# EnricoMiccoli/nodal

Measured on AMD Instinct MI355X. Metric: circuits_per_sec, higher is better.
Workload: dtype f64; 1 GPU; cfg3: grid(1000) 1e6 nodes, sparse CSR path; n=999999, nnz=4995995, parallelism=one GPU

## Files before the change

nodal_amd/csrc/sagg.hip:

```cpp
#include <hip/hip_ext.h>

#include <atomic>
#include <type_traits>

#include "group.h"

int grounded_flags(nodal_ctx *h, uint8_t *flags_dev);

namespace {

using grp::TB;
constexpr int PW = 4;
constexpr int ACAP = 64;
constexpr int RCAP = 96;
constexpr int RCAP_SMALL = 512;
constexpr int RCAP_SMALL_ROWS = 16384;
inline int rcap_for(int64_t nc) { return nc <= RCAP_SMALL_ROWS ? RCAP_SMALL : RCAP; }
constexpr int W0_MAX = 32;
constexpr int COARSEST = 64;
constexpr int MAX_LEVELS = 12;
constexpr int MIS_ROUNDS = 6;
constexpr int TAIL_MAX_N = 1024;
constexpr int TAIL_LEVELS = 6;
constexpr int TAIL_LDS_BUDGET = 150 * 1024;
constexpr int APAD = 32;
constexpr int DOT_BLOCKS = 1024;
#ifndef NODAL_SA_OMEGA
#define NODAL_SA_OMEGA 0.85
#endif
constexpr double OMEGA = NODAL_SA_OMEGA;
constexpr double OMEGA_P = 0.70;
constexpr double OMEGA_P_COARSE = 0.85;
using cyc_t = nodal_cyc_t;

inline unsigned grid_for(int64_t n, unsigned cap = 8192) {
    int64_t g = (n + TB - 1) / TB;
    if (g < 1) g = 1;
    if (g >= 64) g = (g + 7) & ~(int64_t)7;
    return (unsigned)(g > cap ? cap : g);
}
inline int64_t pad64(int64_t n) { return (n + 63) & ~(int64_t)63; }
inline size_t align256(size_t x) { return (x + 255) & ~(size_t)255; }

__device__ __forceinline__ unsigned xcd_block() {
    const unsigned g = gridDim.x, b = blockIdx.x;
    return (g & 7u) ? b : (b & 7u) * (g >> 3) + (b >> 3);
}


struct Ell {
    int64_t n = 0, ld = 0;
    int32_t width = 0;
    const int32_t *col = nullptr;
    const int16_t *dcol = nullptr;
    const double *val = nullptr;
    const float *valf = nullptr;
    const int32_t *len = nullptr;
};

enum { ST_MAXLEN = 0, ST_GRADED = 1, ST_BADDIAG = 2, ST_OVERFLOW = 3, ST_NNZ = 4, ST_UNASSIGNED = 5,
       ST_MAXR = 6, ST_NC = 7 ,
       ST_FARCOL = 8 ,
       ST_FOLDMISS = 9 ,
       ST_COUNT = 10 };

struct SLevel {
    int64_t n = 0, ld = 0, nc = 0;
    int32_t width = 0;
    int32_t maxlen = 0;
    int32_t wfix = 0;
    int64_t nnz = 0;
    DevBuf acol, aval, alen, dinv;
    DevBuf adcol;
    bool d16 = false;
    DevBuf agg, pcol, pval;
    DevBuf rcol, rval, rlen;
    int64_t rld = 0;
    DevBuf vec, part, gflag;
    DevBuf avalf, pvalf, rvalf;
    DevBuf wcol, wval, wlen;
    int32_t wslots = 0;
    bool fold_want = false, fold = false;
    Ell A() const {
        Ell e;
        e.n = n; e.ld = ld; e.width = width;
        e.col = acol.as<int32_t>(); e.val = aval.as<double>(); e.len = alen.as<int32_t>();
        e.valf = avalf.as<float>();
        e.dcol = d16 ? adcol.as<int16_t>() : nullptr;
        return e;
    }
    template <typename T = double> T *v(int which) const { return reinterpret_cast<T *>(vec.as<double>() + (int64_t)which * ld); }
};
enum { V_X = 0, V_R = 1, V_XP = 2, V_RC = 3, V_C1 = 4, V_C2 = 5, V_V1 = 6, V_V2 = 7, V_R2 = 8, V_X1 = 9, V_T = 10,
       V_COUNT = 11 };

struct TailLevelDesc {
    int n, nc, ld, rld, width, nq, lpr;
    const int32_t *acol, *pcol, *rcol, *rlen, *alen;
    const double *aval, *dinv, *pval, *rval;
    int o_aval, o_acol, o_dinv, o_pval, o_pcol, o_rval, o_rcol, o_B, o_X, o_Y, o_R;
};
struct TailDesc {
    int nlev;
    TailLevelDesc lv[TAIL_LEVELS];
    const double *inv;
    int nu;
    int image_bytes;
    int lds_bytes;
    int skip;
    int slots;
    long long *stamps;
};

struct SHierarchy {
    std::vector<SLevel *> pool;
    int nlev = 0;
    int tail = -1;
    bool ready = false;
    bool kcycle = true;
    bool kfrozen = false;
    int kslot = -1, kcount = 0, ksamples = 0;
    int klevels = 1;
    int nu[3] = {2, 1, 2};
    bool dense_coarsest = true;
    DevBuf tail_stamps, tail_image, apcol, apval, aplen, bstat;
    DevBuf tail_op;
    bool tail_dense = false;
    DevBuf mvec;
    hipEvent_t ev_copy = nullptr;
    hipStream_t aux = nullptr;
    hipEvent_t ev_fork = nullptr, ev_join = nullptr, ev_flags = nullptr;
    bool aux_pending = false;
    bool aux_tried = false;
    bool want_flags = false;
    int flags_levels = 0;
    DevBuf stats, coarse_inv, mis_t, mis_m, mis_flag, mis_id, agg1, keys, rstart, cursor, lists;
    TailDesc td;
    uint64_t *host_stats = nullptr;
    bool sym_valid = false;
    uint64_t sym_epoch = 0;
    int64_t sym_n = 0, sym_nnz = 0;
    bool sym_general = false, sym_check = false;
    int32_t sym_floating = 0;
    hipGraph_t it_graph = nullptr;
    hipGraphExec_t it_exec = nullptr;
    uint64_t it_key = 0;
    bool refreshed = false;
    int last_iters = 0;
    int hint_iters = 0;
    int64_t hint_n = 0, hint_nnz = 0;
    int mblock_iters = 0;
    int64_t mblock_n = 0;
    unsigned long long sym_stats[MAX_LEVELS * ST_COUNT] = {0};
    SLevel *level(int l) {
        while ((int)pool.size() <= l) pool.push_back(new SLevel());
        return pool[l];
    }
    void drop_graph() {
        if (it_exec) (void)hipGraphExecDestroy(it_exec);
        if (it_graph) (void)hipGraphDestroy(it_graph);
        it_exec = nullptr;
        it_graph = nullptr;
        it_key = 0;
    }
    ~SHierarchy() {
        drop_graph();
        if (ev_copy) (void)hipEventDestroy(ev_copy);
        if (ev_fork) (void)hipEventDestroy(ev_fork);
        if (ev_join) (void)hipEventDestroy(ev_join);
        if (ev_flags) (void)hipEventDestroy(ev_flags);
        if (aux) (void)hipStreamDestroy(aux);
        for (SLevel *l : pool) {
            DevBuf *b[] = {&l->acol, &l->aval, &l->alen, &l->dinv, &l->agg, &l->pcol, &l->pval, &l->rcol,
                           &l->rval, &l->rlen, &l->vec, &l->part, &l->gflag, &l->avalf, &l->pvalf, &l->rvalf, &l->adcol,
                           &l->wcol, &l->wval, &l->wlen};
            for (DevBuf *x : b) x->release();
            delete l;
        }
        tail_image.release();
        tail_op.release();
        mvec.release();
        tail_stamps.release();
        bstat.release();
        apcol.release();
        apval.release();
        aplen.release();
        DevBuf *b[] = {&stats, &coarse_inv, &mis_t, &mis_m, &mis_flag, &mis_id, &agg1, &keys, &rstart, &cursor, &lists};
        for (DevBuf *x : b) x->release();
        if (host_stats) (void)hipHostFree(host_stats);
    }
};


constexpr int BSTAT_MAX = 65536;
__global__ __launch_bounds__(1024) void reduce_bstat(int nblocks, const uint32_t *__restrict__ bstat,
                                                     unsigned long long *__restrict__ stats, int slot_max,
                                                     int slot_sum) {
    __shared__ unsigned int s_max;
    __shared__ unsigned long long s_sum;
    if (threadIdx.x == 0) { s_max = 0; s_sum = 0; }
    __syncthreads();
    unsigned int m = 0;
    unsigned long long t = 0;
    for (int i = threadIdx.x; i < nblocks; i += 1024) {
        m = max(m, bstat[i]);
        t += bstat[BSTAT_MAX + i];
    }
    atomicMax(&s_max, m);
    atomicAdd(&s_sum, t);
    __syncthreads();
    if (threadIdx.x == 0) {
        if (slot_max >= 0) stats[slot_max] = s_max;
        if (slot_sum >= 0) stats[slot_sum] = s_sum;
    }
}

__global__ __launch_bounds__(TB) void row_stats(int64_t n, const int32_t *__restrict__ indptr,
                                                const int32_t *__restrict__ indices,
                                                const double *__restrict__ data, double share, double spread,
                                                bool general, unsigned long long *__restrict__ stats,
                                                uint32_t *__restrict__ bstat) {
    int32_t mlen = 0;
    uint32_t graded = 0, bad = 0, far = 0;
    for (int64_t i = (int64_t)xcd_block() * TB + threadIdx.x; i < n; i += (int64_t)gridDim.x * TB) {
        const int32_t e0 = indptr[i], e1 = indptr[i + 1];
        mlen = max(mlen, e1 - e0);
        double d = 0.0, mx = 0.0, mn = 1e300;
        for (int32_t e = e0; e < e1; ++e) {
            const double v = data[e];
            const int64_t dc = (int64_t)indices[e] - i;
            if (dc > 32767 || dc < -32767) far = 1;
            if (indices[e] == (int32_t)i) d = v;
            else if (v != 0.0) {
                mx = fmax(mx, fabs(v));
                mn = fmin(mn, fabs(v));
                if (v > 0.0 && !general) bad = 1;
            }
        }
        if (!(d > 0.0)) bad = 1;
        graded += (d > 0.0 && (mx > share * d || mx > spread * mn)) ? 1u : 0u;
    }
    __shared__ unsigned int s_len, s_graded, s_bad;
    if (threadIdx.x == 0) s_len = s_graded = s_bad = 0;
    __syncthreads();
    atomicMax(&s_len, (unsigned)mlen);
    if (graded) atomicAdd(&s_graded, graded);
    if (bad) atomicOr(&s_bad, 1u);
    if (far) atomicOr(&s_bad, 2u);
    __syncthreads();
    if (threadIdx.x == 0) {
        bstat[blockIdx.x] = s_len;
        bstat[BSTAT_MAX + blockIdx.x] = s_graded;
        if (s_bad & 1u) atomicOr(&stats[ST_BADDIAG], 1ull);
        if (s_bad & 2u) stats[ST_FARCOL] = 1ull;
    }
}

__global__ __launch_bounds__(TB) void csr_to_ell(int64_t n, int64_t ld, const int32_t *__restrict__ indptr,
                                                 const int32_t *__restrict__ indices,
                                                 const double *__restrict__ data, int32_t *__restrict__ col,
                                                 double *__restrict__ val, float *__restrict__ valf,
                                                 int32_t *__restrict__ len, double *__restrict__ dinv, int32_t wpad,
                                                 int16_t *__restrict__ dcol) {
    for (int64_t i = (int64_t)xcd_block() * TB + threadIdx.x; i < n; i += (int64_t)gridDim.x * TB) {
        const int32_t e0 = indptr[i], e1 = indptr[i + 1];
        double d = 1.0;
        for (int32_t e = e0; e < e1; ++e) {
            const int32_t c = indices[e];
            const double v = data[e];
            col[(int64_t)(e - e0) * ld + i] = c;
            if (dcol) dcol[(int64_t)(e - e0) * ld + i] = (int16_t)(c - (int32_t)i);
            val[(int64_t)(e - e0) * ld + i] = v;
            valf[(int64_t)(e - e0) * ld + i] = (float)v;
            if (c == (int32_t)i) d = v;
        }
        for (int32_t s = e1 - e0; s < wpad; ++s) {
            col[(int64_t)s * ld + i] = (int32_t)i;
            if (dcol) dcol[(int64_t)s * ld + i] = 0;
            val[(int64_t)s * ld + i] = 0.0;
            valf[(int64_t)s * ld + i] = 0.0f;
        }
        len[i] = e1 - e0;
        dinv[i] = 1.0 / d;
    }
}


__device__ __forceinline__ uint32_t hash30(uint32_t x) {
    x ^= x >> 16;
    x *= 0x7feb352du;
    x ^= x >> 15;
    x *= 0x846ca68bu;
    x ^= x >> 16;
    return x & 0x3fffffffu;
}

__global__ __launch_bounds__(TB) void mis_init(int64_t n, uint32_t *__restrict__ T) {
    for (int64_t i = (int64_t)xcd_block() * TB + threadIdx.x; i < n; i += (int64_t)gridDim.x * TB)
        T[i] = (1u << 30) | hash30((uint32_t)i);
}

template <int NB>
__device__ __forceinline__ uint32_t nbr_max_batch(const Ell &A, const uint32_t *__restrict__ v, int64_t i, int32_t l, int32_t s0,
                                                  uint32_t best) {
    int32_t c[NB];
#pragma unroll
    for (int u = 0; u < NB; ++u) c[u] = A.col[(int64_t)(s0 + u < l ? s0 + u : 0) * A.ld + i];
    uint32_t t[NB];
#pragma unroll
    for (int u = 0; u < NB; ++u) t[u] = v[c[u]];
#pragma unroll
    for (int u = 0; u < NB; ++u) best = t[u] > best ? t[u] : best;
    return best;
}
__device__ __forceinline__ uint32_t nbr_max(const Ell &A, const uint32_t *__restrict__ v, int64_t i, int32_t l, uint32_t best) {
    if (l <= 5) return nbr_max_batch<5>(A, v, i, l, 0, best);
    for (int32_t s0 = 0; s0 < l; s0 += 8) best = nbr_max_batch<8>(A, v, i, l, s0, best);
    return best;
}

__global__ __launch_bounds__(TB) void mis_max(Ell A, const uint32_t *__restrict__ v, uint32_t *__restrict__ m) {
    for (int64_t i = (int64_t)xcd_block() * TB + threadIdx.x; i < A.n; i += (int64_t)gridDim.x * TB)
        m[i] = nbr_max(A, v, i, A.len[i], v[i]);
}

__global__ __launch_bounds__(TB) void mis_update(Ell A, uint32_t *__restrict__ T, const uint32_t *__restrict__ m1) {
    for (int64_t i = (int64_t)xcd_block() * TB + threadIdx.x; i < A.n; i += (int64_t)gridDim.x * TB) {
        const uint32_t own = T[i];
        if ((own >> 30) != 1) continue;
        const uint32_t best = nbr_max(A, m1, i, A.len[i], m1[i]);
        if (best == own) T[i] = own | (2u << 30);
        else if ((best >> 30) == 3) T[i] = 0;
    }
}

__global__ __launch_bounds__(TB) void mis_count(int64_t n, const uint32_t *__restrict__ T,
                                                unsigned long long *__restrict__ out) {
    uint32_t left = 0;
    for (int64_t i = (int64_t)xcd_block() * TB + threadIdx.x; i < n; i += (int64_t)gridDim.x * TB)
        left += (T[i] >> 30) == 1 ? 1u : 0u;
#pragma unroll
    for (int off = 32; off > 0; off >>= 1) left += __shfl_down(left, off, 64);
    if ((threadIdx.x & 63) == 0 && left) atomicAdd(out, (unsigned long long)left);
}

__global__ __launch_bounds__(TB) void mis_flag_roots(Ell A, const uint32_t *__restrict__ T,
                                                     uint32_t *__restrict__ flag) {
    for (int64_t i = (int64_t)xcd_block() * TB + threadIdx.x; i <= A.n; i += (int64_t)gridDim.x * TB) {
        uint32_t f = 0;
        if (i < A.n) {
            const uint32_t own = T[i];
            if ((own >> 30) == 3) f = 1;
            else if ((own >> 30) == 1) {
                bool near = false;
                const int32_t l = A.len[i];
                for (int32_t s = 0; s < l; ++s) near = near || (T[A.col[(int64_t)s * A.ld + i]] >> 30) == 3;
                f = near ? 0u : 1u;
            }
        }
        flag[i] = f;
    }
}

constexpr int64_t MIS_SMALL_MAX = 1024;
__global__ __launch_bounds__(1024) void mis_small(Ell A, uint32_t *__restrict__ T, uint32_t *__restrict__ M,
                                                  uint32_t *__restrict__ flag, int rounds) {
    const int64_t n = A.n;
    for (int64_t i = threadIdx.x; i < n; i += 1024) T[i] = (1u << 30) | hash30((uint32_t)i);
    __syncthreads();
    for (int r = 0; r < rounds; ++r) {
        for (int64_t i = threadIdx.x; i < n; i += 1024) {
            uint32_t best = T[i];
            const int32_t l = A.len[i];
            for (int32_t s = 0; s < l; ++s) {
                const uint32_t t = T[A.col[(int64_t)s * A.ld + i]];
                best = t > best ? t : best;
            }
            M[i] = best;
        }
        __syncthreads();
        for (int64_t i = threadIdx.x; i < n; i += 1024) {
            const uint32_t own = T[i];
            if ((own >> 30) != 1) continue;
            uint32_t best = M[i];
            const int32_t l = A.len[i];
            for (int32_t s = 0; s < l; ++s) {
                const uint32_t t = M[A.col[(int64_t)s * A.ld + i]];
                best = t > best ? t : best;
            }
            if (best == own) T[i] = own | (2u << 30);
            else if ((best >> 30) == 3) T[i] = 0;
        }
        __syncthreads();
    }
    for (int64_t i = threadIdx.x; i <= n; i += 1024) {
        uint32_t f = 0;
        if (i < n) {
            const uint32_t own = T[i];
            if ((own >> 30) == 3) f = 1;
            else if ((own >> 30) == 1) {
                bool near = false;
                const int32_t l = A.len[i];
                for (int32_t s = 0; s < l; ++s) near = near || (T[A.col[(int64_t)s * A.ld + i]] >> 30) == 3;
                f = near ? 0u : 1u;
            }
        }
        flag[i] = f;
    }
}

__global__ __launch_bounds__(TB) void assign_near(Ell A, const uint32_t *__restrict__ T,
                                                  const uint32_t *__restrict__ flag,
                                                  const uint32_t *__restrict__ id, int32_t *__restrict__ agg1) {
    for (int64_t i = (int64_t)xcd_block() * TB + threadIdx.x; i < A.n; i += (int64_t)gridDim.x * TB) {
        int32_t a = -1;
        if (flag[i]) a = (int32_t)id[i];
        else {
            uint32_t best = 0;
            const int32_t l = A.len[i];
            auto batch = [&](auto NBc, int32_t s0) {
                constexpr int NB = decltype(NBc)::value;
                int32_t c[NB];
#pragma unroll
                for (int u = 0; u < NB; ++u) c[u] = A.col[(int64_t)(s0 + u < l ? s0 + u : 0) * A.ld + i];
                uint32_t fl[NB], tt[NB], idd[NB];
#pragma unroll
                for (int u = 0; u < NB; ++u) {
                    fl[u] = flag[c[u]];
                    tt[u] = T[c[u]];
                    idd[u] = id[c[u]];
                }
#pragma unroll
                for (int u = 0; u < NB; ++u) {
                    if (s0 + u >= l || c[u] == (int32_t)i || !fl[u]) continue;
                    const uint32_t t = tt[u] | (3u << 30);
                    if (t > best) { best = t; a = (int32_t)idd[u]; }
                }
            };
            if (l <= 5) batch(std::integral_constant<int, 5>{}, 0);
            else for (int32_t s0 = 0; s0 < l; s0 += 8) batch(std::integral_constant<int, 8>{}, s0);
        }
        agg1[i] = a;
    }
}

__global__ __launch_bounds__(TB) void assign_far(Ell A, const int32_t *__restrict__ agg1, int32_t *__restrict__ agg,
                                                 unsigned long long *__restrict__ stats) {
    for (int64_t i = (int64_t)xcd_block() * TB + threadIdx.x; i < A.n; i += (int64_t)gridDim.x * TB) {
        int32_t a = agg1[i];
        if (a < 0) {
            double bw = -1.0;
            const int32_t l = A.len[i];
            auto batch = [&](auto NBc, int32_t s0) {
                constexpr int NB = decltype(NBc)::value;
                int32_t c[NB];
                double w[NB];
#pragma unroll
                for (int u = 0; u < NB; ++u) {
                    const int64_t at = (int64_t)(s0 + u < l ? s0 + u : 0) * A.ld + i;
                    c[u] = A.col[at];
                    w[u] = fabs(A.val[at]);
                }
                int32_t aj[NB];
#pragma unroll
                for (int u = 0; u < NB; ++u) aj[u] = agg1[c[u]];
#pragma unroll
                for (int u = 0; u < NB; ++u) {
                    if (s0 + u >= l || c[u] == (int32_t)i || aj[u] < 0) continue;
                    if (w[u] > bw) { bw = w[u]; a = aj[u]; }
                }
            };
            if (l <= 5) batch(std::integral_constant<int, 5>{}, 0);
            else for (int32_t s0 = 0; s0 < l; s0 += 8) batch(std::integral_constant<int, 8>{}, s0);
            if (a < 0) stats[ST_UNASSIGNED] = 1;
        }
        agg[i] = a;
    }
}
// ... 59 lines not shown
                                               const uint64_t *__restrict__ keys, int64_t ld,
                                               const double *__restrict__ pval, int32_t *__restrict__ rcol,
                                               double *__restrict__ rval, float *__restrict__ rvalf,
                                               int32_t *__restrict__ rlen,
                                               unsigned long long *__restrict__ stats, uint32_t *__restrict__ bstat,
                                               uint32_t rcap) {
    uint32_t mlen = 0;
    const int sub = threadIdx.x & 7;
    const int64_t rows_per_pass = (int64_t)gridDim.x * (TB / 8);
    for (int64_t I = (int64_t)xcd_block() * (TB / 8) + threadIdx.x / 8; I < nc; I += rows_per_pass) {
        const uint32_t s0 = rstart[I];
        uint32_t l = rstart[I + 1] - s0;
        mlen = l > mlen ? l : mlen;
        if (l > rcap) l = rcap;
        const uint32_t upto = nc <= 4096 ? rcap : ((l + 7u) & ~7u);
        for (uint32_t t = sub; t < upto; t += 8) {
            const int64_t at = ((int64_t)(t >> 3) * rld + I) * 8 + (t & 7);
            if (t < l) {
                const uint64_t key = keys[s0 + t];
                const int64_t i = (int64_t)(key >> 2);
                const double v = pval[(int64_t)(key & 3) * ld + i];
                rcol[at] = (int32_t)i;
                rval[at] = v;
                rvalf[at] = (float)v;
            } else {
                rcol[at] = 0;
                rval[at] = 0.0;
                rvalf[at] = 0.0f;
            }
        }
        if (sub == 0) rlen[I] = (int32_t)l;
    }
    if (mlen > rcap) atomicOr(&stats[ST_OVERFLOW], 2ull);
    __shared__ unsigned int s_max;
    if (threadIdx.x == 0) s_max = 0;
    __syncthreads();
#pragma unroll
    for (int off = 32; off > 0; off >>= 1) {
        const uint32_t o = __shfl_down(mlen, off, 64);
        mlen = o > mlen ? o : mlen;
    }
    if ((threadIdx.x & 63) == 0) atomicMax(&s_max, mlen);
    __syncthreads();
    if (threadIdx.x == 0) {
        bstat[blockIdx.x] = s_max;
        bstat[BSTAT_MAX + blockIdx.x] = 0;
    }
}

__global__ __launch_bounds__(TB) void r_refresh(int64_t nc, int64_t rld, const int32_t *__restrict__ rlen,
                                                const int32_t *__restrict__ rcol, int64_t ld,
                                                const int32_t *__restrict__ pcol, const double *__restrict__ pval,
                                                double *__restrict__ rval, float *__restrict__ rvalf) {
    const int sub = threadIdx.x & 7;
    const int64_t rows_per_pass = (int64_t)gridDim.x * (TB / 8);
    for (int64_t I = (int64_t)xcd_block() * (TB / 8) + threadIdx.x / 8; I < nc; I += rows_per_pass) {
        const int32_t l = rlen[I];
        for (int32_t t = sub; t < l; t += 8) {
            const int64_t at = ((int64_t)(t >> 3) * rld + I) * 8 + (t & 7);
            const int64_t i = rcol[at];
            double v = 0.0;
#pragma unroll
            for (int k = 0; k < PW; ++k) {
                const double pv = pval[(int64_t)k * ld + i];
                v = pcol[(int64_t)k * ld + i] == (int32_t)I ? pv : v;
            }
            rval[at] = v;
            rvalf[at] = (float)v;
        }
    }
}

__global__ __launch_bounds__(TB) void r_sort_short(const uint32_t *__restrict__ rstart, uint64_t *__restrict__ keys,
                                                   int64_t nc) {
    for (int64_t I = (int64_t)xcd_block() * TB + threadIdx.x; I < nc; I += (int64_t)gridDim.x * TB) {
        const uint32_t s0 = rstart[I];
        const int len = (int)(rstart[I + 1] - s0);
        if (len < 2) continue;
        if (len <= 4) grp::sort_short_row<4>(keys + s0, len);
        else if (len <= 8) grp::sort_short_row<8>(keys + s0, len);
        else if (len <= 16) grp::sort_short_row<16>(keys + s0, len);
        else if (len <= 32) grp::sort_short_row<32>(keys + s0, len);
    }
}
__global__ __launch_bounds__(64) void r_sort_medium(const uint32_t *__restrict__ rstart, uint64_t *__restrict__ keys,
                                                    int64_t nc) {
    __shared__ uint64_t buf[RCAP_SMALL];
    const int lane = threadIdx.x;
    for (int64_t I = blockIdx.x; I < nc; I += gridDim.x) {
        const uint32_t s0 = rstart[I];
        const int len = (int)(rstart[I + 1] - s0);
        if (len <= 32 || len > RCAP_SMALL) continue;
        const int P = len <= 64 ? 64 : (len <= 128 ? 128 : (len <= 256 ? 256 : 512));
        for (int e = lane; e < P; e += 64) buf[e] = e < len ? keys[s0 + e] : ~0ull;
        __syncthreads();
        for (int size = 2; size <= P; size <<= 1)
            for (int stride = size >> 1; stride > 0; stride >>= 1) {
                for (int p = lane; p < P / 2; p += 64) {
                    const int i = ((p & ~(stride - 1)) << 1) | (p & (stride - 1));
                    const int j = i | stride;
                    const bool up = (i & size) == 0;
                    const uint64_t a = buf[i], b = buf[j];
                    if ((a > b) == up) { buf[i] = b; buf[j] = a; }
                }
                __syncthreads();
            }
        for (int e = lane; e < len; e += 64) keys[s0 + e] = buf[e];
        __syncthreads();
    }
}

__device__ __forceinline__ int wave_excl_scan(int v, int *total) {
    const int lane = threadIdx.x & 63;
    int incl = v;
#pragma unroll
    for (int off = 1; off < 64; off <<= 1) {
        const int t = __shfl_up(incl, off, 64);
        if (lane >= off) incl += t;
    }
    *total = __shfl(incl, 63, 64);
    return incl - v;
}

template <int APW, bool EMIT>
__global__ __launch_bounds__(TB) void ap_rows(Ell A, const int32_t *__restrict__ pcol, const double *__restrict__ pval,
                                              int32_t *__restrict__ apcol, double *__restrict__ apval,
                                              int32_t *__restrict__ aplen, unsigned long long *__restrict__ stats,
                                              const double *__restrict__ dinv, int32_t *__restrict__ wcol,
                                              float *__restrict__ wval, int32_t *__restrict__ wlen) {
    bool overflow = false, miss = false;
    for (int64_t i = (int64_t)xcd_block() * TB + threadIdx.x; i < A.n; i += (int64_t)gridDim.x * TB) {
        int32_t c[APW];
        double v[APW];
        [[maybe_unused]] int32_t Jo[PW];
        [[maybe_unused]] double po[PW], wd = 0.0;
        if constexpr (EMIT) {
#pragma unroll
            for (int sp = 0; sp < PW; ++sp) {
                Jo[sp] = pcol[(int64_t)sp * A.ld + i];
                po[sp] = pval[(int64_t)sp * A.ld + i];
            }
            wd = OMEGA * dinv[i];
        }
#pragma unroll
        for (int q = 0; q < APW; ++q) { c[q] = -1; v[q] = 0.0; }
        int cnt = 0;
        const int32_t l = A.len[i];
        for (int32_t s = 0; s < l; ++s) {
            const int32_t k = A.col[(int64_t)s * A.ld + i];
            const double a = A.val[(int64_t)s * A.ld + i];
            int32_t J[PW];
            double pp[PW];
#pragma unroll
            for (int sp = 0; sp < PW; ++sp) {
                J[sp] = pcol[(int64_t)sp * A.ld + k];
                pp[sp] = pval[(int64_t)sp * A.ld + k];
            }
#pragma unroll
            for (int sp = 0; sp < PW; ++sp) {
                if (J[sp] < 0) continue;
                const double t = a * pp[sp];
                bool placed = false;
#pragma unroll
                for (int q = 0; q < APW; ++q)
                    if (!placed && c[q] == J[sp]) { v[q] += t; placed = true; }
#pragma unroll
                for (int q = 0; q < APW; ++q)
                    if (!placed && c[q] < 0) { c[q] = J[sp]; v[q] = t; placed = true; cnt = q + 1; }
                if (!placed) overflow = true;
            }
        }
#pragma unroll
        for (int q = 0; q < APW; ++q)
            if (q < cnt) {
                apcol[(int64_t)q * A.ld + i] = c[q];
                apval[(int64_t)q * A.ld + i] = v[q];
            }
        aplen[i] = cnt;
        if constexpr (EMIT) {
            int have = 0, found = 0;
#pragma unroll
            for (int sp = 0; sp < PW; ++sp) have += Jo[sp] >= 0 ? 1 : 0;
#pragma unroll
            for (int q = 0; q < APW; ++q)
                if (q < cnt) {
                    double pv = 0.0;
#pragma unroll
                    for (int sp = 0; sp < PW; ++sp)
                        if (Jo[sp] == c[q]) { pv += po[sp]; ++found; }
                    wcol[(int64_t)q * A.ld + i] = c[q];
                    wval[(int64_t)q * A.ld + i] = (float)(pv - wd * v[q]);
                }
            wlen[i] = cnt;
            if (found != have) miss = true;
        }
    }
    if (overflow) atomicOr(&stats[ST_OVERFLOW], 4ull);
    if (miss) stats[ST_FOLDMISS] = 1ull;
}

template <int APW, bool EMIT>
__global__ __launch_bounds__(64) void ap_rows_lds(Ell A, const int32_t *__restrict__ pcol,
                                                  const double *__restrict__ pval, int32_t *__restrict__ apcol,
                                                  double *__restrict__ apval, int32_t *__restrict__ aplen,
                                                  unsigned long long *__restrict__ stats,
                                                  const double *__restrict__ dinv, int32_t *__restrict__ wcol,
                                                  float *__restrict__ wval, int32_t *__restrict__ wlen) {
    __shared__ int32_t tc[APW * 64];
    __shared__ double tv[APW * 64];
    const int lane = threadIdx.x;
    bool overflow = false, miss = false;
    for (int64_t i0 = (int64_t)xcd_block() * 64; i0 < A.n; i0 += (int64_t)gridDim.x * 64) {
        const int64_t i = i0 + lane;
#pragma unroll 8
        for (int q = 0; q < APW; ++q) tc[q * 64 + lane] = -1;
        int cnt = 0;
        if (i < A.n) {
            const int32_t l = A.len[i];
            [[maybe_unused]] int32_t Jo[PW];
            [[maybe_unused]] double po[PW], wd = 0.0;
            if constexpr (EMIT) {
#pragma unroll
                for (int sp = 0; sp < PW; ++sp) {
                    Jo[sp] = pcol[(int64_t)sp * A.ld + i];
                    po[sp] = pval[(int64_t)sp * A.ld + i];
                }
                wd = OMEGA * dinv[i];
            }
            constexpr int AB = 4;
            for (int32_t s0 = 0; s0 < l; s0 += AB) {
                int32_t kk[AB];
                double aa[AB];
#pragma unroll
                for (int u = 0; u < AB; ++u) {
                    const int32_t su = s0 + u < l ? s0 + u : 0;
                    kk[u] = A.col[(int64_t)su * A.ld + i];
                    aa[u] = A.val[(int64_t)su * A.ld + i];
                }
                int32_t J[AB][PW];
                double pp[AB][PW];
#pragma unroll
                for (int u = 0; u < AB; ++u)
#pragma unroll
                    for (int sp = 0; sp < PW; ++sp) {
                        J[u][sp] = pcol[(int64_t)sp * A.ld + kk[u]];
                        pp[u][sp] = pval[(int64_t)sp * A.ld + kk[u]];
                    }
#pragma unroll
                for (int u = 0; u < AB; ++u) {
                    if (s0 + u >= l) continue;
#pragma unroll
                    for (int sp = 0; sp < PW; ++sp) {
                        if (J[u][sp] < 0) continue;
                        const double t = aa[u] * pp[u][sp];
                        uint32_t slot = ((uint32_t)J[u][sp] * 2654435761u) >> 16 & (APW - 1);
                        bool placed = false;
                        for (int probe = 0; probe < APW && !placed; ++probe) {
                            const int32_t c = tc[slot * 64 + lane];
                            if (c == J[u][sp]) {
                                tv[slot * 64 + lane] += t;
                                placed = true;
                            } else if (c < 0) {
                                tc[slot * 64 + lane] = J[u][sp];
                                tv[slot * 64 + lane] = t;
                                ++cnt;
                                placed = true;
                            }
                            slot = (slot + 1) & (APW - 1);
                        }
                        if (!placed) overflow = true;
                    }
                }
            }
            int o = 0, found = 0;
            for (int q = 0; q < APW; ++q) {
                const int32_t c = tc[q * 64 + lane];
                if (c >= 0) {
                    const double t = tv[q * 64 + lane];
                    apcol[(int64_t)o * A.ld + i] = c;
                    apval[(int64_t)o * A.ld + i] = t;
                    if constexpr (EMIT) {
                        double pv = 0.0;
#pragma unroll
                        for (int sp = 0; sp < PW; ++sp)
                            if (Jo[sp] == c) { pv += po[sp]; ++found; }
                        wcol[(int64_t)o * A.ld + i] = c;
                        wval[(int64_t)o * A.ld + i] = (float)(pv - wd * t);
                    }
                    ++o;
                }
            }
            aplen[i] = cnt;
            if constexpr (EMIT) {
                int have = 0;
#pragma unroll
                for (int sp = 0; sp < PW; ++sp) have += Jo[sp] >= 0 ? 1 : 0;
                wlen[i] = cnt;
                if (found != have) miss = true;
            }
        }
    }
    if (overflow) atomicOr(&stats[ST_OVERFLOW], 4ull);
    if (miss) stats[ST_FOLDMISS] = 1ull;
}

__device__ __forceinline__ int galerkin_products(int64_t ld, const int32_t *__restrict__ apcol,
                                                 const double *__restrict__ apval, const int32_t *__restrict__ aplen,
                                                 int64_t rld, const int32_t *__restrict__ rcol,
                                                 const double *__restrict__ rval, int64_t I, int t0, int tn,
                                                 int32_t *lJ, double *lV) {
    const int lane = threadIdx.x;
    int32_t i = 0, len = 0;
    double w = 0.0;
    if (lane < tn) {
        const int t = t0 + lane;
        const int64_t rat = ((int64_t)(t >> 3) * rld + I) * 8 + (t & 7);
        i = rcol[rat];
        w = rval[rat];
        len = aplen[i];
    }
    int np = 0;
    int o = wave_excl_scan(len, &np);
    constexpr int INFL = 8;
    for (int32_t s0 = 0; s0 < len; s0 += INFL) {
        int32_t cj[INFL];
        double cv[INFL];
#pragma unroll
        for (int q = 0; q < INFL; ++q) {
            const int32_t s = s0 + q < len ? s0 + q : s0;
            cj[q] = apcol[(int64_t)s * ld + i];
            cv[q] = apval[(int64_t)s * ld + i];
        }
#pragma unroll
        for (int q = 0; q < INFL; ++q)
            if (s0 + q < len) {
                lJ[o] = cj[q];
                lV[o] = w * cv[q];
                ++o;
            }
    }
    for (int p = lane + np; p < np + 72; p += 64) lJ[p] = -1;
    __syncthreads();
    return np;
}

template <bool NUMERIC>
__global__ __launch_bounds__(64) void galerkin(int64_t ld, const int32_t *__restrict__ apcol,
                                               const double *__restrict__ apval, const int32_t *__restrict__ aplen,
                                               int64_t nc, int64_t rld, const int32_t *__restrict__ rcol,
                                               const double *__restrict__ rval, const int32_t *__restrict__ rlen,
                                               int64_t cld, int32_t *__restrict__ ccol, double *__restrict__ cval,
                                               float *__restrict__ cvalf,
                                               int32_t *__restrict__ clen, double *__restrict__ cdinv,
                                               unsigned long long *__restrict__ stats, uint32_t *__restrict__ bstat,
                                               int G, int pcap, int maxseg) {
    extern __shared__ __attribute__((aligned(16))) char gsm[];
    int32_t *set = reinterpret_cast<int32_t *>(gsm);
    double *lV = reinterpret_cast<double *>(gsm + 1024);
    int32_t *lJ = reinterpret_cast<int32_t *>(lV + pcap);
    const int lane = threadIdx.x;
    uint32_t my_max = 0, my_nnz = 0, my_flags = 0;
    for (int64_t I = blockIdx.x; I < nc; I += gridDim.x) {
        const int rl = rlen[I];
        const int ngroups = (rl + G - 1) / G;
        int np = 0;
        int total = 0;
        int32_t myJ = 0x7fffffff;
        if constexpr (NUMERIC) {
            total = clen[I];
            if (lane < total) myJ = ccol[(int64_t)lane * cld + I];
        } else {
        for (int k = lane; k < 256; k += 64) set[k] = -1;
        __syncthreads();
        for (int g = 0; g < ngroups; ++g) {
            np = galerkin_products(ld, apcol, apval, aplen, rld, rcol, rval, I, g * G, min(G, rl - g * G), lJ, lV);
            for (int p = lane; p < np; p += 64) {
                const int32_t J = lJ[p];
                uint32_t hsh = ((uint32_t)J * 2654435761u) >> 24;
                for (int probe = 0; probe < 256; ++probe) {
                    const int32_t old = atomicCAS(&set[hsh], -1, J);
                    if (old == -1 || old == J) break;
                    hsh = (hsh + 1) & 255u;
                    if (probe == 255) my_flags |= 1u;
                }
            }
            __syncthreads();
        }
        int32_t mine[4];
        int cnt = 0;
#pragma unroll
        for (int q = 0; q < 4; ++q) {
            mine[q] = set[lane * 4 + q];
            cnt += mine[q] >= 0 ? 1 : 0;
        }
        int off = wave_excl_scan(cnt, &total);
        __syncthreads();
#pragma unroll
        for (int q = 0; q < 4; ++q)
            if (mine[q] >= 0) set[off++] = mine[q];
        __syncthreads();
        if (total > ACAP) {
            my_flags |= 1u;
            total = ACAP;
        }
        myJ = lane < total ? set[lane] : 0x7fffffff;
        __syncthreads();
#pragma unroll
        for (int k = 2; k <= 64; k <<= 1) {
#pragma unroll
            for (int j = k >> 1; j > 0; j >>= 1) {
                const int32_t other = __shfl_xor(myJ, j, 64);
                const bool up = (lane & k) == 0, lower = (lane & j) == 0;
                const int32_t lo = myJ < other ? myJ : other, hi = myJ < other ? other : myJ;
                myJ = (lower == up) ? lo : hi;
            }
        }
        }
        const int nseg = min(maxseg, total <= 16 ? 4 : (total <= 32 ? 2 : 1)), segw = 64 / nseg;
        const int seg = lane / segw;
        const int32_t segJ = __shfl(myJ, lane % segw, 64);
        double acc = 0.0;
        for (int g = 0; g < ngroups; ++g) {
            if (ngroups > 1 || NUMERIC)
                np = galerkin_products(ld, apcol, apval, aplen, rld, rcol, rval, I, g * G, min(G, rl - g * G), lJ, lV);
            int chunk = (((np + nseg - 1) / nseg) + 7) & ~7;
            if (nseg > 1 && ((chunk >> 3) & 1) == 0) chunk += 8;
            for (int p = seg * chunk; p < (seg + 1) * chunk; p += 8) {
                int32_t j8[8];
                double v8[8];
#pragma unroll
                for (int u = 0; u < 8; ++u) {
                    j8[u] = lJ[p + u];
                    v8[u] = lV[p + u];
                }
#pragma unroll
                for (int u = 0; u < 8; ++u) acc += j8[u] == segJ ? v8[u] : 0.0;
            }
            __syncthreads();
        }
        if (nseg == 4) {
            const double a1 = __shfl(acc, lane + 16, 64), a2 = __shfl(acc, lane + 32, 64), a3 = __shfl(acc, lane + 48, 64);
            acc = (acc + a1) + (a2 + a3);
        } else if (nseg == 2) {
            acc += __shfl(acc, lane + 32, 64);
        }
        if (lane >= total && lane < APAD) {
            ccol[(int64_t)lane * cld + I] = (int32_t)I;
            cval[(int64_t)lane * cld + I] = 0.0;
            cvalf[(int64_t)lane * cld + I] = 0.0f;
        }
        if (lane < total) {
            ccol[(int64_t)lane * cld + I] = myJ;
            cval[(int64_t)lane * cld + I] = acc;
            cvalf[(int64_t)lane * cld + I] = (float)acc;
            if (myJ == (int32_t)I) {
                if (!(acc > 0.0)) my_flags |= 4u;
                cdinv[I] = acc > 0.0 ? 1.0 / acc : 1.0;
            }
        }
        if (lane == 0) {
            clen[I] = total;
            my_max = (uint32_t)total > my_max ? (uint32_t)total : my_max;
            my_nnz += (uint32_t)total;
        }
        __syncthreads();
    }
    if (lane == 0) {
        bstat[blockIdx.x] = my_max;
        bstat[BSTAT_MAX + blockIdx.x] = my_nnz;
    }
    if (my_flags & 1u) atomicOr(&stats[ST_OVERFLOW], 1ull);
    if (my_flags & 4u) atomicOr(&stats[ST_BADDIAG], 1ull);
}

__global__ __launch_bounds__(256) void coarsest_inverse(Ell A, double *__restrict__ inv,
                                                        unsigned long long *__restrict__ stats) {
    __shared__ double M[COARSEST][2 * COARSEST + 1];
    const int n = (int)A.n;
    for (int t = threadIdx.x; t < n * 2 * n; t += 256) {
        const int r = t / (2 * n), c = t % (2 * n);
        M[r][c] = (c >= n && c - n == r) ? 1.0 : 0.0;
    }
    __syncthreads();
    for (int r = threadIdx.x; r < n; r += 256)
        for (int s = 0; s < A.len[r]; ++s) M[r][A.col[(int64_t)s * A.ld + r]] = A.val[(int64_t)s * A.ld + r];
    __syncthreads();
    for (int k = 0; k < n; ++k) {
        const double pv = M[k][k];
        if (!(pv > 0.0)) {
            if (threadIdx.x == 0) atomicOr(&stats[ST_BADDIAG], 2ull);
            return;
        }
        const double rp = 1.0 / pv;
        __syncthreads();
        for (int c = threadIdx.x; c < 2 * n; c += 256) M[k][c] *= rp;
        __syncthreads();
        for (int t = threadIdx.x; t < n * 2 * n; t += 256) {
            const int r = t / (2 * n), c = t % (2 * n);
            if (r != k && c != k) M[r][c] = fma(-M[r][k], M[k][c], M[r][c]);
        }
        __syncthreads();
        for (int r = threadIdx.x; r < n; r += 256)
            if (r != k) M[r][k] = 0.0;
        __syncthreads();
    }
    for (int t = threadIdx.x; t < n * n; t += 256) inv[t] = M[t / n][n + t % n];
}

__global__ __launch_bounds__(TB) void flags_up(int64_t n, const int32_t *__restrict__ agg,
                                               const uint8_t *__restrict__ fine, uint8_t *__restrict__ coarse) {
    for (int64_t i = (int64_t)xcd_block() * TB + threadIdx.x; i < n; i += (int64_t)gridDim.x * TB)
        if (fine[i]) coarse[agg[i]] = 1;
}
__global__ __launch_bounds__(64) void last_level_floating(Ell A, const uint8_t *__restrict__ grounded,
                                                          uint32_t *__restrict__ floating) {
    __shared__ int label[COARSEST];
    __shared__ int changed;
    const int n = (int)A.n, i = threadIdx.x;
    if (i < n) label[i] = i;
    __syncthreads();
    for (int it = 0; it < COARSEST; ++it) {
        if (i == 0) changed = 0;
        __syncthreads();
        int best = i < n ? label[i] : 0;
        if (i < n)
            for (int s = 0; s < A.len[i]; ++s) {
                const int l = label[A.col[(int64_t)s * A.ld + i]];
                best = l < best ? l : best;
            }
        __syncthreads();
        if (i < n && best < label[i]) {
            label[i] = best;
            changed = 1;
        }
        __syncthreads();
        if (!changed) break;
        __syncthreads();
    }
    __shared__ int ok[COARSEST];
    if (i < n) ok[i] = 0;
    __syncthreads();
    if (i < n && grounded[i]) ok[label[i]] = 1;
    __syncthreads();
    if (i < n && label[i] == i && !ok[i]) *floating = 1;
}

__global__ __launch_bounds__(TB) void any_unflagged(int64_t n, const uint8_t *__restrict__ grounded,
                                                    uint32_t *__restrict__ floating) {
    for (int64_t i = (int64_t)xcd_block() * TB + threadIdx.x; i < n; i += (int64_t)gridDim.x * TB)
        if (!grounded[i]) *floating = 1;
}

}

#include "sagg_cycle.h"

namespace {

constexpr int SAGG_DECLINED = -3;

int width_class(int maxlen) {
    static const int classes[] = {4, 5, 6, 8, 12, 16, 20, 24, 32};
    for (int c : classes)
        if (maxlen <= c) return c;
    return 0;
}
int choose_wfix(int maxlen, int64_t n, int64_t nnz, int pad_limit) {
    const int c = width_class(maxlen);
    if (c == 0 || c > pad_limit) return 0;
    static const double slack = getenv("NODAL_SA_PADSLACK") ? atof(getenv("NODAL_SA_PADSLACK")) : 1.3;
    if ((double)c * (double)n <= slack * (double)nnz || n <= 32768) return c;
    return 0;
}

SHierarchy *hierarchy_of(nodal_ctx *h) {
    if (!h->sagg) h->sagg = new SHierarchy();
    return static_cast<SHierarchy *>(h->sagg);
}

struct SolveBufs {
    double *r, *p, *p2, *Ap, *part_rz, *part_zap, *part_rr, *part_pap, *sc;
    cyc_t *z, *x0;
    int g0;
};

template <bool NUMERIC>
int galerkin_product(nodal_ctx *h, SHierarchy *H, int l, hipEvent_t r_ready = nullptr, int phase = 0) {
    hipStream_t st = h->stream;
    SLevel *L = H->level(l), *C = H->level(l + 1);
    const int64_t n = L->n, ld = L->ld, nc = C->n;
    Ell A = L->A();
    A.width = L->maxlen;
    unsigned long long *dstats = H->stats.as<unsigned long long>();
    const int apw = A.width <= 6 ? 16 : 64;
    NODAL_HIP_TRY(h, H->apcol.reserve((size_t)apw * ld * 4 + 64));
    NODAL_HIP_TRY(h, H->apval.reserve((size_t)apw * ld * 8 + 64));
    NODAL_HIP_TRY(h, H->aplen.reserve((size_t)ld * 4 + 64));
    int32_t *apcol = H->apcol.as<int32_t>(), *aplen = H->aplen.as<int32_t>();
    double *apval = H->apval.as<double>();
    unsigned long long *lst = dstats + (size_t)l * ST_COUNT;
    const unsigned g = grid_for(n);
    if (phase != 2) {
        const bool w = L->fold_want && L->wslots == apw;
        int32_t *wcol = w ? L->wcol.as<int32_t>() : nullptr, *wlen = w ? L->wlen.as<int32_t>() : nullptr;
        float *wval = w ? L->wval.as<float>() : nullptr;
        const double *dinv = L->dinv.as<double>();
        const int32_t *pc = L->pcol.as<int32_t>();
        const double *pv = L->pval.as<double>();
        const unsigned gl = (unsigned)((n + 63) / 64 < 4096 ? (n + 63) / 64 : 4096);
        if (apw == 16 && w) ap_rows<16, true><<<g, TB, 0, st>>>(A, pc, pv, apcol, apval, aplen, lst, dinv, wcol, wval, wlen);
        else if (apw == 16) ap_rows<16, false><<<g, TB, 0, st>>>(A, pc, pv, apcol, apval, aplen, lst, dinv, wcol, wval, wlen);
        else if (w) ap_rows_lds<64, true><<<gl, 64, 0, st>>>(A, pc, pv, apcol, apval, aplen, lst, dinv, wcol, wval, wlen);
        else ap_rows_lds<64, false><<<gl, 64, 0, st>>>(A, pc, pv, apcol, apval, aplen, lst, dinv, wcol, wval, wlen);
        NODAL_HIP_TRY(h, hipGetLastError());
    }
    if (phase == 1) return NODAL_OK;
    int G = 1024 / apw;
    G = (G < 8 ? 8 : (G > 64 ? 64 : G));
    static const int g_env = getenv("NODAL_SA_GG") ? atoi(getenv("NODAL_SA_GG")) : 40;
    if (g_env >= 8 && g_env <= 64 && apw == 16) G = g_env & ~7;
    const int pcap = G * apw + 72;
    const size_t lds = 1024 + (size_t)pcap * 12;
    static const int64_t gcap = getenv("NODAL_SA_GCAP") ? atoll(getenv("NODAL_SA_GCAP")) : 16384;
    static const int maxseg = getenv("NODAL_SA_GSEG") ? atoi(getenv("NODAL_SA_GSEG")) : 4;
    const unsigned gg = (unsigned)(nc < gcap ? nc : (gcap < BSTAT_MAX ? gcap : BSTAT_MAX));
    if (r_ready) NODAL_HIP_TRY(h, hipStreamWaitEvent(st, r_ready, 0));
    galerkin<NUMERIC><<<gg, 64, lds, st>>>(
        ld, apcol, apval, aplen, nc, L->rld, L->rcol.as<int32_t>(), L->rval.as<double>(), L->rlen.as<int32_t>(),
        C->ld, C->acol.as<int32_t>(), C->aval.as<double>(), C->avalf.as<float>(), C->alen.as<int32_t>(),
        C->dinv.as<double>(), dstats + (size_t)(l + 1) * ST_COUNT, H->bstat.as<uint32_t>(), G, pcap, maxseg);
    if (!NUMERIC)
        reduce_bstat<<<1, 1024, 0, st>>>((int)gg, H->bstat.as<uint32_t>(), dstats + (size_t)(l + 1) * ST_COUNT,
                                         ST_MAXLEN, ST_NNZ);
    NODAL_HIP_TRY(h, hipGetLastError());
    return NODAL_OK;
}

double omega_p(int level) {
    static double w[2] = {-1.0, -1.0};
    if (w[0] < 0.0) {
        double a = OMEGA_P, b = OMEGA_P_COARSE;
        if (const char *e = getenv("NODAL_SA_OMEGA_P")) {
            a = atof(e);
            const char *c = strchr(e, ',');
            b = c ? atof(c + 1) : a;
        }
        w[1] = b > 0.0 && b < 1.2 ? b : OMEGA_P_COARSE;
        w[0] = a > 0.0 && a < 1.0 ? a : OMEGA_P;
    }
    return w[level > 0 ? 1 : 0];
}

constexpr int64_t FOLD_MAX_ROWS = 1 << 19;
struct FoldSetting { int mode = 0; unsigned mask = 0; };
const FoldSetting &fold_setting() {
    static const FoldSetting s = [] {
        FoldSetting f;
        const char *e = getenv("NODAL_SA_FOLD_POST");
        if (!e || !*e) return f;
        if (strchr(e, 'l')) {
            f.mode = 3;
            for (const char *q = e; (q = strchr(q, 'l')) != nullptr; ++q) {
                const int k = atoi(q + 1);
                if (q[1] >= '0' && q[1] <= '9' && k < MAX_LEVELS) f.mask |= 1u << k;
            }
        } else {
            f.mode = atoi(e) == 0 ? 1 : 2;
        }
        return f;
    }();
    return s;
}
bool fold_wanted(int level, int64_t n) {
    if (level > 0 && n <= TAIL_MAX_N) return false;
    const FoldSetting &f = fold_setting();
    switch (f.mode) {
    case 1: return false;
    case 2: return true;
    case 3: return (f.mask >> level & 1u) != 0;
    default: return n <= FOLD_MAX_ROWS;
    }
}
void decide_folds(SHierarchy *H, const unsigned long long *hs, bool trace) {
    for (int k = 0; k < H->nlev; ++k) {
        SLevel *L = H->pool[k];
        const bool runs_cycle = k + 1 < H->nlev && (H->tail < 0 || k < H->tail);
        const bool miss = hs[(size_t)k * ST_COUNT + ST_FOLDMISS] != 0;
        L->fold = L->fold_want && runs_cycle && !miss;
        if (trace && L->fold_want && runs_cycle)
            fprintf(stderr, "[sagg] level %d (%lld rows): first post-smoothing sweep %s\n", k, (long long)L->n,
                    miss ? "NOT folded: a row of A P lacks a column of its P row (no stored diagonal)"
                         : "folded into the prolongation");
    }
}

int build_level(nodal_ctx *h, SHierarchy *H, int l, unsigned long long *hs, bool *declined, bool *stop) {
    hipStream_t st = h->stream;
    SLevel *L = H->level(l);
    const int64_t n = L->n, ld = L->ld;
    Ell A = L->A();
    A.width = L->maxlen;
    unsigned long long *dstats = H->stats.as<unsigned long long>();

    NODAL_HIP_TRY(h, H->mis_t.reserve((size_t)n * 8 + 64));
    NODAL_HIP_TRY(h, H->mis_m.reserve((size_t)n * 8 + 64));
    NODAL_HIP_TRY(h, H->mis_flag.reserve((size_t)(n + 1) * 4 + 64));
    NODAL_HIP_TRY(h, H->mis_id.reserve((size_t)(n + 1) * 4 + 64 + scan_tmp_bytes(n + 1)));
    NODAL_HIP_TRY(h, H->agg1.reserve((size_t)n * 4 + 64));
    NODAL_HIP_TRY(h, L->agg.reserve((size_t)n * 4 + 64));
    NODAL_HIP_TRY(h, H->cursor.reserve((MIS_ROUNDS + 2) * 8 + 64));
    uint32_t *T = H->mis_t.as<uint32_t>(), *M = H->mis_m.as<uint32_t>();
    uint32_t *flag = H->mis_flag.as<uint32_t>(), *id = H->mis_id.as<uint32_t>();
    unsigned long long *cnt = H->cursor.as<unsigned long long>();
    void *scan_tmp = H->mis_id.as<char>() + (((size_t)(n + 1) * 4 + 63) & ~(size_t)63);

    const unsigned g = grid_for(n);
    static const bool trace_mis = getenv("NODAL_TRACE") != nullptr;
    if (trace_mis) NODAL_HIP_TRY(h, hipMemsetAsync(cnt, 0, (MIS_ROUNDS + 2) * 8, st));
    static const int mis_rounds = getenv("NODAL_SA_MIS") ? std::min(MIS_ROUNDS, std::max(1, atoi(getenv("NODAL_SA_MIS")))) : MIS_ROUNDS;
    if (n <= MIS_SMALL_MAX && !trace_mis) {
        mis_small<<<1, 1024, 0, st>>>(A, T, M, flag, mis_rounds);
    } else {
        mis_init<<<g, TB, 0, st>>>(n, T);
        for (int r = 0; r < mis_rounds; ++r) {
            mis_max<<<g, TB, 0, st>>>(A, T, M);
            mis_update<<<g, TB, 0, st>>>(A, T, M);
            if (trace_mis) mis_count<<<g, TB, 0, st>>>(n, T, cnt + r + 1);
        }
        mis_flag_roots<<<grid_for(n + 1), TB, 0, st>>>(A, T, flag);
    }
    NODAL_HIP_TRY(h, hipGetLastError());
    NODAL_TRY(scan_exclusive_u32(h, flag, id, n + 1, reinterpret_cast<uint32_t *>(dstats + (size_t)l * ST_COUNT + ST_NC),
                                 scan_tmp));
    NODAL_HIP_TRY(h, hipMemcpyAsync(hs, dstats, (size_t)MAX_LEVELS * ST_COUNT * 8, hipMemcpyDeviceToHost, st));
    unsigned long long hcnt[MIS_ROUNDS + 1] = {0};
    if (trace_mis) NODAL_HIP_TRY(h, hipMemcpyAsync(hcnt, cnt, sizeof hcnt, hipMemcpyDeviceToHost, st));
    if (!H->ev_copy) NODAL_HIP_TRY(h, hipEventCreateWithFlags(&H->ev_copy, hipEventDisableTiming));
    NODAL_HIP_TRY(h, hipEventRecord(H->ev_copy, st));
    NODAL_HIP_TRY(h, L->pcol.reserve((size_t)PW * ld * 4 + 64));
    NODAL_HIP_TRY(h, L->pval.reserve((size_t)PW * ld * 8 + 64));
    NODAL_HIP_TRY(h, L->pvalf.reserve((size_t)PW * ld * 4 + 64));
    assign_near<<<g, TB, 0, st>>>(A, T, flag, id, H->agg1.as<int32_t>());
    assign_far<<<g, TB, 0, st>>>(A, H->agg1.as<int32_t>(), L->agg.as<int32_t>(), dstats + (size_t)l * ST_COUNT);
    build_P<<<g, TB, 0, st>>>(A, L->dinv.as<double>(), L->agg.as<int32_t>(), L->pcol.as<int32_t>(),
                             L->pval.as<double>(), L->pvalf.as<float>(), omega_p(l));
    NODAL_HIP_TRY(h, hipGetLastError());
    NODAL_WAIT_EVENT(h, H->ev_copy, st);
    if (trace_mis) {
        fprintf(stderr, "[sagg] level %d: undecided after each MIS round:", l);
        for (int r = 1; r <= MIS_ROUNDS; ++r) fprintf(stderr, " %llu", hcnt[r]);
        fprintf(stderr, "\n");
    }
    const int64_t nc = (int64_t)(hs[(size_t)l * ST_COUNT + ST_NC] & 0xffffffffull);
    if (l > 0) {
        const unsigned long long *s = hs + (size_t)l * ST_COUNT;
        L->maxlen = (int32_t)s[ST_MAXLEN];
        L->nnz = (int64_t)s[ST_NNZ];
        A.width = L->maxlen;
        if (s[ST_OVERFLOW] || s[ST_BADDIAG] || hs[(size_t)(l - 1) * ST_COUNT + ST_OVERFLOW] ||
            hs[(size_t)(l - 1) * ST_COUNT + ST_UNASSIGNED]) {
            *declined = true;
            return NODAL_OK;
        }
    }
    if (nc >= n || L->maxlen <= 1) {
        *stop = true;
        return NODAL_OK;
    }
    if ((nc * 2 > n && n > 4096) || nc < 1) {
        *declined = true;
        return NODAL_OK;
    }
    L->nc = nc;

    static const bool fork_allowed = !(getenv("NODAL_SA_FORK") && atoi(getenv("NODAL_SA_FORK")) == 0);
    if (H->aux && !nodal_extra_streams_ok(h) && nodal_calls_in_flight() <= 1) {
        NODAL_WAIT_STREAM(h, H->aux);
        (void)hipStreamDestroy(H->aux);
        H->aux = nullptr;
        H->aux_tried = false;
    }
    if (fork_allowed && !H->aux_tried && nodal_extra_streams_ok(h)) {
        H->aux_tried = true;
        if (hipStreamCreateWithFlags(&H->aux, hipStreamNonBlocking) != hipSuccess) H->aux = nullptr;
        if (H->aux && ((!H->ev_fork && hipEventCreateWithFlags(&H->ev_fork, hipEventDisableTiming) != hipSuccess) ||
                       (!H->ev_join && hipEventCreateWithFlags(&H->ev_join, hipEventDisableTiming) != hipSuccess) ||
                       (!H->ev_flags && hipEventCreateWithFlags(&H->ev_flags, hipEventDisableTiming) != hipSuccess))) {
            (void)hipStreamDestroy(H->aux);
            H->aux = nullptr;
        }
        (void)hipGetLastError();
    }
    const bool forked = fork_allowed && H->aux != nullptr && nodal_extra_streams_ok(h);
    const size_t a4 = (((size_t)(nc + 1) * 4) + 255) & ~(size_t)255;
    const size_t scan2 = (scan_tmp_bytes(nc + 1) + 255) & ~(size_t)255;
    NODAL_HIP_TRY(h, H->rstart.reserve(a4 + 256 + scan2 + (size_t)PW * ld * 4 + 64));
    NODAL_HIP_TRY(h, H->keys.reserve((size_t)PW * n * 8 + 64));
    SLevel *C = H->level(l + 1);
    C->n = nc;
    C->ld = pad64(nc);
    C->width = ACAP;
    C->nc = 0;
    L->rld = C->ld;
    const int rcap = rcap_for(nc);
    NODAL_HIP_TRY(h, L->rcol.reserve((size_t)rcap * C->ld * 4 + 64));
    NODAL_HIP_TRY(h, L->rval.reserve((size_t)rcap * C->ld * 8 + 64));
    NODAL_HIP_TRY(h, L->rvalf.reserve((size_t)rcap * C->ld * 4 + 64));
    NODAL_HIP_TRY(h, L->rlen.reserve((size_t)C->ld * 4 + 64));
    NODAL_HIP_TRY(h, C->acol.reserve((size_t)ACAP * C->ld * 4 + 64));
    NODAL_HIP_TRY(h, C->aval.reserve((size_t)ACAP * C->ld * 8 + 64));
    NODAL_HIP_TRY(h, C->avalf.reserve((size_t)ACAP * C->ld * 4 + 64));
    NODAL_HIP_TRY(h, C->alen.reserve((size_t)C->ld * 4 + 64));
    NODAL_HIP_TRY(h, C->dinv.reserve((size_t)C->ld * 8 + 64));
    if (forked && H->want_flags) {
        if (l == 0) NODAL_HIP_TRY(h, L->gflag.reserve((size_t)n + 64));
        NODAL_HIP_TRY(h, C->gflag.reserve((size_t)C->n + 64));
    }
    {
        const int apw = L->maxlen <= 6 ? 16 : 64;
        NODAL_HIP_TRY(h, H->apcol.reserve((size_t)apw * ld * 4 + 64));
        NODAL_HIP_TRY(h, H->apval.reserve((size_t)apw * ld * 8 + 64));
        NODAL_HIP_TRY(h, H->aplen.reserve((size_t)ld * 4 + 64));
        L->fold = false;
        L->fold_want = fold_wanted(l, n);
        L->wslots = apw;
        if (L->fold_want) {
            NODAL_HIP_TRY(h, L->wcol.reserve((size_t)apw * ld * 4 + 64));
            NODAL_HIP_TRY(h, L->wval.reserve((size_t)apw * ld * 4 + 64));
            NODAL_HIP_TRY(h, L->wlen.reserve((size_t)ld * 4 + 64));
        }
    }
    hipStream_t main_st = h->stream;
    struct StreamGuard {
        nodal_ctx *h;
        hipStream_t keep;
        ~StreamGuard() { h->stream = keep; }
    } guard{h, main_st};
    if (forked) {
        NODAL_HIP_TRY(h, hipEventRecord(H->ev_fork, main_st));
        NODAL_HIP_TRY(h, hipStreamWaitEvent(H->aux, H->ev_fork, 0));
        H->aux_pending = true;
        NODAL_TRY(galerkin_product<false>(h, H, l, nullptr, 1));
        h->stream = H->aux;
        st = H->aux;
    }
    char *rs = H->rstart.as<char>();
    uint32_t *rstart = reinterpret_cast<uint32_t *>(rs);
    void *scan_tmp2 = rs + a4 + 256;
    uint32_t *place = reinterpret_cast<uint32_t *>(rs + a4 + 256 + scan2);
    NODAL_HIP_TRY(h, hipMemsetAsync(rs, 0, a4 + 256, st));
    r_count<<<g, TB, 0, st>>>(n, ld, L->pcol.as<int32_t>(), rstart, place);
    NODAL_HIP_TRY(h, hipGetLastError());
    NODAL_TRY(scan_exclusive_u32(h, rstart, rstart, nc + 1, nullptr, scan_tmp2));
    uint64_t *keys = H->keys.as<uint64_t>();
    r_fill<<<g, TB, 0, st>>>(n, ld, L->pcol.as<int32_t>(), rstart, place, keys);
    r_sort_short<<<grid_for(nc), TB, 0, st>>>(rstart, keys, nc);
    r_sort_medium<<<(unsigned)(nc < 8192 ? nc : 8192), 64, 0, st>>>(rstart, keys, nc);
    NODAL_HIP_TRY(h, hipGetLastError());

    {
        const unsigned gr = grid_for(nc * 8);
        r_to_ell<<<gr, TB, 0, st>>>(nc, L->rld, rstart, keys, ld, L->pval.as<double>(), L->rcol.as<int32_t>(),
                                   L->rval.as<double>(), L->rvalf.as<float>(), L->rlen.as<int32_t>(),
                                   dstats + (size_t)l * ST_COUNT, H->bstat.as<uint32_t>(), (uint32_t)rcap);
        reduce_bstat<<<1, 1024, 0, st>>>((int)gr, H->bstat.as<uint32_t>(), dstats + (size_t)l * ST_COUNT, ST_MAXR, -1);
    }
    if (forked) {
        NODAL_HIP_TRY(h, hipGetLastError());
        NODAL_HIP_TRY(h, hipEventRecord(H->ev_join, H->aux));
        if (H->want_flags && H->flags_levels == l) {
            if (l == 0) NODAL_TRY(grounded_flags(h, L->gflag.as<uint8_t>()));
            NODAL_HIP_TRY(h, hipMemsetAsync(C->gflag.p, 0, ((size_t)C->n + 63) & ~(size_t)63, st));
            flags_up<<<grid_for(n), TB, 0, st>>>(n, L->agg.as<int32_t>(), L->gflag.as<uint8_t>(), C->gflag.as<uint8_t>());
            NODAL_HIP_TRY(h, hipGetLastError());
            NODAL_HIP_TRY(h, hipEventRecord(H->ev_flags, H->aux));
            H->flags_levels = l + 1;
        }
        h->stream = main_st;
        st = main_st;
    }
    NODAL_TRY(galerkin_product<false>(h, H, l, forked ? H->ev_join : nullptr, forked ? 2 : 0));
    if (forked && H->flags_levels != l + 1) H->aux_pending = false;
    return NODAL_OK;
}

const void *tail_kernel(int slots) {
    return slots <= 8 ? reinterpret_cast<const void *>(k_tail<8>)
                      : slots <= 16 ? reinterpret_cast<const void *>(k_tail<16>)
                                    : reinterpret_cast<const void *>(k_tail<32>);
}

const void *tail_op_kernel(int slots) {
    return slots <= 8 ? reinterpret_cast<const void *>(k_tail_pack_op<8>)
                      : slots <= 16 ? reinterpret_cast<const void *>(k_tail_pack_op<16>)
                                    : reinterpret_cast<const void *>(k_tail_pack_op<32>);
}

int tail_walk(nodal_ctx *h, SHierarchy *H, const double *b, double *out, int nv) {
    const TailDesc &d = H->td;
    const char *img = H->tail_image.as<char>();
    if (d.slots <= 8) k_tail<8><<<nv, 1024, (size_t)d.lds_bytes, h->stream>>>(d, img, b, out, nv);
    else if (d.slots <= 16) k_tail<16><<<nv, 1024, (size_t)d.lds_bytes, h->stream>>>(d, img, b, out, nv);
    else k_tail<32><<<nv, 1024, (size_t)d.lds_bytes, h->stream>>>(d, img, b, out, nv);
    NODAL_HIP_TRY(h, hipGetLastError());
    return NODAL_OK;
}

template <int NV>
int tail_apply(nodal_ctx *h, SHierarchy *H, const double *b, double *out) {
    const int n = H->td.lv[0].n;
    const double *T = H->tail_op.as<double>();
    const unsigned gr = (unsigned)((n + 3) / 4);
    if (n <= 256) k_tail_apply<4, NV><<<gr, 256, 0, h->stream>>>(n, T, b, out);
    else if (n <= 512) k_tail_apply<8, NV><<<gr, 256, 0, h->stream>>>(n, T, b, out);
    else k_tail_apply<16, NV><<<gr, 256, 0, h->stream>>>(n, T, b, out);
    NODAL_HIP_TRY(h, hipGetLastError());
    return NODAL_OK;
}

int tail_self_check(nodal_ctx *h, SHierarchy *H) {
    const int n = H->td.lv[0].n;
    std::vector<double> b((size_t)n), yc((size_t)n), yd((size_t)n), T((size_t)n * n);
    uint64_t seed = 0x9e3779b97f4a7c15ull;
    for (int i = 0; i < n; ++i) {
        uint64_t z = (seed += 0x9e3779b97f4a7c15ull);
        z = (z ^ (z >> 30)) * 0xbf58476d1ce4e5b9ull;
        z = (z ^ (z >> 27)) * 0x94d049bb133111ebull;
        z ^= z >> 31;
        b[i] = (double)(z >> 11) * (1.0 / 4503599627370496.0) - 1.0;
    }
    DevBuf v;
    hipError_t e = v.reserve((size_t)3 * n * 8);
    double *db = v.as<double>(), *dc = db + n, *dd = dc + n;
    int rc = NODAL_OK;
    if (e == hipSuccess) e = hipMemcpyAsync(db, b.data(), (size_t)n * 8, hipMemcpyHostToDevice, h->stream);
    if (e == hipSuccess) rc = tail_walk(h, H, db, dc, 1);
    if (e == hipSuccess && rc == NODAL_OK) rc = tail_apply<1>(h, H, db, dd);
    if (e == hipSuccess && rc == NODAL_OK) e = hipStreamSynchronize(h->stream);
    if (e == hipSuccess) e = hipMemcpy(yc.data(), dc, (size_t)n * 8, hipMemcpyDeviceToHost);
    if (e == hipSuccess) e = hipMemcpy(yd.data(), dd, (size_t)n * 8, hipMemcpyDeviceToHost);
    if (e == hipSuccess) e = hipMemcpy(T.data(), H->tail_op.p, (size_t)n * n * 8, hipMemcpyDeviceToHost);
    v.release();
    if (rc != NODAL_OK) return rc;
    NODAL_HIP_TRY(h, e);
    double d = 0.0, dp = 0.0;
    for (int i = 0; i < n; ++i) {
        long double y = 0.0L, a = 0.0L;
        for (int j = 0; j < n; ++j) {
            y += (long double)T[(size_t)i * n + j] * b[j];
            a += fabsl((long double)T[(size_t)i * n + j] * b[j]);
        }
        const double den = (double)a;
        const double q = fabs(yd[i] - yc[i]) / den, qp = (double)(fabsl((long double)yd[i] - y) / a);
        d = !(q <= d) ? q : d;
        dp = !(qp <= dp) ? qp : dp;
    }
    fprintf(stderr, "[sagg] tail check: n_t %d, dense operator against the cycle d = %.3e (product alone %.3e)\n", n, d, dp);
    return NODAL_OK;
}

int form_tail_op(nodal_ctx *h, SHierarchy *H) {
    static const bool on = !(getenv("NODAL_SA_TAIL_DENSE") && atoi(getenv("NODAL_SA_TAIL_DENSE")) == 0);
    H->tail_dense = false;
    if (!on || H->tail < 0) return NODAL_OK;
    const TailDesc &d = H->td;
    const int n = d.lv[0].n;
    static std::atomic<int> cus[64];
    const int dev = h->device >= 0 && h->device < 64 ? h->device : 0;
    int ncu = cus[dev].load(std::memory_order_acquire);
    if (ncu == 0) {
        NODAL_HIP_TRY(h, hipDeviceGetAttribute(&ncu, hipDeviceAttributeMultiprocessorCount, h->device >= 0 ? h->device : 0));
        if (ncu < 1) ncu = 1;
        cus[dev].store(ncu, std::memory_order_release);
    }
    NODAL_HIP_TRY(h, H->tail_op.reserve((size_t)n * n * 8 + 64));
    const unsigned gr = (unsigned)(n < ncu ? n : ncu);
    double *T = H->tail_op.as<double>();
    const char *img = H->tail_image.as<char>();
    if (d.slots <= 8) k_tail_pack_op<8><<<gr, 1024, (size_t)d.lds_bytes, h->stream>>>(d, img, T);
    else if (d.slots <= 16) k_tail_pack_op<16><<<gr, 1024, (size_t)d.lds_bytes, h->stream>>>(d, img, T);
    else k_tail_pack_op<32><<<gr, 1024, (size_t)d.lds_bytes, h->stream>>>(d, img, T);
    NODAL_HIP_TRY(h, hipGetLastError());
    H->tail_dense = true;
    static const bool check = getenv("NODAL_TRACE") && getenv("NODAL_SA_TAIL_CHECK") && atoi(getenv("NODAL_SA_TAIL_CHECK")) != 0;
    if (check) NODAL_TRY(tail_self_check(h, H));
    return NODAL_OK;
}

template <typename TC>
int fold_check_level(nodal_ctx *h, SHierarchy *H, int l, bool two) {
    hipStream_t st = h->stream;
    const SLevel *L = H->pool[l];
    const int64_t n = L->n, nc = H->pool[l + 1]->n;
    const Ell A = L->A();
    uint64_t seed = 0x9e3779b97f4a7c15ull + (uint64_t)l;
    auto unit = [&]() {
        uint64_t z = (seed += 0x9e3779b97f4a7c15ull);
        z = (z ^ (z >> 30)) * 0xbf58476d1ce4e5b9ull;
        z = (z ^ (z >> 27)) * 0x94d049bb133111ebull;
        z ^= z >> 31;
        return (double)(z >> 11) * (1.0 / 4503599627370496.0) - 1.0;
    };
    std::vector<cyc_t> hx((size_t)n), hb((size_t)n);
    std::vector<TC> he((size_t)2 * nc);
    for (auto &v : hx) v = (cyc_t)unit();
    for (auto &v : hb) v = (cyc_t)unit();
    for (auto &v : he) v = (TC)unit();
    const double hcoef[2] = {0.9, 0.4};
    const size_t vb = align256((size_t)n * sizeof(cyc_t)), eb = align256((size_t)nc * sizeof(TC)), db = align256((size_t)n * 8);
    DevBuf buf;
    hipError_t e = buf.reserve(6 * vb + 2 * eb + 2 * db + 256);
    char *p = buf.as<char>();
    cyc_t *x = reinterpret_cast<cyc_t *>(p), *b = reinterpret_cast<cyc_t *>(p + vb), *r = reinterpret_cast<cyc_t *>(p + 2 * vb),
          *xp = reinterpret_cast<cyc_t *>(p + 3 * vb), *mt = reinterpret_cast<cyc_t *>(p + 4 * vb),
          *mf = reinterpret_cast<cyc_t *>(p + 5 * vb);
    TC *c1 = reinterpret_cast<TC *>(p + 6 * vb), *c2 = reinterpret_cast<TC *>(p + 6 * vb + eb);
    double *d = reinterpret_cast<double *>(p + 6 * vb + 2 * eb), *q = reinterpret_cast<double *>(p + 6 * vb + 2 * eb + db);
    double *coef = reinterpret_cast<double *>(p + 6 * vb + 2 * eb + 2 * db);
    std::vector<double> hd((size_t)n), hq((size_t)n);
    if (e == hipSuccess) e = hipMemcpyAsync(x, hx.data(), (size_t)n * sizeof(cyc_t), hipMemcpyHostToDevice, st);
    if (e == hipSuccess) e = hipMemcpyAsync(b, hb.data(), (size_t)n * sizeof(cyc_t), hipMemcpyHostToDevice, st);
    if (e == hipSuccess) e = hipMemcpyAsync(c1, he.data(), (size_t)nc * sizeof(TC), hipMemcpyHostToDevice, st);
    if (e == hipSuccess) e = hipMemcpyAsync(c2, he.data() + nc, (size_t)nc * sizeof(TC), hipMemcpyHostToDevice, st);
    if (e == hipSuccess) e = hipMemcpyAsync(coef, hcoef, sizeof hcoef, hipMemcpyHostToDevice, st);
    if (e == hipSuccess) {
        const unsigned g = grid_for(n), tb = L->wfix ? TB : TB * LPR_RAGGED;
        const double *dinv = L->dinv.as<double>(), *cf = two ? coef : nullptr;
        const int32_t *wcol = L->wcol.as<int32_t>(), *wlen = L->wlen.as<int32_t>();
        const float *wval = L->wval.as<float>();
        SAGG_DISPATCH_W(L->wfix, (k_smooth_residual<W, cyc_t><<<g, tb, 0, st>>>(A, b, x, r)));
        k_prolong<TC><<<g, TB, 0, st>>>(n, L->ld, L->pcol.as<int32_t>(), L->pvalf.as<float>(), x, c1, two ? c2 : nullptr, cf, xp);
        SAGG_DISPATCH_W(L->wfix, (k_post<W, false, cyc_t, cyc_t><<<g, tb, 0, st>>>(A, dinv, b, xp, mt, nullptr, nullptr, nullptr)));
        k_prolong_post<TC, cyc_t><<<g, TB, 0, st>>>(n, L->ld, wcol, wval, wlen, x, r, dinv, c1, two ? c2 : nullptr, cf, mf);
        k_fold_check<TC><<<g, TB, 0, st>>>(A, dinv, b, x, xp, wcol, wval, wlen, c1, two ? c2 : nullptr, cf, mt, mf, d, q);
        e = hipGetLastError();
    }
    if (e == hipSuccess) e = hipStreamSynchronize(st);
    if (e == hipSuccess) e = hipMemcpy(hd.data(), d, (size_t)n * 8, hipMemcpyDeviceToHost);
    if (e == hipSuccess) e = hipMemcpy(hq.data(), q, (size_t)n * 8, hipMemcpyDeviceToHost);
    buf.release();
    NODAL_HIP_TRY(h, e);
    double dm = 0.0, qm = 0.0;
    for (int64_t i = 0; i < n; ++i) {
        dm = !(hd[i] <= dm) ? hd[i] : dm;
        qm = !(hq[i] <= qm) ? hq[i] : qm;
    }
    fprintf(stderr, "[sagg] fold check: level %d, rows %lld, slots %d, width %d, fused launch against the two d = %.3e "
                    "(worst row against its own bound: %.3e)\n", l, (long long)n, (int)L->wslots, (int)L->maxlen, dm, qm);
    return NODAL_OK;
}
int fold_self_check(nodal_ctx *h, SHierarchy *H) {
    static const bool check = getenv("NODAL_TRACE") && getenv("NODAL_SA_FOLD_CHECK") && atoi(getenv("NODAL_SA_FOLD_CHECK")) != 0;
    if (!check) return NODAL_OK;
    for (int l = 0; l + 1 < H->nlev; ++l) {
        if (!H->pool[l]->fold) continue;
        const bool last = l + 1 == H->tail || l + 1 == H->nlev - 1;
        if (last) NODAL_TRY(fold_check_level<double>(h, H, l, false));
        else NODAL_TRY(fold_check_level<cyc_t>(h, H, l, true));
    }
    return NODAL_OK;
}

int build_tail(nodal_ctx *h, SHierarchy *H, const unsigned long long *hs) {
    H->tail = -1;
    H->tail_dense = false;
    const int last = H->nlev - 1;
    auto up16 = [](int x) { return (x + 15) & ~15; };
    for (int t = 1; t <= last; ++t) {
        if (H->pool[t]->n > TAIL_MAX_N || last - t + 1 > TAIL_LEVELS) continue;
        TailDesc d;
        memset(&d, 0, sizeof d);
        d.nlev = last - t + 1;
        d.nu = getenv("NODAL_SA_TAIL_NU") ? atoi(getenv("NODAL_SA_TAIL_NU")) : 3;
        if (d.nu < 1) d.nu = 1;
        int off = 0;
        for (int k = 0; k < d.nlev; ++k) {
            const SLevel *L = H->pool[t + k];
            TailLevelDesc &q = d.lv[k];
            q.n = (int)L->n; q.nc = (int)L->nc; q.ld = (int)L->ld; q.rld = (int)L->rld; q.width = L->maxlen;
            q.acol = L->acol.as<int32_t>(); q.aval = L->aval.as<double>();
            q.dinv = L->dinv.as<double>(); q.alen = L->alen.as<int32_t>();
            q.pcol = L->pcol.as<int32_t>(); q.pval = L->pval.as<double>();
            q.rcol = L->rcol.as<int32_t>(); q.rval = L->rval.as<double>(); q.rlen = L->rlen.as<int32_t>();
            if (k == d.nlev - 1) {
                q.o_aval = off; off = up16(off + (H->dense_coarsest ? q.n * q.n : q.n) * 8);
                continue;
            }
            const int maxr = (int)hs[(size_t)(t + k) * ST_COUNT + ST_MAXR];
            q.nq = (maxr + 7) / 8;
            q.lpr = 1;
            while (q.lpr < 8 && q.n * q.lpr * 2 <= 1024) q.lpr *= 2;
            q.o_aval = off; off = up16(off + q.n * q.width * 8);
            q.o_acol = off; off = up16(off + q.n * q.width * 2);
            q.o_dinv = off; off = up16(off + q.n * 8);
            q.o_pval = off; off = up16(off + q.n * PW * 8);
            q.o_pcol = off; off = up16(off + q.n * PW * 2);
            q.o_rval = off; off = up16(off + q.nq * q.nc * 8 * 8);
            q.o_rcol = off; off = up16(off + q.nq * q.nc * 8 * 2);
        }
        d.image_bytes = off;
        for (int k = 0; k < d.nlev; ++k) {
            TailLevelDesc &q = d.lv[k];
            q.o_B = off; off = up16(off + q.n * 8);
            q.o_X = off; off = up16(off + q.n * 8);
            if (k == d.nlev - 1) continue;
            q.o_Y = off; off = up16(off + q.n * 8);
            q.o_R = off; off = up16(off + q.n * 8);
        }
        d.inv = H->dense_coarsest ? H->coarse_inv.as<double>() : nullptr;
        d.skip = d.nlev > 1 ? d.lv[0].o_dinv : 0;
        d.lds_bytes = off - d.skip;
        if (getenv("NODAL_TAIL_PROBE")) {
            NODAL_HIP_TRY(h, H->tail_stamps.reserve(64 * sizeof(long long)));
            d.stamps = H->tail_stamps.as<long long>();
        }
        if (d.lds_bytes > TAIL_LDS_BUDGET) continue;
        d.slots = d.nlev > 1 ? (d.lv[0].width + d.lv[0].lpr - 1) / d.lv[0].lpr : 1;
        if (d.slots > 32) continue;
        {
            static std::atomic<bool> lds_allowed[64][3];
            const int dev = h->device >= 0 && h->device < 64 ? h->device : 0;
            const int which = d.slots <= 8 ? 0 : (d.slots <= 16 ? 1 : 2);
            if (!lds_allowed[dev][which].load(std::memory_order_acquire)) {
                NODAL_HIP_TRY(h, hipFuncSetAttribute(tail_kernel(d.slots), hipFuncAttributeMaxDynamicSharedMemorySize,
                                                     TAIL_LDS_BUDGET));
                NODAL_HIP_TRY(h, hipFuncSetAttribute(tail_op_kernel(d.slots), hipFuncAttributeMaxDynamicSharedMemorySize,
                                                     TAIL_LDS_BUDGET));
                lds_allowed[dev][which].store(true, std::memory_order_release);
            }
        }
        NODAL_HIP_TRY(h, H->tail_image.reserve((size_t)d.image_bytes + 256));
        k_tail_pack<<<1, 1024, 0, h->stream>>>(d, H->tail_image.as<char>());
        NODAL_HIP_TRY(h, hipGetLastError());
        H->td = d;
        H->tail = t;
        NODAL_TRY(form_tail_op(h, H));
        break;
    }
    return NODAL_OK;
}

int sagg_refresh(nodal_ctx *h, SHierarchy *H, const int32_t *indptr0, const int32_t *indices0, const double *data0,
                 bool general, bool *ok) {
    *ok = false;
    hipStream_t st = h->stream;
    unsigned long long *dstats = H->stats.as<unsigned long long>();
    unsigned long long *hs = reinterpret_cast<unsigned long long *>(H->host_stats);
    NODAL_HIP_TRY(h, hipMemsetAsync(dstats, 0, (size_t)MAX_LEVELS * ST_COUNT * 8, st));
    SLevel *L0 = H->pool[0];
    const int64_t n0 = L0->n;
    {
        const unsigned gr = grid_for(n0);
        static const double spread = getenv("NODAL_SA_SPREAD") ? atof(getenv("NODAL_SA_SPREAD")) : 16.0;
        static const double share = getenv("NODAL_SA_SHARE") ? atof(getenv("NODAL_SA_SHARE")) : 0.9;
        row_stats<<<gr, TB, 0, st>>>(n0, indptr0, indices0, data0, share, spread, general, dstats, H->bstat.as<uint32_t>());
        reduce_bstat<<<1, 1024, 0, st>>>((int)gr, H->bstat.as<uint32_t>(), dstats, ST_MAXLEN, ST_GRADED);
    }
    csr_to_ell<<<grid_for(n0), TB, 0, st>>>(n0, L0->ld, indptr0, indices0, data0, L0->acol.as<int32_t>(),
                                           L0->aval.as<double>(), L0->avalf.as<float>(),
                                           L0->alen.as<int32_t>(), L0->dinv.as<double>(), L0->wfix,
                                           L0->d16 ? L0->adcol.as<int16_t>() : nullptr);
    NODAL_HIP_TRY(h, hipGetLastError());
    for (int l = 0; l + 1 < H->nlev; ++l) {
        SLevel *L = H->pool[l], *C = H->pool[l + 1];
        Ell A = L->A();
        A.width = L->maxlen;
        build_P<<<grid_for(L->n), TB, 0, st>>>(A, L->dinv.as<double>(), L->agg.as<int32_t>(), L->pcol.as<int32_t>(),
                                              L->pval.as<double>(), L->pvalf.as<float>(), omega_p(l));
        const bool forked = H->aux != nullptr && nodal_extra_streams_ok(h) &&
                            !(getenv("NODAL_SA_FORK") && atoi(getenv("NODAL_SA_FORK")) == 0);
        hipStream_t rst = st;
        if (forked) {
            NODAL_HIP_TRY(h, hipEventRecord(H->ev_fork, st));
            NODAL_HIP_TRY(h, hipStreamWaitEvent(H->aux, H->ev_fork, 0));
            H->aux_pending = true;
            NODAL_TRY(galerkin_product<true>(h, H, l, nullptr, 1));
            rst = H->aux;
        }
        r_refresh<<<grid_for(C->n * 8), TB, 0, rst>>>(C->n, L->rld, L->rlen.as<int32_t>(), L->rcol.as<int32_t>(), L->ld,
                                                     L->pcol.as<int32_t>(), L->pval.as<double>(), L->rval.as<double>(),
                                                     L->rvalf.as<float>());
        NODAL_HIP_TRY(h, hipGetLastError());
        if (forked) NODAL_HIP_TRY(h, hipEventRecord(H->ev_join, H->aux));
        NODAL_TRY(galerkin_product<true>(h, H, l, forked ? H->ev_join : nullptr, forked ? 2 : 0));
        if (forked) H->aux_pending = false;
    }
    const int last = H->nlev - 1;
    if (H->dense_coarsest)
        coarsest_inverse<<<1, 256, 0, st>>>(H->pool[last]->A(), H->coarse_inv.as<double>(), dstats + (size_t)last * ST_COUNT);
    if (H->tail >= 0) k_tail_pack<<<1, 1024, 0, st>>>(H->td, H->tail_image.as<char>());
    NODAL_HIP_TRY(h, hipGetLastError());
    NODAL_TRY(form_tail_op(h, H));
    NODAL_HIP_TRY(h, hipMemcpyAsync(hs, dstats, (size_t)MAX_LEVELS * ST_COUNT * 8, hipMemcpyDeviceToHost, st));
    NODAL_WAIT_STREAM(h, st);
    const int64_t bar = n0 / 100 < 32 ? (n0 / 100 > 0 ? n0 / 100 : 1) : 32;
    if (hs[ST_BADDIAG] || (int64_t)hs[ST_GRADED] >= bar) return NODAL_OK;
    for (int k = 1; k < H->nlev; ++k)
        if (hs[(size_t)k * ST_COUNT + ST_BADDIAG] || hs[(size_t)k * ST_COUNT + ST_OVERFLOW]) return NODAL_OK;
    decide_folds(H, hs, false);
    NODAL_TRY(fold_self_check(h, H));
    *ok = true;
    return NODAL_OK;
}

}

void sagg_destroy(nodal_ctx *h) {
    delete static_cast<SHierarchy *>(h->sagg);
    h->sagg = nullptr;
}

static int sagg_setup_csr_body(nodal_ctx *h, int64_t n0, int64_t nnz0, const int32_t *indptr0, const int32_t *indices0,
                               const double *data0, bool general, bool check_floating, bool *accepted, int32_t *floating);

int sagg_setup_csr(nodal_ctx *h, int64_t n0, int64_t nnz0, const int32_t *indptr0, const int32_t *indices0,
                   const double *data0, bool general, bool check_floating, bool *accepted, int32_t *floating) {
    const int s = sagg_setup_csr_body(h, n0, nnz0, indptr0, indices0, data0, general, check_floating, accepted, floating);
    SHierarchy *H = static_cast<SHierarchy *>(h->sagg);
    if (H && H->aux && H->aux_pending && H->ev_flags) {
        if (hipEventRecord(H->ev_flags, H->aux) == hipSuccess) (void)hipStreamWaitEvent(h->stream, H->ev_flags, 0);
        H->aux_pending = false;
        (void)hipGetLastError();
    }
    return s;
}

static int sagg_setup_csr_body(nodal_ctx *h, int64_t n0, int64_t nnz0, const int32_t *indptr0, const int32_t *indices0,
                               const double *data0, bool general, bool check_floating, bool *accepted, int32_t *floating) {
    *accepted = false;
    *floating = 0;
    static const bool enabled = !(getenv("NODAL_SAGG") && atoi(getenv("NODAL_SAGG")) == 0);
    static const bool trace = getenv("NODAL_TRACE") != nullptr;
    if (!enabled) return NODAL_OK;
    SHierarchy *H = hierarchy_of(h);
    H->ready = false;
    hipStream_t st = h->stream;
    if (n0 >= (1ll << 30)) return NODAL_OK;
    static const bool reuse = !(getenv("NODAL_SA_REUSE") && atoi(getenv("NODAL_SA_REUSE")) == 0);
    if (reuse && H->sym_valid && H->sym_epoch == h->struct_epoch && H->sym_n == n0 && H->sym_nnz == nnz0 &&
        H->sym_general == general && H->sym_check == check_floating) {
        bool ok = false;
        NODAL_TRY(sagg_refresh(h, H, indptr0, indices0, data0, general, &ok));
        if (ok) {
            *floating = H->sym_floating;
            H->refreshed = true;
            H->ready = true;
            *accepted = true;
            if (trace) fprintf(stderr, "[sagg] symbolic setup kept (struct epoch %llu): values refreshed\n",
                               (unsigned long long)h->struct_epoch);
            return NODAL_OK;
        }
        if (trace) fprintf(stderr, "[sagg] the kept hierarchy does not take the new values: full setup\n");
    }
    H->sym_valid = false;
    H->refreshed = false;
    H->want_flags = check_floating;
    H->flags_levels = 0;
    H->last_iters = 0;
    H->drop_graph();
    NODAL_HIP_TRY(h, H->stats.reserve((size_t)MAX_LEVELS * ST_COUNT * 8 + 64));
    if (!H->host_stats)
        NODAL_HIP_TRY(h, hipHostMalloc(reinterpret_cast<void **>(&H->host_stats), (size_t)MAX_LEVELS * ST_COUNT * 8 + 64));
    unsigned long long *dstats = H->stats.as<unsigned long long>();
    unsigned long long *hs = reinterpret_cast<unsigned long long *>(H->host_stats);
    NODAL_HIP_TRY(h, hipMemsetAsync(dstats, 0, (size_t)MAX_LEVELS * ST_COUNT * 8, st));
    NODAL_HIP_TRY(h, H->bstat.reserve((size_t)2 * BSTAT_MAX * 4 + 64));
    {
        const unsigned gr = grid_for(n0);
        static const double spread = getenv("NODAL_SA_SPREAD") ? atof(getenv("NODAL_SA_SPREAD")) : 16.0;
        static const double share = getenv("NODAL_SA_SHARE") ? atof(getenv("NODAL_SA_SHARE")) : 0.9;
        row_stats<<<gr, TB, 0, st>>>(n0, indptr0, indices0, data0, share, spread, general, dstats, H->bstat.as<uint32_t>());
        reduce_bstat<<<1, 1024, 0, st>>>((int)gr, H->bstat.as<uint32_t>(), dstats, ST_MAXLEN, ST_GRADED);
    }
    NODAL_HIP_TRY(h, hipGetLastError());
    NODAL_HIP_TRY(h, hipMemcpyAsync(hs, dstats, ST_COUNT * 8, hipMemcpyDeviceToHost, st));
    NODAL_WAIT_STREAM(h, st);
    const int64_t bar = n0 / 100 < 32 ? (n0 / 100 > 0 ? n0 / 100 : 1) : 32;
    if (hs[ST_MAXLEN] > (unsigned long long)W0_MAX || hs[ST_MAXLEN] == 0 || hs[ST_BADDIAG] ||
        (int64_t)hs[ST_GRADED] >= bar) {
        if (trace)
            fprintf(stderr, "[sagg] declined: longest row %llu, graded nodes %llu (bar %lld), M-matrix %s\n",
                    hs[ST_MAXLEN], hs[ST_GRADED], (long long)bar, hs[ST_BADDIAG] ? "no" : "yes");
        return NODAL_OK;
    }
    SLevel *L0 = H->level(0);
    L0->n = n0;
    L0->ld = pad64(n0);
    L0->maxlen = (int32_t)hs[ST_MAXLEN];
    L0->nnz = nnz0;
    L0->wfix = choose_wfix(L0->maxlen, n0, nnz0, 8);
    L0->width = L0->wfix ? L0->wfix : L0->maxlen;
    NODAL_HIP_TRY(h, L0->acol.reserve((size_t)L0->width * L0->ld * 4 + 64));
    NODAL_HIP_TRY(h, L0->aval.reserve((size_t)L0->width * L0->ld * 8 + 64));
    NODAL_HIP_TRY(h, L0->avalf.reserve((size_t)L0->width * L0->ld * 4 + 64));
    NODAL_HIP_TRY(h, L0->alen.reserve((size_t)L0->ld * 4 + 64));
    NODAL_HIP_TRY(h, L0->dinv.reserve((size_t)L0->ld * 8 + 64));
    static const bool d16_env = !(getenv("NODAL_SA_D16") && atoi(getenv("NODAL_SA_D16")) == 0);
    L0->d16 = d16_env && hs[ST_FARCOL] == 0;
    if (L0->d16) NODAL_HIP_TRY(h, L0->adcol.reserve((size_t)L0->width * L0->ld * 2 + 64));
    csr_to_ell<<<grid_for(n0), TB, 0, st>>>(n0, L0->ld, indptr0, indices0, data0, L0->acol.as<int32_t>(),
                                           L0->aval.as<double>(), L0->avalf.as<float>(),
                                           L0->alen.as<int32_t>(), L0->dinv.as<double>(), L0->wfix,
                                           L0->d16 ? L0->adcol.as<int16_t>() : nullptr);
    NODAL_HIP_TRY(h, hipGetLastError());

    int l = 0;
    bool diag_last = false;
    for (;; ++l) {
        SLevel *L = H->level(l);
        if (L->n <= COARSEST && l > 0) break;
        if (l + 1 >= MAX_LEVELS) {
            if (trace) fprintf(stderr, "[sagg] declined: more than %d levels\n", MAX_LEVELS);
            return NODAL_OK;
        }
        bool declined = false, stop = false;
        NODAL_TRY(build_level(h, H, l, hs, &declined, &stop));
        if (declined) {
            if (trace)
                fprintf(stderr, "[sagg] declined at level %d (%lld rows): does not coarsen / over a cap / not positive "
                                "(this level: overflow %llx baddiag %llx; level above: overflow %llx unassigned %llu maxr %llu)\n",
                        l, (long long)L->n, hs[(size_t)l * ST_COUNT + ST_OVERFLOW], hs[(size_t)l * ST_COUNT + ST_BADDIAG],
                        l > 0 ? hs[(size_t)(l - 1) * ST_COUNT + ST_OVERFLOW] : 0ull,
                        l > 0 ? hs[(size_t)(l - 1) * ST_COUNT + ST_UNASSIGNED] : 0ull,
                        l > 0 ? hs[(size_t)(l - 1) * ST_COUNT + ST_MAXR] : 0ull);
            return NODAL_OK;
        }
        if (stop) {
            diag_last = true;
            break;
        }
    }
    H->nlev = l + 1;
    SLevel *last = H->level(l);
    last->fold_want = last->fold = false;
    if (H->nlev < 2) return NODAL_OK;
    NODAL_HIP_TRY(h, hipMemcpyAsync(hs, dstats, (size_t)MAX_LEVELS * ST_COUNT * 8, hipMemcpyDeviceToHost, st));
    if (!H->ev_copy) NODAL_HIP_TRY(h, hipEventCreateWithFlags(&H->ev_copy, hipEventDisableTiming));
    NODAL_HIP_TRY(h, hipEventRecord(H->ev_copy, st));
    if (check_floating) {
        if (H->flags_levels == 0) {
            NODAL_HIP_TRY(h, H->level(0)->gflag.reserve((size_t)n0 + 64));
            NODAL_TRY(grounded_flags(h, H->level(0)->gflag.as<uint8_t>()));
        } else {
            NODAL_HIP_TRY(h, hipStreamWaitEvent(st, H->ev_flags, 0));
            H->aux_pending = false;
        }
        for (int k = H->flags_levels; k + 1 < H->nlev; ++k) {
            SLevel *L = H->pool[k], *C = H->pool[k + 1];
            NODAL_HIP_TRY(h, C->gflag.reserve((size_t)C->n + 64));
            NODAL_HIP_TRY(h, hipMemsetAsync(C->gflag.p, 0, ((size_t)C->n + 63) & ~(size_t)63, st));
            flags_up<<<grid_for(L->n), TB, 0, st>>>(L->n, L->agg.as<int32_t>(), L->gflag.as<uint8_t>(),
                                                   C->gflag.as<uint8_t>());
        }
        NODAL_HIP_TRY(h, hipGetLastError());
    }
    NODAL_WAIT_EVENT(h, H->ev_copy, st);
    for (int k = 0; k < H->nlev; ++k) {
        const unsigned long long *s = hs + (size_t)k * ST_COUNT;
        if (k > 0) {
            H->pool[k]->maxlen = (int32_t)s[ST_MAXLEN];
            H->pool[k]->nnz = (int64_t)s[ST_NNZ];
            H->pool[k]->wfix = choose_wfix(H->pool[k]->maxlen, H->pool[k]->n, H->pool[k]->nnz, APAD);
        }
        if (s[ST_OVERFLOW] || (k > 0 && s[ST_BADDIAG]) || s[ST_UNASSIGNED]) {
            if (trace) fprintf(stderr, "[sagg] declined: level %d over a cap / not positive\n", k);
            return NODAL_OK;
        }
    }
    diag_last = last->maxlen <= 1;
    H->dense_coarsest = !diag_last;
    if (H->dense_coarsest) {
        if (last->n > COARSEST) return NODAL_OK;
        NODAL_HIP_TRY(h, H->coarse_inv.reserve((size_t)last->n * last->n * 8 + 64));
        coarsest_inverse<<<1, 256, 0, st>>>(last->A(), H->coarse_inv.as<double>(),
                                            dstats + (size_t)l * ST_COUNT);
        NODAL_HIP_TRY(h, hipGetLastError());
    }
    for (int k = 0; k < H->nlev; ++k) {
        SLevel *L = H->pool[k];
        NODAL_HIP_TRY(h, L->vec.reserve((size_t)V_COUNT * L->ld * 8 + 256));
        NODAL_HIP_TRY(h, L->part.reserve(5 * DOT_BLOCKS * 8 + 512));
    }
    NODAL_TRY(build_tail(h, H, hs));

    if (!check_floating) {
        NODAL_HIP_TRY(h, hipMemcpyAsync(hs, dstats, (size_t)MAX_LEVELS * ST_COUNT * 8, hipMemcpyDeviceToHost, st));
        NODAL_WAIT_STREAM(h, st);
        if (hs[(size_t)l * ST_COUNT + ST_BADDIAG] & 2ull) return NODAL_OK;
    } else {
        uint32_t *fl = reinterpret_cast<uint32_t *>(dstats + (size_t)(MAX_LEVELS - 1) * ST_COUNT + ST_COUNT - 1);
        if (H->dense_coarsest) last_level_floating<<<1, 64, 0, st>>>(last->A(), last->gflag.as<uint8_t>(), fl);
        else any_unflagged<<<grid_for(last->n), TB, 0, st>>>(last->n, last->gflag.as<uint8_t>(), fl);
        NODAL_HIP_TRY(h, hipGetLastError());
        NODAL_HIP_TRY(h, hipMemcpyAsync(hs, dstats, (size_t)MAX_LEVELS * ST_COUNT * 8, hipMemcpyDeviceToHost, st));
        NODAL_WAIT_STREAM(h, st);
        if (hs[(size_t)l * ST_COUNT + ST_BADDIAG] & 2ull) {
            if (trace) fprintf(stderr, "[sagg] declined: coarsest matrix not positive definite\n");
            return NODAL_OK;
        }
        *floating = hs[(size_t)(MAX_LEVELS - 1) * ST_COUNT + ST_COUNT - 1] != 0 ? 1 : 0;
    }
    if (trace) {
        fprintf(stderr, "[sagg] levels (rows/entries/longest row/padded width):");
        for (int k = 0; k < H->nlev; ++k)
            fprintf(stderr, " %lld/%lld/%d/%d", (long long)H->pool[k]->n, (long long)H->pool[k]->nnz,
                    H->pool[k]->maxlen, H->pool[k]->wfix);
        fprintf(stderr, "  tail %d (%d register slots)  coarsest %s\n", H->tail, H->tail >= 0 ? H->td.slots : 0,
                H->dense_coarsest ? "dense" : "diagonal");
    }
    decide_folds(H, hs, trace);
    NODAL_TRY(fold_self_check(h, H));
    H->ready = true;
    *accepted = true;
    H->sym_valid = true;
    H->sym_epoch = h->struct_epoch;
    H->sym_n = n0;
    H->sym_nnz = nnz0;
    H->sym_general = general;
    H->sym_check = check_floating;
    H->sym_floating = *floating;
    memcpy(H->sym_stats, hs, sizeof H->sym_stats);
    return NODAL_OK;
}

int sagg_setup(nodal_ctx *h, bool *accepted, int32_t *floating) {
    return sagg_setup_csr(h, h->n, h->nnz, h->indptr.as<int32_t>(), h->indices.as<int32_t>(), h->data.as<double>(),
                          false, true, accepted, floating);
}

namespace {

int last_level(nodal_ctx *h, SHierarchy *H, int l, const double *b, double *out) {
    hipStream_t st = h->stream;
    SLevel *L = H->pool[l];
    const int64_t n = L->n;
    if (l == H->tail) return H->tail_dense ? tail_apply<1>(h, H, b, out) : tail_walk(h, H, b, out, 1);
    k_coarsest<<<grid_for(n), TB, 0, st>>>(n, H->dense_coarsest ? H->coarse_inv.as<double>() : nullptr,
                                           L->dinv.as<double>(), b, out);
    NODAL_HIP_TRY(h, hipGetLastError());
    return NODAL_OK;
}

void kcycle_schedule(SHierarchy *H, int it) {
    static const bool on = !(getenv("NODAL_SA_KFREEZE") && atoi(getenv("NODAL_SA_KFREEZE")) == 0);
    H->kfrozen = false;
    H->kslot = -1;
    if (!on || it < 0) return;
    if (it == 0) H->ksamples = 0;
    const bool adaptive = it < 4 || (it & 3) == 0;
    if (!adaptive && H->ksamples > 0) {
        H->kfrozen = true;
    } else if (it >= 2) {
        H->kslot = H->ksamples % 3;
        ++H->ksamples;
        H->kcount = H->ksamples < 3 ? H->ksamples : 3;
    }
}

template <typename TBV, typename TOUT>
int cycle(nodal_ctx *h, SHierarchy *H, int l, const TBV *b, const cyc_t *x0, TOUT *out, const SolveBufs *sb) {
    hipStream_t st = h->stream;
    SLevel *L = H->pool[l];
    const int64_t n = L->n;
    SLevel *C = H->pool[l + 1];
    const int64_t nc = C->n;
    const Ell A = L->A();
    const double *dinv = L->dinv.as<double>();
    const cyc_t *x = x0;
    cyc_t *r = L->v<cyc_t>(V_R), *xp = L->v<cyc_t>(V_XP);
    const unsigned g = sb ? (unsigned)sb->g0 : grid_for(n);
    const unsigned tb = L->wfix ? TB : TB * LPR_RAGGED;
    const int nu = H->nu[l < 2 ? l : 2];
    const bool fold = L->fold && !(sb && nu == 1);
    auto hand_up = [&](const auto *c1, const auto *c2, const double *cf) {
        using TC = std::remove_cv_t<std::remove_pointer_t<decltype(c1)>>;
        if (!fold)
            k_prolong<TC><<<grid_for(n), TB, 0, st>>>(n, L->ld, L->pcol.as<int32_t>(), L->pvalf.as<float>(), x, c1, c2, cf, xp);
        else if (nu == 1)
            k_prolong_post<TC, TOUT><<<grid_for(n), TB, 0, st>>>(n, L->ld, L->wcol.as<int32_t>(), L->wval.as<float>(),
                                                               L->wlen.as<int32_t>(), x, r, dinv, c1, c2, cf, out);
        else
            k_prolong_post<TC, cyc_t><<<grid_for(n), TB, 0, st>>>(n, L->ld, L->wcol.as<int32_t>(), L->wval.as<float>(),
                                                                L->wlen.as<int32_t>(), x, r, dinv, c1, c2, cf, xp);
    };
    if (nu >= 2) {
        cyc_t *x1 = L->v<cyc_t>(V_X1);
        SAGG_DISPATCH_W(L->wfix, (k_post<W, false, TBV, cyc_t><<<g, tb, 0, st>>>(A, dinv, b, x0, x1, nullptr, nullptr, nullptr)));
        x = x1;
    }
    if (nu >= 3) {
        cyc_t *x2 = L->v<cyc_t>(V_T);
        SAGG_DISPATCH_W(L->wfix, (k_post<W, false, TBV, cyc_t><<<g, tb, 0, st>>>(A, dinv, b, x, x2, nullptr, nullptr, nullptr)));
        x = x2;
    }
    SAGG_DISPATCH_W(L->wfix, (k_smooth_residual<W, TBV><<<g, tb, 0, st>>>(A, b, x, r)));
    const bool last = l + 1 == H->tail || l + 1 == H->nlev - 1;
    const double *coef = nullptr;
    if (last) {
        double *rc = C->v<double>(V_RC), *c1 = C->v<double>(V_C1);
        k_restrict<double><<<grid_for(nc * RL), TB, 0, st>>>(nc, L->rld, L->rcol.as<int32_t>(), L->rvalf.as<float>(),
                                                            L->rlen.as<int32_t>(), r, rc, C->dinv.as<double>(), nullptr);
        NODAL_HIP_TRY(h, hipGetLastError());
        NODAL_TRY(last_level(h, H, l + 1, rc, c1));
        hand_up((const double *)c1, (const double *)nullptr, nullptr);
    } else {
        cyc_t *rc = C->v<cyc_t>(V_RC), *c1 = C->v<cyc_t>(V_C1), *c2 = C->v<cyc_t>(V_C2), *x0c = C->v<cyc_t>(V_X);
        k_restrict<cyc_t><<<grid_for(nc * RL), TB, 0, st>>>(nc, L->rld, L->rcol.as<int32_t>(), L->rvalf.as<float>(),
                                                           L->rlen.as<int32_t>(), r, rc, C->dinv.as<double>(), x0c);
        NODAL_HIP_TRY(h, hipGetLastError());
        int nparts = 0;
        const bool kcycle = l < H->klevels && H->kcycle;
        if (kcycle) {
            cyc_t *v1 = C->v<cyc_t>(V_V1), *v2 = C->v<cyc_t>(V_V2), *r2 = C->v<cyc_t>(V_R2);
            double *part = C->part.as<double>();
            const Ell Ac = C->A();
            const unsigned gd = grid_for(nc, DOT_BLOCKS);
            const unsigned tbc = C->wfix ? TB : TB * LPR_RAGGED;
            nparts = (int)gd;
            double *cf = part + 5 * DOT_BLOCKS;
            if (H->kfrozen && l == 0) {
                NODAL_TRY((cycle<cyc_t, cyc_t>(h, H, l + 1, rc, x0c, c1, nullptr)));
                SAGG_DISPATCH_W(C->wfix, (k_spmv_resid<W><<<gd, tbc, 0, st>>>(Ac, c1, rc, cf + 3, r2, C->dinv.as<double>(), x0c)));
                NODAL_HIP_TRY(h, hipGetLastError());
                NODAL_TRY((cycle<cyc_t, cyc_t>(h, H, l + 1, r2, x0c, c2, nullptr)));
                coef = cf + 3;
                nparts = 0;
            } else {
                NODAL_TRY((cycle<cyc_t, cyc_t>(h, H, l + 1, rc, x0c, c1, nullptr)));
                SAGG_DISPATCH_W(C->wfix, (k_spmv_dots<W><<<gd, tbc, 0, st>>>(Ac, c1, v1, rc, nullptr, part + 0 * DOT_BLOCKS,
                                                                            part + 1 * DOT_BLOCKS, nullptr)));
                k_second_residual<<<grid_for(nc), TB, 0, st>>>(nc, rc, v1, part, nparts, r2, C->dinv.as<double>(), x0c);
                NODAL_HIP_TRY(h, hipGetLastError());
                NODAL_TRY((cycle<cyc_t, cyc_t>(h, H, l + 1, r2, x0c, c2, nullptr)));
                SAGG_DISPATCH_W(C->wfix, (k_spmv_dots<W><<<gd, tbc, 0, st>>>(Ac, c2, v2, v1, r2, part + 3 * DOT_BLOCKS,
                                                                            part + 2 * DOT_BLOCKS, part + 4 * DOT_BLOCKS)));
                NODAL_HIP_TRY(h, hipGetLastError());
            }
        } else {
            NODAL_TRY((cycle<cyc_t, cyc_t>(h, H, l + 1, rc, x0c, c1, nullptr)));
        }
        if (nparts) {
            double *cf = C->part.as<double>() + 5 * DOT_BLOCKS;
            const bool sample = l == 0 && H->kslot >= 0;
            k_kcoef<<<1, 320, 0, st>>>(C->part.as<double>(), nparts, cf, sample ? H->kslot : -1, sample ? H->kcount : 0);
            coef = cf;
        }
        hand_up((const cyc_t *)c1, (const cyc_t *)c2, coef);
    }
    const cyc_t *cur = xp;
    const int left = fold ? nu - 1 : nu;
    if (left == 0) {
        NODAL_HIP_TRY(h, hipGetLastError());
        return NODAL_OK;
    }
    if (left >= 2) {
        cyc_t *mid = L->v<cyc_t>(V_T);
        SAGG_DISPATCH_W(L->wfix, (k_post<W, false, TBV, cyc_t><<<g, tb, 0, st>>>(A, dinv, b, cur, mid, nullptr, nullptr, nullptr)));
        cur = mid;
    }
    if (left >= 3) {
        cyc_t *mid2 = L->v<cyc_t>(V_X1);
        SAGG_DISPATCH_W(L->wfix, (k_post<W, false, TBV, cyc_t><<<g, tb, 0, st>>>(A, dinv, b, cur, mid2, nullptr, nullptr, nullptr)));
        cur = mid2;
    }
    if (sb) {
        SAGG_DISPATCH_W(L->wfix, (k_post<W, true, TBV, TOUT><<<g, tb, 0, st>>>(A, dinv, b, cur, out, sb->Ap, sb->part_rz,
                                                                              sb->part_zap)));
    } else {
        SAGG_DISPATCH_W(L->wfix, (k_post<W, false, TBV, TOUT><<<g, tb, 0, st>>>(A, dinv, b, cur, out, nullptr, nullptr, nullptr)));
    }
    NODAL_HIP_TRY(h, hipGetLastError());
    return NODAL_OK;
}

__global__ void f_set_scalars(double *__restrict__ sc, double tol2) {
    for (int k = 0; k < F_COUNT; ++k) sc[k] = 0.0;
    sc[F_TOL2] = tol2;
}

size_t align_up(size_t x) { return (x + 255) & ~(size_t)255; }

}

__global__ __launch_bounds__(TB) void k_x0(int64_t n, const double *__restrict__ dinv, const double *__restrict__ r,
                                           cyc_t *__restrict__ x0) {
    for (int64_t i = (int64_t)xcd_block() * TB + threadIdx.x; i < n; i += (int64_t)gridDim.x * TB)
        x0[i] = (cyc_t)(OMEGA * dinv[i] * r[i]);
}
bool sagg_ready(nodal_ctx *h, int64_t n) {
    SHierarchy *H = static_cast<SHierarchy *>(h->sagg);
    return H && H->ready && H->pool[0]->n == n;
}
void sagg_invalidate(nodal_ctx *h) {
    if (h->sagg) static_cast<SHierarchy *>(h->sagg)->ready = false;
}
int sagg_levels(nodal_ctx *h) { return h->sagg ? static_cast<SHierarchy *>(h->sagg)->nlev : 0; }
bool sagg_x0_slot(nodal_ctx *h, const double **dinv, nodal_cyc_t **x0, int64_t *n0, double *omega) {
    SHierarchy *H = static_cast<SHierarchy *>(h->sagg);
    if (!H || !H->ready) return false;
    SLevel *L0 = H->pool[0];
    *dinv = L0->dinv.as<double>();
    *x0 = L0->v<cyc_t>(V_X);
    *n0 = L0->n;
    *omega = OMEGA;
    return true;
}
int sagg_apply(nodal_ctx *h, const double *r, double *z, bool x0_ready, int it) {
    SHierarchy *H = static_cast<SHierarchy *>(h->sagg);
    if (!H || !H->ready) return nodal_fail(h, NODAL_E_INVALID, "sagg_setup_csr not called");
    SLevel *L0 = H->pool[0];
    cyc_t *x0 = L0->v<cyc_t>(V_X);
    if (!x0_ready) k_x0<<<grid_for(L0->n), TB, 0, h->stream>>>(L0->n, L0->dinv.as<double>(), r, x0);
    NODAL_HIP_TRY(h, hipGetLastError());
    kcycle_schedule(H, it);
    const int rc = cycle<double, double>(h, H, 0, r, x0, z, nullptr);
    H->kfrozen = false;
    H->kslot = -1;
    return rc;
}

int sagg_spmv(nodal_ctx *h, const double *x, double *y, hipEvent_t start, hipEvent_t stop) {
    SHierarchy *H = static_cast<SHierarchy *>(h->sagg);
    if (!H || !H->ready) return nodal_fail(h, NODAL_E_INVALID, "sagg_setup_csr not called");
    const SLevel *L0 = H->pool[0];
    const Ell A0 = L0->A();
    const unsigned tb0 = L0->wfix ? TB : TB * LPR_RAGGED;
    if (start && stop) {
        SAGG_DISPATCH_W(L0->wfix, (hipExtLaunchKernelGGL((k_ell_spmv<W>), dim3(grid_for(L0->n)), dim3(tb0), 0, h->stream,
                                                         start, stop, 0, A0, x, y)));
    } else {
        SAGG_DISPATCH_W(L0->wfix, (k_ell_spmv<W><<<grid_for(L0->n), tb0, 0, h->stream>>>(A0, x, y)));
    }
    NODAL_HIP_TRY(h, hipGetLastError());
    return NODAL_OK;
}

int sagg_fcg_solve(nodal_ctx *h, const double *b, bool do_setup, int32_t *info, int32_t *iters, double *resid) {
    static const bool trace = getenv("NODAL_TRACE") != nullptr;
    const int64_t n = h->n;
    hipStream_t st = h->stream;
    SHierarchy *H = hierarchy_of(h);
    if (do_setup) {
        bool accepted = false;
        int32_t floating = 0;
        NODAL_TRY(sagg_setup(h, &accepted, &floating));
        if (!accepted) return SAGG_DECLINED;
        if (floating) {
            *info = 1;
            *iters = 0;
            *resid = 0.0;
            return -2;
        }
    }
    if (!H->ready || H->pool[0]->n != n) return SAGG_DECLINED;
    h->amg_levels = H->nlev;
    static const int kc = getenv("NODAL_SA_KCYCLE") ? atoi(getenv("NODAL_SA_KCYCLE")) : 1;
    H->kcycle = kc != 0;
    H->klevels = getenv("NODAL_SA_KLEVELS") ? atoi(getenv("NODAL_SA_KLEVELS")) : 1;
    if (const char *e = getenv("NODAL_SA_NU")) {
        for (int k = 0; k < 3 && e[k] >= '1' && e[k] <= '3'; ++k) H->nu[k] = e[k] - '0';
    }

    const size_t vec = align_up((size_t)n * 8);
    NODAL_HIP_TRY(h, h->solver.reserve(6 * vec + 4 * MAX_PARTIALS * 8 + F_COUNT * 8 + 256));
    char *base = h->solver.as<char>();
    SolveBufs sb;
    sb.r = reinterpret_cast<double *>(base);
    sb.z = reinterpret_cast<cyc_t *>(base + vec);
    sb.p = reinterpret_cast<double *>(base + 2 * vec);
    sb.Ap = reinterpret_cast<double *>(base + 3 * vec);
    sb.x0 = reinterpret_cast<cyc_t *>(base + 4 * vec);
    sb.p2 = reinterpret_cast<double *>(base + 5 * vec);
    sb.part_rz = reinterpret_cast<double *>(base + 6 * vec);
    sb.part_zap = sb.part_rz + MAX_PARTIALS;
    sb.part_rr = sb.part_zap + MAX_PARTIALS;
    sb.part_pap = sb.part_rr + MAX_PARTIALS;
    sb.sc = sb.part_pap + MAX_PARTIALS;
    sb.g0 = (int)grid_for(n, MAX_PARTIALS);
    double *x = h->x.as<double>();
    const Ell A0 = H->pool[0]->A();

    const double tol = 1e-13;
    f_set_scalars<<<1, 1, 0, st>>>(sb.sc, tol * tol);
    const double *dinv0 = H->pool[0]->dinv.as<double>();
    f_init<<<sb.g0, TB, 0, st>>>(b, x, sb.r, sb.Ap, dinv0, sb.x0, sb.part_rr, n);
    NODAL_HIP_TRY(h, hipGetLastError());

    const int64_t maxit = getenv("NODAL_FCG_MAXIT") ? atoll(getenv("NODAL_FCG_MAXIT")) : 2000;
    hipEvent_t e0 = h->ev[2], e1 = h->ev[3];
    h->kern_ms = 0;
    h->kern_launches = 0;
    double hs[F_COUNT];
    int64_t enqueued = 0;
    int batch = 6;
    if (H->last_iters > 6 && (H->refreshed || !do_setup)) batch = H->last_iters + 1 > 32 ? 32 : H->last_iters + 1;
    else if (H->hint_iters > 8 && H->hint_n == n && H->hint_nnz == H->pool[0]->nnz) {
        batch = (3 * H->hint_iters) / 4;
        if (batch > 32) batch = 32;
    }
    int status = 0;
    const bool poll_partials = !(getenv("NODAL_FCG_HOST_SUM") && atoi(getenv("NODAL_FCG_HOST_SUM")) == 0);
    double rr_prev = -1.0;
    int64_t it_prev = 0;
    int polls = 0;
    static const bool fuse_dir_env = !(getenv("NODAL_SA_FUSE_DIR") && atoi(getenv("NODAL_SA_FUSE_DIR")) == 0);
    const bool fuse_dir = fuse_dir_env && LPR_RAGGED == 1;
    static const bool graphs_env = getenv("NODAL_SA_GRAPH") && atoi(getenv("NODAL_SA_GRAPH")) != 0;
    auto iteration = [&](int it, bool timed) -> int {
        kcycle_schedule(H, graphs_env ? -1 : it);
        struct KReset {
            SHierarchy *H;
            ~KReset() { H->kfrozen = false; H->kslot = -1; }
        } kreset{H};
        NODAL_TRY((cycle<double, cyc_t>(h, H, 0, sb.r, sb.x0, sb.z, &sb)));
        if (fuse_dir) {
            double *p_new = (it & 1) ? sb.p2 : sb.p;
            const double *p_old = (it & 1) ? sb.p : sb.p2;
            const unsigned tbf = TB;
            if (timed) {
                SAGG_DISPATCH_W(H->pool[0]->wfix, (hipExtLaunchKernelGGL((f_dir_spmv<W>), dim3(sb.g0), dim3(tbf), 0, st, e0, e1, 0,
                                                                         A0, (const cyc_t *)sb.z, p_old, p_new, sb.Ap,
                                                                         (const double *)sb.part_rz, (const double *)sb.part_zap,
                                                                         (const double *)sb.part_rr, sb.g0, sb.part_pap, sb.sc,
                                                                         it & 1)));
            } else {
                SAGG_DISPATCH_W(H->pool[0]->wfix, (f_dir_spmv<W><<<sb.g0, tbf, 0, st>>>(A0, sb.z, p_old, p_new, sb.Ap, sb.part_rz,
                                                                                       sb.part_zap, sb.part_rr, sb.g0,
                                                                                       sb.part_pap, sb.sc, it & 1)));
            }
            f_update<<<sb.g0, TB, 0, st>>>(x, sb.r, p_new, sb.Ap, sb.part_pap, sb.g0, dinv0, sb.x0, sb.part_rr, sb.sc, it & 1, n);
            NODAL_HIP_TRY(h, hipGetLastError());
            return NODAL_OK;
        }
        f_direction<<<sb.g0, TB, 0, st>>>(sb.z, sb.p, sb.part_rz, sb.part_zap, sb.part_rr, sb.g0, sb.sc, it & 1, n);
        const unsigned tb0 = H->pool[0]->wfix ? TB : TB * LPR_RAGGED;
        if (timed) {
            SAGG_DISPATCH_W(H->pool[0]->wfix, (hipExtLaunchKernelGGL((f_spmv<W>), dim3(sb.g0), dim3(tb0), 0, st, e0, e1, 0,
                                                                     A0, (const double *)sb.p, sb.Ap, sb.part_pap,
                                                                     (const double *)sb.sc, it & 1)));
        } else {
            SAGG_DISPATCH_W(H->pool[0]->wfix, (f_spmv<W><<<sb.g0, tb0, 0, st>>>(A0, sb.p, sb.Ap, sb.part_pap, sb.sc, it & 1)));
        }
        f_update<<<sb.g0, TB, 0, st>>>(x, sb.r, sb.p, sb.Ap, sb.part_pap, sb.g0, dinv0, sb.x0, sb.part_rr, sb.sc, it & 1, n);
        NODAL_HIP_TRY(h, hipGetLastError());
        return NODAL_OK;
    };
    static const bool graphs = getenv("NODAL_SA_GRAPH") && atoi(getenv("NODAL_SA_GRAPH")) != 0;
    if (graphs && (H->refreshed || !do_setup)) {
        uint64_t key = 1469598103934665603ull;
        auto mix = [&](uint64_t v) { key = (key ^ v) * 1099511628211ull; };
        mix((uint64_t)(uintptr_t)base); mix((uint64_t)(uintptr_t)x); mix((uint64_t)n); mix((uint64_t)sb.g0);
        mix((uint64_t)H->nlev); mix((uint64_t)(H->tail + 1)); mix((uint64_t)H->kcycle); mix((uint64_t)H->klevels);
        mix((uint64_t)(H->nu[0] * 100 + H->nu[1] * 10 + H->nu[2])); mix((uint64_t)H->td.lds_bytes);
        mix((uint64_t)(uintptr_t)H->tail_image.p); mix((uint64_t)(uintptr_t)H->coarse_inv.p);
        mix((uint64_t)(uintptr_t)(H->tail_dense ? H->tail_op.p : nullptr));
        for (int k = 0; k < H->nlev; ++k) {
            const SLevel *L = H->pool[k];
            const void *ps[] = {L->acol.p, L->aval.p, L->avalf.p, L->alen.p, L->dinv.p, L->pcol.p, L->pvalf.p,
                                L->rcol.p, L->rvalf.p, L->rlen.p, L->vec.p, L->part.p};
            for (const void *q : ps) mix((uint64_t)(uintptr_t)q);
            mix((uint64_t)(L->fold ? 1 + L->wslots : 0));
            if (L->fold) { mix((uint64_t)(uintptr_t)L->wcol.p); mix((uint64_t)(uintptr_t)L->wval.p); mix((uint64_t)(uintptr_t)L->wlen.p); }
            mix((uint64_t)L->n); mix((uint64_t)L->ld); mix((uint64_t)L->wfix); mix((uint64_t)L->rld);
        }
        if (H->it_exec && H->it_key != key) H->drop_graph();
        if (!H->it_exec) {
            hipGraph_t g = nullptr;
            hipGraphExec_t ex = nullptr;
            if (hipStreamBeginCapture(st, hipStreamCaptureModeThreadLocal) == hipSuccess) {
                int cs = iteration(0, false);
                if (cs == NODAL_OK) cs = iteration(1, false);
                const hipError_t ce = hipStreamEndCapture(st, &g);
                if (cs == NODAL_OK && ce == hipSuccess && g && hipGraphInstantiate(&ex, g, nullptr, nullptr, 0) == hipSuccess) {
                    H->it_graph = g;
                    H->it_exec = ex;
                    H->it_key = key;
                } else {
                    if (g) (void)hipGraphDestroy(g);
                    (void)hipGetLastError();
                }
            } else {
                (void)hipGetLastError();
            }
        }
    } else if (H->it_exec && do_setup) {
        H->drop_graph();
    }
    while (status == 0) {
        for (int c = 0; c < batch;) {
            if (H->it_exec && c > 0 && c + 1 < batch && (enqueued & 1) == 0) {
                NODAL_HIP_TRY(h, hipGraphLaunch(H->it_exec, st));
                c += 2;
                enqueued += 2;
            } else {
                NODAL_TRY(iteration((int)enqueued, c == 0));
                ++c;
                ++enqueued;
            }
        }
        double rr_now = -1.0;
        {
            const size_t bytes = (size_t)(2 * MAX_PARTIALS + F_COUNT) * 8;
            double *stage = poll_partials ? static_cast<double *>(nodal_pinned_arena(h, bytes)) : nullptr;
            if (stage) {
                NODAL_HIP_TRY(h, hipMemcpyAsync(stage, sb.part_rr, bytes, hipMemcpyDeviceToHost, st));
                NODAL_WAIT_STREAM(h, st);
                memcpy(hs, stage + 2 * MAX_PARTIALS, F_COUNT * 8);
                double acc = 0.0;
                for (int k = 0; k < sb.g0; ++k) acc += stage[k];
                rr_now = acc;
            } else {
                NODAL_TRY(nodal_read_words(h, hs, sb.sc, F_COUNT * 8));
            }
        }
        ++polls;
        bool conv = hs[F_CONV + ((enqueued - 1) & 1)] != 0.0;
        bool host_conv = false;
        if (!conv && rr_now >= 0.0 && hs[F_FLAG] == 0.0 && hs[F_BB] > 0.0 && rr_now <= tol * tol * hs[F_BB]) {
            host_conv = true;
            hs[F_RR] = rr_now;
            hs[F_ITERS] = (double)enqueued;
        } else if (!conv && rr_now >= 0.0) {
            hs[F_RR] = rr_now;
        }
        float ms = 0;
        if (!(conv && !host_conv && hs[F_ITERS] <= (double)(enqueued - batch)) && hipEventElapsedTime(&ms, e0, e1) == hipSuccess) {
            h->kern_ms += ms;
            h->kern_launches += 1;
        }
        if (hs[F_FLAG] != 0.0 || !(hs[F_RR] == hs[F_RR])) status = 2;
        else if (conv || host_conv) status = 1;
        else if (enqueued >= maxit) status = 3;
        else {
            int next = 2;
            const double target = tol * tol * hs[F_BB];
            const double rr_ref = rr_prev > 0.0 ? rr_prev : hs[F_BB];
            const int64_t it_ref = rr_prev > 0.0 ? it_prev : 0;
            if (hs[F_RR] > 0.0 && hs[F_RR] < rr_ref && enqueued > it_ref) {
                const double rate = log(hs[F_RR] / rr_ref) / (double)(enqueued - it_ref);
                static const double look = getenv("NODAL_FCG_LOOK") ? atof(getenv("NODAL_FCG_LOOK")) : 0.75;
                next = (int)floor(look * log(target / hs[F_RR]) / rate);
            }
            if (next > enqueued) next = (int)enqueued;
            batch = next < 1 ? 1 : (next > 32 ? 32 : next);
            rr_prev = hs[F_RR];
            it_prev = enqueued;
        }
    }
    const int64_t its = status == 1 ? (int64_t)hs[F_ITERS] : enqueued;
    *iters = (int32_t)its;
    *resid = hs[F_BB] > 0 ? sqrt(hs[F_RR] / hs[F_BB]) : 0.0;
    const SLevel *L0 = H->pool[0];
    h->kern_alg = 12.0 * (double)L0->nnz + 4.0 * (double)n + 16.0 * (double)n;
    if (fuse_dir) h->kern_alg += 12.0 * (double)n;
    if (trace)
        fprintf(stderr, "[sagg] %d iterations (%lld enqueued, %d polls), relative residual %.2e, status %d\n", *iters,
                (long long)enqueued, polls, *resid, status);
    if (trace && H->tail >= 0 && H->td.stamps && !H->tail_dense) {
        long long ts[64];
        if (hipMemcpy(ts, H->td.stamps, sizeof ts, hipMemcpyDeviceToHost) == hipSuccess) {
            fprintf(stderr, "[sagg] tail phases (us):");
            for (int k = 1; k < (int)ts[63] && k < 63; ++k) fprintf(stderr, " %.2f", (double)(ts[k] - ts[k - 1]) * 0.01);
            fprintf(stderr, "  total %.2f, image %d B, lds %d B\n", (double)(ts[ts[63] - 1] - ts[0]) * 0.01,
                    H->td.image_bytes, H->td.lds_bytes);
            for (int k = 0; k < H->td.nlev; ++k)
                fprintf(stderr, "[sagg]   tail level %d: n %d width %d lpr %d nq %d\n", k, H->td.lv[k].n,
                        H->td.lv[k].width, H->td.lv[k].lpr, H->td.lv[k].nq);
        }
    }
    if (status != 1) {
        H->last_iters = 0;
        return -1;
    }
    H->last_iters = (int)its;
    H->hint_iters = (int)its;
    H->hint_n = n;
    H->hint_nnz = H->pool[0]->nnz;
    *info = 0;
    return NODAL_OK;
}

#include "sagg_multi.h"
```

nodal_amd/csrc/sagg_cycle.h:

```cpp
#pragma once

namespace {

constexpr int LPR_RAGGED = 1;
template <int W> struct RowLanes { static constexpr int value = W == 0 ? LPR_RAGGED : 1; };

template <class VT, class XF>
__device__ __forceinline__ double ell_row_lanes(const Ell &A, const VT *__restrict__ val, int64_t i, int sub, XF xf) {
    constexpr int Q = 8;
    const int32_t len = A.len[i];
    double acc = 0.0;
    for (int32_t s0 = sub; s0 < len; s0 += LPR_RAGGED * Q) {
        int32_t c[Q];
        double v[Q];
        if (A.dcol) {
#pragma unroll
            for (int q = 0; q < Q; ++q) {
                const bool ok = s0 + q * LPR_RAGGED < len;
                const int64_t at = (int64_t)(ok ? s0 + q * LPR_RAGGED : s0) * A.ld + i;
                c[q] = (int32_t)i + (int32_t)A.dcol[at];
                const VT loaded = val[at];
                v[q] = ok ? (double)loaded : 0.0;
            }
        } else {
// ... 73 lines not shown
    case 6: { constexpr int W = 6; CALL; } break;        \
    case 8: { constexpr int W = 8; CALL; } break;        \
    case 12: { constexpr int W = 12; CALL; } break;      \
    case 16: { constexpr int W = 16; CALL; } break;      \
    case 20: { constexpr int W = 20; CALL; } break;      \
    case 24: { constexpr int W = 24; CALL; } break;      \
    case 32: { constexpr int W = 32; CALL; } break;      \
    default: { constexpr int W = 0; CALL; } break;       \
    }

__device__ __forceinline__ double wave_sum(double v) {
#pragma unroll
    for (int off = 32; off > 0; off >>= 1) v += __shfl_down(v, off, 64);
    return v;
}
template <int NT = TB>
__device__ __forceinline__ double block_sum(double v) {
    __shared__ double ws[NT / 64];
    __syncthreads();
    v = wave_sum(v);
    if ((threadIdx.x & 63) == 0) ws[threadIdx.x >> 6] = v;
    __syncthreads();
    double s = 0.0;
#pragma unroll
    for (int w = 0; w < NT / 64; ++w) s += ws[w];
    return s;
}
__device__ __forceinline__ double reduce_partials(const double *__restrict__ part, int count) {
    double s = 0.0;
    for (int i = threadIdx.x; i < count; i += TB) s += part[i];
    return block_sum(s);
}
__device__ __forceinline__ void reduce_partials3(const double *__restrict__ pa, const double *__restrict__ pb,
                                                 const double *__restrict__ pc, int count, double &ra, double &rb,
                                                 double &rc) {
    __shared__ double ws[3][TB / 64];
    double a = 0.0, b = 0.0, c = 0.0;
    for (int i = threadIdx.x; i < count; i += TB) {
        a += pa[i];
        b += pb[i];
        if (pc) c += pc[i];
    }
    __syncthreads();
    a = wave_sum(a);
    b = wave_sum(b);
    c = wave_sum(c);
    if ((threadIdx.x & 63) == 0) {
        ws[0][threadIdx.x >> 6] = a;
        ws[1][threadIdx.x >> 6] = b;
        ws[2][threadIdx.x >> 6] = c;
    }
    __syncthreads();
    ra = rb = rc = 0.0;
#pragma unroll
    for (int w = 0; w < TB / 64; ++w) {
        ra += ws[0][w];
        rb += ws[1][w];
        rc += ws[2][w];
    }
}

template <int W, typename TBV>
__global__ __launch_bounds__(TB * RowLanes<W>::value) void k_smooth_residual(Ell A, const TBV *__restrict__ b,
                                                        const cyc_t *__restrict__ x0, cyc_t *__restrict__ r) {
    constexpr int LPR = RowLanes<W>::value, NT = TB * LPR;
    const int sub = threadIdx.x & (LPR - 1);
    for (int64_t t = (int64_t)xcd_block() * NT + threadIdx.x; t / LPR < A.n; t += (int64_t)gridDim.x * NT) {
        const int64_t i = t / LPR;
        const double s = ell_row_w<W>(A, A.valf, i, sub, [&](int32_t j) { return (double)x0[j]; });
        if (sub == 0) r[i] = (cyc_t)((double)b[i] - s);
    }
}

constexpr int RL = 8;
template <typename TO>
__global__ __launch_bounds__(TB) void k_restrict(int64_t nc, int64_t rld, const int32_t *__restrict__ rcol,
                                                 const float *__restrict__ rval, const int32_t *__restrict__ rlen,
                                                 const cyc_t *__restrict__ r, TO *__restrict__ rc,
                                                 const double *__restrict__ cdinv, cyc_t *__restrict__ x0c) {
    const int sub = threadIdx.x & (RL - 1);
    const int64_t rows_per_pass = (int64_t)gridDim.x * (TB / RL);
    for (int64_t I0 = (int64_t)xcd_block() * (TB / RL); I0 < nc; I0 += rows_per_pass) {
        const int64_t I = I0 + threadIdx.x / RL;
        double s = 0.0;
        if (I < nc) {
            const int32_t len = rlen[I];
            constexpr int RU = 6;
            for (int32_t q0 = 0; q0 * RL < len; q0 += RU) {
                int32_t c[RU];
                double v[RU];
#pragma unroll
                for (int u = 0; u < RU; ++u) {
                    const bool ok = (q0 + u) * RL < len;
                    const int64_t at = ((int64_t)(ok ? q0 + u : q0) * rld + I) * RL + sub;
                    c[u] = rcol[at];
                    const float loaded = rval[at];
                    v[u] = ok ? (double)loaded : 0.0;
                }
#pragma unroll
                for (int u = 0; u < RU; ++u) s = fma(v[u], (double)r[c[u]], s);
            }
        }
#pragma unroll
        for (int off = RL >> 1; off > 0; off >>= 1) s += __shfl_down(s, off, RL);
        if (I < nc && sub == 0) {
            rc[I] = (TO)s;
            if (x0c) x0c[I] = (cyc_t)(OMEGA * cdinv[I] * s);
        }
    }
}

struct KCoef { double s1, s2; };
__device__ __forceinline__ KCoef kcycle_coefficients(const double *__restrict__ part, int nparts) {
    if (nparts == 0) return KCoef{1.0, 0.0};
    const double rho1 = reduce_partials(part + 0 * DOT_BLOCKS, nparts);
    const double alpha1 = reduce_partials(part + 1 * DOT_BLOCKS, nparts);
    const double gamma = reduce_partials(part + 2 * DOT_BLOCKS, nparts);
    const double beta = reduce_partials(part + 3 * DOT_BLOCKS, nparts);
    const double alpha2 = reduce_partials(part + 4 * DOT_BLOCKS, nparts);
    if (!(rho1 > 0.0)) return KCoef{0.0, 0.0};
    const double rho2 = beta - gamma * gamma / rho1;
    if (!(rho2 > 0.0)) return KCoef{alpha1 / rho1, 0.0};
    return KCoef{alpha1 / rho1 - gamma * alpha2 / (rho1 * rho2), alpha2 / rho2};
}

__global__ __launch_bounds__(320) void k_kcoef(const double *__restrict__ part, int nparts, double *__restrict__ coef,
                                               int slot, int count) {
    __shared__ double d[5];
    const int w = threadIdx.x >> 6, lane = threadIdx.x & 63;
    double s = 0.0;
    for (int i = lane; i < nparts; i += 64) s += part[w * DOT_BLOCKS + i];
    s = wave_sum(s);
    if (lane == 0) d[w] = s;
    __syncthreads();
    if (threadIdx.x == 0) {
        const double rho1 = d[0], alpha1 = d[1], gamma = d[2], beta = d[3], alpha2 = d[4];
        double s1 = 0.0, s2 = 0.0;
        if (rho1 > 0.0) {
            const double rho2 = beta - gamma * gamma / rho1;
            if (rho2 > 0.0) {
                s1 = alpha1 / rho1 - gamma * alpha2 / (rho1 * rho2);
                s2 = alpha2 / rho2;
            } else {
                s1 = alpha1 / rho1;
            }
        }
        coef[0] = s1;
        coef[1] = s2;
        if (slot >= 0) {
            double *ring = coef + 6;
            ring[3 * slot + 0] = s1;
            ring[3 * slot + 1] = s2;
            ring[3 * slot + 2] = rho1 > 0.0 ? alpha1 / rho1 : 0.0;
            double m0 = 0.0, m1 = 0.0, m2 = 0.0;
            for (int q = 0; q < count; ++q) {
                m0 += ring[3 * q + 0];
                m1 += ring[3 * q + 1];
                m2 += ring[3 * q + 2];
            }
            coef[3] = m0 / count;
            coef[4] = m1 / count;
            coef[5] = m2 / count;
        }
    }
}

template <int W>
__global__ __launch_bounds__(TB * RowLanes<W>::value) void k_spmv_resid(Ell A, const cyc_t *__restrict__ c,
                                                   const cyc_t *__restrict__ rc, const double *__restrict__ frz,
                                                   cyc_t *__restrict__ r2, const double *__restrict__ dinv,
                                                   cyc_t *__restrict__ x0) {
    constexpr int LPR = RowLanes<W>::value, NT = TB * LPR;
    const int sub = threadIdx.x & (LPR - 1);
    const double t = frz[2];
    for (int64_t tt = (int64_t)xcd_block() * NT + threadIdx.x; tt / LPR < A.n; tt += (int64_t)gridDim.x * NT) {
        const int64_t i = tt / LPR;
        const double sd = ell_row_w<W>(A, A.valf, i, sub, [&](int32_t j) { return (double)c[j]; });
        if (sub != 0) continue;
        const double v = fma(-t, (double)(cyc_t)sd, (double)rc[i]);
        r2[i] = (cyc_t)v;
        x0[i] = (cyc_t)(OMEGA * dinv[i] * v);
    }
}

template <typename TC>
__global__ __launch_bounds__(TB) void k_prolong(int64_t n, int64_t ld, const int32_t *__restrict__ pcol,
                                                const float *__restrict__ pval, const cyc_t *__restrict__ x,
                                                const TC *__restrict__ c1, const TC *__restrict__ c2,
                                                const double *__restrict__ coef, cyc_t *__restrict__ xp) {
    const bool two = coef != nullptr;
    const double s1 = two ? coef[0] : 1.0, s2 = two ? coef[1] : 0.0;
    for (int64_t i = (int64_t)xcd_block() * TB + threadIdx.x; i < n; i += (int64_t)gridDim.x * TB) {
        int32_t J[PW];
        double w[PW];
#pragma unroll
        for (int q = 0; q < PW; ++q) {
            J[q] = pcol[(int64_t)q * ld + i];
            w[q] = (double)pval[(int64_t)q * ld + i];
        }
        double s = (double)x[i];
#pragma unroll
        for (int q = 0; q < PW; ++q) {
            const int32_t j = J[q] < 0 ? 0 : J[q];
            const double e = two ? s1 * (double)c1[j] + s2 * (double)c2[j] : (double)c1[j];
            s = fma(J[q] < 0 ? 0.0 : w[q], e, s);
        }
        xp[i] = (cyc_t)s;
    }
}

template <int W, bool DOTS, typename TBV, typename TOUT>
__global__ __launch_bounds__(TB * RowLanes<W>::value) void k_post(Ell A, const double *__restrict__ dinv, const TBV *__restrict__ b,
                                             const cyc_t *__restrict__ xp, TOUT *__restrict__ out,
                                             const double *__restrict__ u, double *__restrict__ p_ob,
                                             double *__restrict__ p_ou) {
    double a0 = 0.0, a1 = 0.0;
    constexpr int LPR = RowLanes<W>::value, NT = TB * LPR;
    const int sub = threadIdx.x & (LPR - 1);
    for (int64_t t = (int64_t)xcd_block() * NT + threadIdx.x; t / LPR < A.n; t += (int64_t)gridDim.x * NT) {
        const int64_t i = t / LPR;
        const double s = ell_row_w<W>(A, A.valf, i, sub, [&](int32_t j) { return (double)xp[j]; });
        if (sub != 0) continue;
        const double bi = (double)b[i];
        const TOUT os = (TOUT)fma(OMEGA * dinv[i], bi - s, (double)xp[i]);
        const double o = (double)os;
        out[i] = os;
        if (DOTS) {
            a0 = fma(o, bi, a0);
            a1 = fma(o, u[i], a1);
        }
    }
    if (DOTS) {
        a0 = block_sum<NT>(a0);
        a1 = block_sum<NT>(a1);
        if (threadIdx.x == 0) {
            p_ob[blockIdx.x] = a0;
            p_ou[blockIdx.x] = a1;
        }
    }
}

template <typename TC, typename TOUT>
__global__ __launch_bounds__(TB) void k_prolong_post(int64_t n, int64_t ld, const int32_t *__restrict__ wcol,
                                                     const float *__restrict__ wval, const int32_t *__restrict__ wlen,
                                                     const cyc_t *__restrict__ x, const cyc_t *__restrict__ r,
                                                     const double *__restrict__ dinv, const TC *__restrict__ c1,
                                                     const TC *__restrict__ c2, const double *__restrict__ coef,
                                                     TOUT *__restrict__ out) {
    constexpr int Q = 8;
    const bool two = coef != nullptr;
    const double s1 = two ? coef[0] : 1.0, s2 = two ? coef[1] : 0.0;
    for (int64_t i = (int64_t)xcd_block() * TB + threadIdx.x; i < n; i += (int64_t)gridDim.x * TB) {
        const int32_t len = wlen[i];
        const cyc_t xi = x[i], ri = r[i];
        const double di = dinv[i];
        double acc = 0.0;
        for (int32_t s0 = 0; s0 < len; s0 += Q) {
            int32_t J[Q];
            double w[Q];
#pragma unroll
            for (int q = 0; q < Q; ++q) {
                const bool ok = s0 + q < len;
                const int64_t at = (int64_t)(ok ? s0 + q : s0) * ld + i;
                J[q] = wcol[at];
                const float loaded = wval[at];
                w[q] = ok ? (double)loaded : 0.0;
            }
#pragma unroll
            for (int q = 0; q < Q; ++q) {
                const double e = two ? s1 * (double)c1[J[q]] + s2 * (double)c2[J[q]] : (double)c1[J[q]];
                acc = fma(w[q], e, acc);
            }
        }
        out[i] = (TOUT)(fma(OMEGA * di, (double)ri, (double)xi) + acc);
    }
}

template <typename TC>
__global__ __launch_bounds__(TB) void k_fold_check(Ell A, const double *__restrict__ dinv, const cyc_t *__restrict__ b,
                                                   const cyc_t *__restrict__ x, const cyc_t *__restrict__ xp,
                                                   const int32_t *__restrict__ wcol, const float *__restrict__ wval,
                                                   const int32_t *__restrict__ wlen, const TC *__restrict__ c1,
                                                   const TC *__restrict__ c2, const double *__restrict__ coef,
                                                   const cyc_t *__restrict__ m_two, const cyc_t *__restrict__ m_fused,
                                                   double *__restrict__ d, double *__restrict__ q) {
    const bool two = coef != nullptr;
    const double s1 = two ? coef[0] : 1.0, s2 = two ? coef[1] : 0.0;
    for (int64_t i = (int64_t)xcd_block() * TB + threadIdx.x; i < A.n; i += (int64_t)gridDim.x * TB) {
        double ax = 0.0, we = 0.0;
        const int32_t la = A.len[i], lw = wlen[i];
        for (int32_t s = 0; s < la; ++s)
            ax += fabs((double)A.valf[(int64_t)s * A.ld + i]) * fabs((double)xp[A.col[(int64_t)s * A.ld + i]]);
        for (int32_t s = 0; s < lw; ++s) {
            const int32_t j = wcol[(int64_t)s * A.ld + i];
            const double e = two ? s1 * (double)c1[j] + s2 * (double)c2[j] : (double)c1[j];
            we += fabs((double)wval[(int64_t)s * A.ld + i]) * fabs(e);
        }
        const double den = fabs((double)x[i]) + OMEGA * dinv[i] * (fabs((double)b[i]) + ax) + we;
        const double diff = fabs((double)m_fused[i] - (double)m_two[i]);
        const double di = diff / den;
        d[i] = di;
        q[i] = di / ((double)(lw + la + 8) * 0x1p-23);
    }
}

template <int W>
__global__ __launch_bounds__(TB * RowLanes<W>::value) void k_spmv_dots(Ell A, const cyc_t *__restrict__ c, cyc_t *__restrict__ v,
                                                  const cyc_t *__restrict__ u1, const cyc_t *__restrict__ u2,
                                                  double *__restrict__ p_cv, double *__restrict__ p_cu1,
                                                  double *__restrict__ p_cu2) {
    double a0 = 0.0, a1 = 0.0, a2 = 0.0;
    constexpr int LPR = RowLanes<W>::value, NT = TB * LPR;
    const int sub = threadIdx.x & (LPR - 1);
    for (int64_t t = (int64_t)xcd_block() * NT + threadIdx.x; t / LPR < A.n; t += (int64_t)gridDim.x * NT) {
        const int64_t i = t / LPR;
        const double sd = ell_row_w<W>(A, A.valf, i, sub, [&](int32_t j) { return (double)c[j]; });
        if (sub != 0) continue;
        const cyc_t vs = (cyc_t)sd;
        v[i] = vs;
        const double s = (double)vs, ci = (double)c[i];
        a0 = fma(ci, s, a0);
        a1 = fma(ci, (double)u1[i], a1);
        if (u2) a2 = fma(ci, (double)u2[i], a2);
    }
    a0 = block_sum<NT>(a0);
    a1 = block_sum<NT>(a1);
    a2 = block_sum<NT>(a2);
    if (threadIdx.x == 0) {
        p_cv[blockIdx.x] = a0;
        p_cu1[blockIdx.x] = a1;
        if (p_cu2) p_cu2[blockIdx.x] = a2;
    }
}

__global__ __launch_bounds__(TB) void k_second_residual(int64_t n, const cyc_t *__restrict__ rc,
                                                        const cyc_t *__restrict__ v1,
                                                        const double *__restrict__ part, int nparts,
                                                        cyc_t *__restrict__ r2, const double *__restrict__ dinv,
                                                        cyc_t *__restrict__ x0) {
    double rho1, alpha1, unused;
    reduce_partials3(part + 0 * DOT_BLOCKS, part + 1 * DOT_BLOCKS, nullptr, nparts, rho1, alpha1, unused);
    const double t = rho1 > 0.0 ? alpha1 / rho1 : 0.0;
    for (int64_t i = (int64_t)xcd_block() * TB + threadIdx.x; i < n; i += (int64_t)gridDim.x * TB)
    {
        const double v = fma(-t, (double)v1[i], (double)rc[i]);
        r2[i] = (cyc_t)v;
        x0[i] = (cyc_t)(OMEGA * dinv[i] * v);
    }
}

__global__ __launch_bounds__(TB) void k_coarsest(int64_t n, const double *__restrict__ inv,
                                                 const double *__restrict__ dinv, const double *__restrict__ b,
                                                 double *__restrict__ out) {
    for (int64_t i = (int64_t)xcd_block() * TB + threadIdx.x; i < n; i += (int64_t)gridDim.x * TB) {
        double s = 0.0;
        if (inv)
            for (int64_t j = 0; j < n; ++j) s = fma(inv[i * n + j], b[j], s);
        else
            s = dinv[i] * b[i];
        out[i] = s;
    }
}



__device__ __forceinline__ double lds_row(const double *aval, const uint16_t *acol, int n, int width, int i,
                                          int sub, int lpr, const double *x) {
    double s0 = 0.0, s1 = 0.0;
    int t = sub;
    for (; t + 3 * lpr < width; t += 4 * lpr) {
        const double v0 = aval[t * n + i], v1 = aval[(t + lpr) * n + i], v2 = aval[(t + 2 * lpr) * n + i],
                     v3 = aval[(t + 3 * lpr) * n + i];
        const int c0 = acol[t * n + i], c1 = acol[(t + lpr) * n + i], c2 = acol[(t + 2 * lpr) * n + i],
                  c3 = acol[(t + 3 * lpr) * n + i];
        s0 = fma(v0, x[c0], s0);
        s1 = fma(v1, x[c1], s1);
        s0 = fma(v2, x[c2], s0);
        s1 = fma(v3, x[c3], s1);
    }
    for (; t < width; t += lpr) s0 = fma(aval[t * n + i], x[acol[t * n + i]], s0);
    double s = s0 + s1;
    for (int off = lpr >> 1; off > 0; off >>= 1) s += __shfl_xor(s, off, 64);
    return s;
}

__global__ __launch_bounds__(1024) void k_tail_pack(TailDesc d, char *__restrict__ image) {
    const int tid = threadIdx.x;
    const int last = d.nlev - 1;
    auto f64 = [&](int off) { return reinterpret_cast<double *>(image + off); };
    auto u16 = [&](int off) { return reinterpret_cast<uint16_t *>(image + off); };
    auto copy_f64 = [&](double *dst, const double *src, int rows, int64_t ld, int slots) {
        for (int e = tid; e < rows * slots; e += 1024) {
            const int t = e / rows, i = e - t * rows;
            dst[e] = src[(int64_t)t * ld + i];
        }
    };
    auto copy_u16 = [&](uint16_t *dst, const int32_t *src, int rows, int64_t ld, int slots) {
        for (int e = tid; e < rows * slots; e += 1024) {
            const int t = e / rows, i = e - t * rows;
            const int32_t v = src[(int64_t)t * ld + i];
            dst[e] = (uint16_t)(v < 0 ? 0 : v);
        }
    };
    for (int k = 0; k < last; ++k) {
        const TailLevelDesc &L = d.lv[k];
        for (int e = tid; e < L.n * L.width; e += 1024) {
            const int t = e / L.n, i = e - t * L.n;
            const bool in = t < L.alen[i];
            f64(L.o_aval)[e] = in ? L.aval[(int64_t)t * L.ld + i] : 0.0;
            const int32_t c = in ? L.acol[(int64_t)t * L.ld + i] : 0;
            u16(L.o_acol)[e] = (uint16_t)(c < 0 ? 0 : c);
        }
        copy_f64(f64(L.o_dinv), L.dinv, L.n, L.ld, 1);
        copy_f64(f64(L.o_pval), L.pval, L.n, L.ld, PW);
        copy_u16(u16(L.o_pcol), L.pcol, L.n, L.ld, PW);
        copy_f64(f64(L.o_rval), L.rval, L.nc * RL, (int64_t)L.rld * RL, L.nq);
        copy_u16(u16(L.o_rcol), L.rcol, L.nc * RL, (int64_t)L.rld * RL, L.nq);
    }
    const TailLevelDesc &L = d.lv[last];
    if (d.inv) copy_f64(f64(L.o_aval), d.inv, L.n * L.n, L.n * L.n, 1);
    else copy_f64(f64(L.o_aval), L.dinv, L.n, L.n, 1);
}

template <int SLOTS>
__device__ __forceinline__ double reg_row(const double (&v)[SLOTS], const uint32_t (&c)[SLOTS / 2], int lpr,
                                          const double *x) {
    double s0 = 0.0, s1 = 0.0;
#pragma unroll
    for (int j = 0; j < SLOTS; j += 2) {
        s0 = fma(v[j], x[c[j / 2] & 0xffffu], s0);
        s1 = fma(v[j + 1], x[c[j / 2] >> 16], s1);
    }
    double s = s0 + s1;
    for (int off = lpr >> 1; off > 0; off >>= 1) s += __shfl_xor(s, off, 64);
    return s;
}

template <int SLOTS, bool UNIT>
__device__ __forceinline__ void tail_cycle(const TailDesc &d, char *smem, const char *__restrict__ image,
                                           const double *__restrict__ rc, double *__restrict__ out, int vs, int voff) {
    const int tid = threadIdx.x;
    const int last = d.nlev - 1;
    const int TAIL_NU = d.nu;
    auto f64 = [&](int off) { return reinterpret_cast<double *>(smem + (off - d.skip)); };
    auto u16 = [&](int off) { return reinterpret_cast<uint16_t *>(smem + (off - d.skip)); };
    int stamp_no = 0;
    auto stamp = [&]() {
        if (!UNIT && d.stamps && tid == 0) d.stamps[stamp_no] = wall_clock64();
        ++stamp_no;
    };
    stamp();
    double v0[SLOTS];
    uint32_t c0[SLOTS / 2];
    {
        const TailLevelDesc &L = d.lv[0];
        const double *aval = reinterpret_cast<const double *>(image + L.o_aval);
        const uint16_t *acol = reinterpret_cast<const uint16_t *>(image + L.o_acol);
        const int lpr = L.lpr, sub = tid & (lpr - 1), i = tid / lpr, ii = i < L.n ? i : L.n - 1;
        const bool row = last > 0 && i < L.n;
#pragma unroll
        for (int j = 0; j < SLOTS; j += 2) {
            const int ta = sub + j * lpr, tb = ta + lpr;
            const bool ha = row && ta < L.width, hb = row && tb < L.width;
            const int ea = ha ? ta * L.n + ii : 0, eb = hb ? tb * L.n + ii : 0;
            const double va = aval[ea], vb = aval[eb];
            const uint32_t ca = acol[ea], cb = acol[eb];
            v0[j] = ha ? va : 0.0;
            v0[j + 1] = hb ? vb : 0.0;
            c0[j / 2] = (ha ? ca : 0u) | ((hb ? cb : 0u) << 16);
        }
    }
    {
        constexpr int FLY = (TAIL_LDS_BUDGET / 16 + 1023) / 1024;
        const int4 *src = reinterpret_cast<const int4 *>(image + d.skip);
        int4 *dst = reinterpret_cast<int4 *>(smem);
        const int pieces = (d.image_bytes - d.skip) / 16;
        int4 v[FLY];
#pragma unroll
        for (int u = 0; u < FLY; ++u) v[u] = src[tid + u * 1024 < pieces ? tid + u * 1024 : 0];
#pragma unroll
        for (int u = 0; u < FLY; ++u)
            if (tid + u * 1024 < pieces) dst[tid + u * 1024] = v[u];
    }
    for (;;) {
        for (int i = tid; i < d.lv[0].n; i += 1024)
            f64(d.lv[0].o_B)[i] = UNIT ? (i == voff ? 1.0 : 0.0) : rc[(int64_t)i * vs + voff];
        __syncthreads();
        stamp();
        for (int k = 0; k < last; ++k) {
            const TailLevelDesc &L = d.lv[k];
            const double *aval = f64(L.o_aval), *dinv = f64(L.o_dinv), *B = f64(L.o_B);
            const uint16_t *acol = u16(L.o_acol);
            double *X = f64(L.o_X), *Y = f64(L.o_Y), *R = f64(L.o_R);
            const int lpr = L.lpr, sub = tid & (lpr - 1), rows = 1024 / lpr;
            for (int i = tid; i < L.n; i += 1024) X[i] = OMEGA * dinv[i] * B[i];
            __syncthreads();
            for (int sweep = 1; sweep < TAIL_NU; ++sweep) {
                for (int i0 = 0; i0 < L.n; i0 += rows) {
                    const int i = i0 + tid / lpr, ii = i < L.n ? i : L.n - 1;
                    const double ax = k == 0 ? reg_row<SLOTS>(v0, c0, lpr, X)
                                             : lds_row(aval, acol, L.n, L.width, ii, sub, lpr, X);
                    if (i < L.n && sub == 0) Y[i] = fma(OMEGA * dinv[i], B[i] - ax, X[i]);
                }
                __syncthreads();
                double *t = X; X = Y; Y = t;
            }
            for (int i0 = 0; i0 < L.n; i0 += rows) {
                const int i = i0 + tid / lpr, ii = i < L.n ? i : L.n - 1;
                const double ax = k == 0 ? reg_row<SLOTS>(v0, c0, lpr, X)
                                         : lds_row(aval, acol, L.n, L.width, ii, sub, lpr, X);
                if (i < L.n && sub == 0) R[i] = B[i] - ax;
            }
            __syncthreads();
            stamp();
            const double *rval = f64(L.o_rval);
            const uint16_t *rcol = u16(L.o_rcol);
            double *Bc = f64(d.lv[k + 1].o_B);
            for (int I0 = 0; I0 < L.nc; I0 += 1024 / RL) {
                const int I = I0 + tid / RL, r8 = tid & (RL - 1);
                double s = 0.0;
                if (I < L.nc) {
                    double s1 = 0.0;
                    const int e0 = I * RL + r8, step = L.nc * RL;
                    int q = 0;
                    for (; q + 3 < L.nq; q += 4) {
                        const int ea = e0 + q * step, eb = ea + step, ec = eb + step, ed = ec + step;
                        const double va = rval[ea], vb = rval[eb], vc = rval[ec], vd = rval[ed];
                        const int ca = rcol[ea], cb = rcol[eb], cc = rcol[ec], cd = rcol[ed];
                        s = fma(va, R[ca], s);
                        s1 = fma(vb, R[cb], s1);
                        s = fma(vc, R[cc], s);
                        s1 = fma(vd, R[cd], s1);
                    }
                    for (; q < L.nq; ++q) s = fma(rval[e0 + q * step], R[rcol[e0 + q * step]], s);
                    s += s1;
                }
#pragma unroll
                for (int off = RL >> 1; off > 0; off >>= 1) s += __shfl_xor(s, off, 64);
                if (I < L.nc && r8 == 0) Bc[I] = s;
            }
            __syncthreads();
            stamp();
        }
        {
            const TailLevelDesc &L = d.lv[last];
            const double *inv = f64(L.o_aval), *B = f64(L.o_B);
            double *E = f64(L.o_X);
            for (int i = tid; i < L.n; i += 1024) {
                double s = 0.0;
                if (d.inv) {
                    double s1 = 0.0, s2 = 0.0, s3 = 0.0;
                    const double *row = inv + i * L.n;
                    int j = 0;
                    for (; j + 3 < L.n; j += 4) {
                        s = fma(row[j], B[j], s);
                        s1 = fma(row[j + 1], B[j + 1], s1);
                        s2 = fma(row[j + 2], B[j + 2], s2);
                        s3 = fma(row[j + 3], B[j + 3], s3);
                    }
                    for (; j < L.n; ++j) s = fma(row[j], B[j], s);
                    s = (s + s1) + (s2 + s3);
                } else {
                    s = inv[i] * B[i];
                }
                E[i] = s;
            }
            __syncthreads();
            stamp();
        }
        const double *Ec = f64(d.lv[last].o_X);
        for (int k = last - 1; k >= 0; --k) {
            const TailLevelDesc &L = d.lv[k];
            const double *aval = f64(L.o_aval), *dinv = f64(L.o_dinv), *B = f64(L.o_B), *pval = f64(L.o_pval);
            const uint16_t *acol = u16(L.o_acol), *pcol = u16(L.o_pcol);
            double *X = f64((TAIL_NU & 1) ? L.o_X : L.o_Y), *Y = f64((TAIL_NU & 1) ? L.o_Y : L.o_X);
            for (int i = tid; i < L.n; i += 1024) {
                double s = X[i];
#pragma unroll
                for (int q = 0; q < PW; ++q) s = fma(pval[q * L.n + i], Ec[pcol[q * L.n + i]], s);
                Y[i] = s;
            }
            __syncthreads();
            stamp();
            const int lpr = L.lpr, sub = tid & (lpr - 1), rows = 1024 / lpr;
            for (int sweep = 0; sweep < TAIL_NU; ++sweep) {
                for (int i0 = 0; i0 < L.n; i0 += rows) {
                    const int i = i0 + tid / lpr, ii = i < L.n ? i : L.n - 1;
                    const double ax = k == 0 ? reg_row<SLOTS>(v0, c0, lpr, Y)
                                             : lds_row(aval, acol, L.n, L.width, ii, sub, lpr, Y);
                    if (i < L.n && sub == 0) X[i] = fma(OMEGA * dinv[i], B[i] - ax, Y[i]);
                }
                __syncthreads();
                double *t = X; X = Y; Y = t;
            }
            Ec = Y;
            stamp();
        }
        for (int i = tid; i < d.lv[0].n; i += 1024) out[(int64_t)i * vs + voff] = Ec[i];
        stamp();
        voff += (int)gridDim.x;
        if (!UNIT || voff >= d.lv[0].n) break;
        __syncthreads();
    }
    if (!UNIT && d.stamps && tid == 0) d.stamps[63] = stamp_no;
}

// ... 276 lines not shown
```

Measured before the change: 164.6 circuits/s.

## Fold pre/post smoothing sweep pairs into single launches via precomputed E2 and V operators

Builds extra per-level operators during setup. E2 folds two Jacobi pre-smoothing sweeps, and V folds the post-smoothing pair together with the prolongation correction. Each smoothing pair in the V-cycle can then run as one fused kernel instead of two SpMV passes. Setup kernels build these operators with hash-based row accumulation and can run on the aux stream. Error checks decide per level whether the fold is kept. The cost is more setup work, extra memory, float-precision folded operators and wider rows per fused pass. By default this applies only to coarse levels below a row threshold, so the finest 1e6 level may not use it.

```diff
diff --git a/nodal_amd/csrc/sagg.hip b/nodal_amd/csrc/sagg.hip
--- a/nodal_amd/csrc/sagg.hip
+++ b/nodal_amd/csrc/sagg.hip
@@ -62,7 +62,9 @@
        ST_MAXR = 6, ST_NC = 7 ,
        ST_FARCOL = 8 ,
        ST_FOLDMISS = 9 ,
-       ST_COUNT = 10 };
+       ST_E2MISS = 10 ,
+       ST_VMISS = 11 ,
+       ST_COUNT = 12 };
 
 struct SLevel {
     int64_t n = 0, ld = 0, nc = 0;
@@ -81,6 +83,9 @@
     DevBuf wcol, wval, wlen;
     int32_t wslots = 0;
     bool fold_want = false, fold = false;
+    DevBuf ecol, eval, elen, vcol, vval, vlen;
+    int32_t eslots = 0;
+    bool pre_want = false, v_want = false, fold_pre = false, fold_v = false;
     Ell A() const {
         Ell e;
         e.n = n; e.ld = ld; e.width = width;
@@ -130,6 +135,8 @@
     hipEvent_t ev_copy = nullptr;
     hipStream_t aux = nullptr;
     hipEvent_t ev_fork = nullptr, ev_join = nullptr, ev_flags = nullptr;
+    hipEvent_t ev_w = nullptr, ev_fold = nullptr;
+    bool fold_aux = false;
     bool aux_pending = false;
     bool aux_tried = false;
     bool want_flags = false;
@@ -169,11 +176,13 @@
         if (ev_fork) (void)hipEventDestroy(ev_fork);
         if (ev_join) (void)hipEventDestroy(ev_join);
         if (ev_flags) (void)hipEventDestroy(ev_flags);
+        if (ev_w) (void)hipEventDestroy(ev_w);
+        if (ev_fold) (void)hipEventDestroy(ev_fold);
         if (aux) (void)hipStreamDestroy(aux);
         for (SLevel *l : pool) {
             DevBuf *b[] = {&l->acol, &l->aval, &l->alen, &l->dinv, &l->agg, &l->pcol, &l->pval, &l->rcol,
                            &l->rval, &l->rlen, &l->vec, &l->part, &l->gflag, &l->avalf, &l->pvalf, &l->rvalf, &l->adcol,
-                           &l->wcol, &l->wval, &l->wlen};
+                           &l->wcol, &l->wval, &l->wlen, &l->ecol, &l->eval, &l->elen, &l->vcol, &l->vval, &l->vlen};
             for (DevBuf *x : b) x->release();
             delete l;
         }
@@ -839,6 +848,243 @@
     }
     if (overflow) atomicOr(&stats[ST_OVERFLOW], 4ull);
     if (miss) stats[ST_FOLDMISS] = 1ull;
+}
+
+template <bool SQUARE>
+__global__ __launch_bounds__(64) void fold_rows(Ell A, const double *__restrict__ dinv, const int32_t *__restrict__ wcol,
+                                                const float *__restrict__ wval, const int32_t *__restrict__ wlen,
+                                                int32_t *__restrict__ ocol, float *__restrict__ oval,
+                                                int32_t *__restrict__ olen, int cap, unsigned long long *__restrict__ flag) {
+    constexpr int SLOTS = 16;
+    __shared__ double tv[SLOTS * 64];
+    __shared__ int32_t tc[SLOTS * 64];
+    const int lane = threadIdx.x;
+    bool bad = false;
+    for (int64_t i0 = (int64_t)xcd_block() * 64; i0 < A.n; i0 += (int64_t)gridDim.x * 64) {
+        const int64_t i = i0 + lane;
+#pragma unroll 8
+        for (int q = 0; q < SLOTS; ++q) tc[q * 64 + lane] = -1;
+        if (i >= A.n) continue;
+        int cnt = 0;
+        auto put = [&](int32_t c, double t) {
+            uint32_t slot = ((uint32_t)c * 2654435761u) >> 16 & (SLOTS - 1);
+            for (int probe = 0; probe < SLOTS; ++probe) {
+                const int32_t have = tc[slot * 64 + lane];
+                if (have == c) {
+                    tv[slot * 64 + lane] += t;
+                    return;
+                }
+                if (have < 0) {
+                    tc[slot * 64 + lane] = c;
+                    tv[slot * 64 + lane] = t;
+                    ++cnt;
+                    return;
+                }
+                slot = (slot + 1) & (SLOTS - 1);
+            }
+            bad = true;
+        };
+        auto add_row = [&](int64_t k, int32_t lk, double coef) {
+            constexpr int Q = 8;
+            for (int32_t s0 = 0; s0 < lk; s0 += Q) {
+                int32_t c[Q];
+                double v[Q];
+#pragma unroll
+                for (int u = 0; u < Q; ++u) {
+                    const int64_t at = (int64_t)(s0 + u < lk ? s0 + u : s0) * A.ld + k;
+                    c[u] = SQUARE ? A.col[at] : wcol[at];
+                    v[u] = SQUARE ? A.val[at] : (double)wval[at];
+                }
+#pragma unroll
+                for (int u = 0; u < Q; ++u)
+                    if (s0 + u < lk) put(c[u], coef * v[u]);
+            }
+        };
+        const int32_t l = A.len[i];
+        const double di = OMEGA * dinv[i];
+        add_row(i, SQUARE ? l : wlen[i], SQUARE ? -2.0 : 1.0);
+        constexpr int AB = 4;
+        for (int32_t s0 = 0; s0 < l; s0 += AB) {
+            int32_t kk[AB], lk[AB];
+            double aa[AB], dk[AB];
+#pragma unroll
+            for (int u = 0; u < AB; ++u) {
+                const int32_t su = s0 + u < l ? s0 + u : s0;
+                kk[u] = A.col[(int64_t)su * A.ld + i];
+                aa[u] = A.val[(int64_t)su * A.ld + i];
+            }
+#pragma unroll
+            for (int u = 0; u < AB; ++u) {
+                lk[u] = SQUARE ? A.len[kk[u]] : wlen[kk[u]];
+                dk[u] = SQUARE ? OMEGA * dinv[kk[u]] : 0.0;
+            }
+#pragma unroll
+            for (int u = 0; u < AB; ++u)
+                if (s0 + u < l) add_row(kk[u], lk[u], SQUARE ? aa[u] * dk[u] : -di * aa[u]);
+        }
+        int o = 0;
+        bool diag = false;
+        for (int q = 0; q < SLOTS; ++q) {
+            const int32_t c = tc[q * 64 + lane];
+            if (c < 0) continue;
+            const double t = tv[q * 64 + lane];
+            if (SQUARE) {
+                const int64_t at = ((int64_t)(o / 8) * A.ld + i) * 8 + o % 8;
+                ocol[at] = c;
+                oval[at] = (float)((c == (int32_t)i ? 1.0 : 0.0) + OMEGA * dinv[c] * t);
+                diag = diag || c == (int32_t)i;
+            } else {
+                ocol[(int64_t)o * A.ld + i] = c;
+                oval[(int64_t)o * A.ld + i] = (float)t;
+            }
+            ++o;
+        }
+        if (SQUARE) {
+            for (int p = o; p % 8 != 0; ++p) {
+                const int64_t at = ((int64_t)(p / 8) * A.ld + i) * 8 + p % 8;
+                ocol[at] = (int32_t)i;
+                oval[at] = 0.0f;
+            }
+            if (!diag) bad = true;
+        }
+        olen[i] = cnt;
+        if (cnt > cap) bad = true;
+    }
+    if (bad) *flag = 1ull;
+}
+
+template <int SLOTS, bool SQUARE>
+__global__ __launch_bounds__(64) void fold_rows_wave(Ell A, const double *__restrict__ dinv, const int32_t *__restrict__ wcol,
+                                                     const float *__restrict__ wval, const int32_t *__restrict__ wlen,
+                                                     int32_t *__restrict__ ocol, float *__restrict__ oval,
+                                                     int32_t *__restrict__ olen, int cap,
+                                                     unsigned long long *__restrict__ flag) {
+    static_assert(SLOTS % 64 == 0, "every lane owns SLOTS / 64 slots of the set");
+    constexpr int LIST = 1536, PER = SLOTS / 64;
+    __shared__ int32_t tc[SLOTS];
+    __shared__ int32_t pc[LIST];
+    __shared__ double pv[LIST];
+    __shared__ int full;
+    const int lane = threadIdx.x;
+    bool bad = false;
+    for (int64_t i = blockIdx.x; i < A.n; i += gridDim.x) {
+        __syncthreads();
+        for (int q = lane; q < SLOTS; q += 64) tc[q] = -1;
+        if (lane == 0) full = 0;
+        const int32_t l = A.len[i] < 64 ? A.len[i] : 64;
+        const double di = OMEGA * dinv[i];
+        int32_t k = (int32_t)i, lk = 0;
+        double coef = 0.0;
+        if (lane < l) {
+            k = A.col[(int64_t)lane * A.ld + i];
+            const double a = A.val[(int64_t)lane * A.ld + i];
+            lk = SQUARE ? A.len[k] : wlen[k];
+            coef = SQUARE ? a * (OMEGA * dinv[k]) : -di * a;
+        }
+        const int32_t l0 = SQUARE ? l : wlen[i];
+        int tot;
+        const int off = l0 + wave_excl_scan(lk, &tot);
+        tot += l0;
+        if (tot > LIST || A.len[i] > 64) {
+            bad = true;
+            if (lane == 0) olen[i] = 0;
+            continue;
+        }
+        if (lane < l0) {
+            const int64_t at = (int64_t)lane * A.ld + i;
+            pc[lane] = SQUARE ? A.col[at] : wcol[at];
+            pv[lane] = SQUARE ? -2.0 * A.val[at] : (double)wval[at];
+        }
+        for (int32_t t0 = 0; t0 < l; t0 += 4) {
+            int32_t c[4], o[4];
+            double v[4];
+            bool ok[4];
+#pragma unroll
+            for (int u = 0; u < 4; ++u) {
+                const int t = t0 + u < l ? t0 + u : t0;
+                const int32_t kt = __shfl(k, t, 64), lt = __shfl(lk, t, 64), ot = __shfl(off, t, 64);
+                const double ct = __shfl(coef, t, 64);
+                ok[u] = t0 + u < l && lane < lt;
+                const int64_t at = (int64_t)(ok[u] ? lane : 0) * A.ld + kt;
+                c[u] = SQUARE ? A.col[at] : wcol[at];
+                v[u] = ct * (SQUARE ? A.val[at] : (double)wval[at]);
+                o[u] = ot + lane;
+            }
+#pragma unroll
+            for (int u = 0; u < 4; ++u)
+                if (ok[u]) {
+                    pc[o[u]] = c[u];
+                    pv[o[u]] = v[u];
+                }
+        }
+        __syncthreads();
+        for (int p = lane; p < tot; p += 64) {
+            const int32_t c = pc[p];
+            uint32_t slot = ((uint32_t)c * 2654435761u) >> 16 & (SLOTS - 1);
+            bool placed = false;
+            for (int probe = 0; probe < SLOTS && !placed; ++probe) {
+                const int32_t prev = atomicCAS(&tc[slot], -1, c);
+                placed = prev == -1 || prev == c;
+                slot = (slot + 1) & (SLOTS - 1);
+            }
+            if (!placed) full = 1;
+        }
+        __syncthreads();
+        if (full) {
+            bad = true;
+            if (lane == 0) olen[i] = 0;
+            continue;
+        }
+        int32_t mine[PER], rank[PER];
+        double sum[PER];
+#pragma unroll
+        for (int m = 0; m < PER; ++m) {
+            mine[m] = tc[lane + 64 * m];
+            rank[m] = 0;
+            sum[m] = 0.0;
+        }
+        int cnt = 0;
+        for (int q = 0; q < SLOTS; ++q) {
+            const int32_t c = tc[q];
+            cnt += c >= 0 ? 1 : 0;
+#pragma unroll
+            for (int m = 0; m < PER; ++m) rank[m] += c >= 0 && c < mine[m] ? 1 : 0;
+        }
+        for (int p = 0; p < tot; ++p) {
+            const int32_t c = pc[p];
+            const double t = pv[p];
+#pragma unroll
+            for (int m = 0; m < PER; ++m)
+                if (c == mine[m]) sum[m] += t;
+        }
+        bool diag = false;
+#pragma unroll
+        for (int m = 0; m < PER; ++m) {
+            if (mine[m] < 0) continue;
+            const int o = rank[m];
+            if (SQUARE) {
+                const int64_t at = ((int64_t)(o / 8) * A.ld + i) * 8 + o % 8;
+                ocol[at] = mine[m];
+                oval[at] = (float)((mine[m] == (int32_t)i ? 1.0 : 0.0) + OMEGA * dinv[mine[m]] * sum[m]);
+                diag = diag || mine[m] == (int32_t)i;
+            } else {
+                ocol[(int64_t)o * A.ld + i] = mine[m];
+                oval[(int64_t)o * A.ld + i] = (float)sum[m];
+            }
+        }
+        if (SQUARE) {
+            const int p = cnt + lane;
+            if (p < ((cnt + 7) & ~7)) {
+                const int64_t at = ((int64_t)(p / 8) * A.ld + i) * 8 + p % 8;
+                ocol[at] = (int32_t)i;
+                oval[at] = 0.0f;
+            }
+            if (!__any(diag ? 1 : 0)) bad = true;
+        }
+        if (lane == 0) olen[i] = cnt;
+        if (cnt > cap) bad = true;
+    }
+    if (bad) *flag = 1ull;
 }
 
 __device__ __forceinline__ int galerkin_products(int64_t ld, const int32_t *__restrict__ apcol,
@@ -1218,6 +1464,64 @@
     default: return n <= FOLD_MAX_ROWS;
     }
 }
+constexpr int64_t FOLD_WIDE_MAX_ROWS = 131072;
+int e2_slots(int maxlen) { return maxlen <= 5 ? 16 : maxlen <= 20 ? 64 : 128; }
+bool fold_visit_wanted(const SHierarchy *H, int level, int64_t n, int maxlen) {
+    if (level > 0 && n <= TAIL_MAX_N) return false;
+    if (H->nu[level < 2 ? level : 2] != 2) return false;
+    static const int mode = [] {
+        const char *e = getenv("NODAL_SA_FOLD_VISIT");
+        return !e || !*e ? -1 : (atoi(e) != 0 ? 1 : 0);
+    }();
+    if (mode == 0) return false;
+    if (e2_slots(maxlen) > 16 && n > FOLD_WIDE_MAX_ROWS) return false;
+    return mode == 1 || (level > 0 && n <= FOLD_MAX_ROWS);
+}
+int fold_cap() {
+    static const int cap = getenv("NODAL_SA_FOLD_CAP") && atoi(getenv("NODAL_SA_FOLD_CAP")) > 0 ? atoi(getenv("NODAL_SA_FOLD_CAP")) : 1 << 30;
+    return cap;
+}
+
+int fold_visit_products(nodal_ctx *h, SHierarchy *H, int l, hipStream_t st, hipEvent_t w_ready) {
+    SLevel *L = H->pool[l];
+    if (!L->pre_want && !L->v_want) return NODAL_OK;
+    const int64_t n = L->n;
+    Ell A = L->A();
+    A.width = L->maxlen;
+    const double *dinv = L->dinv.as<double>();
+    unsigned long long *lst = H->stats.as<unsigned long long>() + (size_t)l * ST_COUNT;
+    const unsigned g = (unsigned)((n + 63) / 64 < 4096 ? (n + 63) / 64 : 4096);
+    if (L->pre_want) {
+        int32_t *ec = L->ecol.as<int32_t>(), *el = L->elen.as<int32_t>();
+        float *ev = L->eval.as<float>();
+        const unsigned gw = (unsigned)(n < 65536 ? n : 65536);
+        if (L->eslots == 128) fold_rows_wave<128, true><<<gw, 64, 0, st>>>(A, dinv, nullptr, nullptr, nullptr, ec, ev, el, fold_cap(), lst + ST_E2MISS);
+        else if (L->eslots == 64) fold_rows_wave<64, true><<<gw, 64, 0, st>>>(A, dinv, nullptr, nullptr, nullptr, ec, ev, el, fold_cap(), lst + ST_E2MISS);
+        else fold_rows<true><<<g, 64, 0, st>>>(A, dinv, nullptr, nullptr, nullptr, ec, ev, el, fold_cap(), lst + ST_E2MISS);
+        NODAL_HIP_TRY(h, hipGetLastError());
+    }
+    if (L->v_want) {
+        if (w_ready) NODAL_HIP_TRY(h, hipStreamWaitEvent(st, w_ready, 0));
+        const int32_t *wc = L->wcol.as<int32_t>(), *wl = L->wlen.as<int32_t>();
+        const float *wv = L->wval.as<float>();
+        int32_t *vc = L->vcol.as<int32_t>(), *vl = L->vlen.as<int32_t>();
+        float *vv = L->vval.as<float>();
+        if (L->wslots == 64) fold_rows_wave<64, false><<<(unsigned)(n < 65536 ? n : 65536), 64, 0, st>>>(A, dinv, wc, wv, wl, vc, vv, vl, fold_cap(), lst + ST_VMISS);
+        else fold_rows<false><<<g, 64, 0, st>>>(A, dinv, wc, wv, wl, vc, vv, vl, fold_cap(), lst + ST_VMISS);
+        NODAL_HIP_TRY(h, hipGetLastError());
+    }
+    return NODAL_OK;
+}
+int join_fold(nodal_ctx *h, SHierarchy *H) {
+    if (!H->fold_aux) return NODAL_OK;
+    H->fold_aux = false;
+    if (!H->aux) return NODAL_OK;
+    NODAL_HIP_TRY(h, hipEventRecord(H->ev_fold, H->aux));
+    NODAL_HIP_TRY(h, hipStreamWaitEvent(h->stream, H->ev_fold, 0));
+    H->aux_pending = false;
+    return NODAL_OK;
+}
+
 void decide_folds(SHierarchy *H, const unsigned long long *hs, bool trace) {
     for (int k = 0; k < H->nlev; ++k) {
         SLevel *L = H->pool[k];
@@ -1228,6 +1532,22 @@
             fprintf(stderr, "[sagg] level %d (%lld rows): first post-smoothing sweep %s\n", k, (long long)L->n,
                     miss ? "NOT folded: a row of A P lacks a column of its P row (no stored diagonal)"
                          : "folded into the prolongation");
+        const bool emiss = hs[(size_t)k * ST_COUNT + ST_E2MISS] != 0, vmiss = hs[(size_t)k * ST_COUNT + ST_VMISS] != 0;
+        L->fold_pre = L->pre_want && runs_cycle && !emiss;
+        L->fold_v = L->v_want && L->fold && L->fold_pre && !vmiss;
+        const bool pre_wanted = L->pre_want;
+        if (L->pre_want && runs_cycle && emiss) L->pre_want = L->v_want = false;
+        if (L->v_want && runs_cycle && vmiss) L->v_want = false;
+        if (trace && pre_wanted && runs_cycle) {
+            const char *why = "a row of E2 overflows its slots or has no stored diagonal";
+            if (emiss)
+                fprintf(stderr, "[sagg] level %d (%lld rows): sweep pairs NOT folded, the visit keeps its launches: %s\n", k,
+                        (long long)L->n, why);
+            else
+                fprintf(stderr, "[sagg] level %d (%lld rows): pre-smoothing pair folded into one launch (E2: %d slots), "
+                                "post-smoothing pair %s\n", k, (long long)L->n, (int)L->eslots,
+                        L->fold_v ? "folded into one launch" : (vmiss ? "NOT folded: a row of V overflows its slots" : "NOT folded: no W"));
+        }
     }
 }
 
@@ -1316,13 +1636,16 @@
         (void)hipStreamDestroy(H->aux);
         H->aux = nullptr;
         H->aux_tried = false;
+        H->fold_aux = false;
     }
     if (fork_allowed && !H->aux_tried && nodal_extra_streams_ok(h)) {
         H->aux_tried = true;
         if (hipStreamCreateWithFlags(&H->aux, hipStreamNonBlocking) != hipSuccess) H->aux = nullptr;
         if (H->aux && ((!H->ev_fork && hipEventCreateWithFlags(&H->ev_fork, hipEventDisableTiming) != hipSuccess) ||
                        (!H->ev_join && hipEventCreateWithFlags(&H->ev_join, hipEventDisableTiming) != hipSuccess) ||
-                       (!H->ev_flags && hipEventCreateWithFlags(&H->ev_flags, hipEventDisableTiming) != hipSuccess))) {
+                       (!H->ev_flags && hipEventCreateWithFlags(&H->ev_flags, hipEventDisableTiming) != hipSuccess) ||
+                       (!H->ev_w && hipEventCreateWithFlags(&H->ev_w, hipEventDisableTiming) != hipSuccess) ||
+                       (!H->ev_fold && hipEventCreateWithFlags(&H->ev_fold, hipEventDisableTiming) != hipSuccess))) {
             (void)hipStreamDestroy(H->aux);
             H->aux = nullptr;
         }
@@ -1366,6 +1689,20 @@
             NODAL_HIP_TRY(h, L->wval.reserve((size_t)apw * ld * 4 + 64));
             NODAL_HIP_TRY(h, L->wlen.reserve((size_t)ld * 4 + 64));
         }
+        L->fold_pre = L->fold_v = false;
+        L->pre_want = fold_visit_wanted(H, l, n, L->maxlen);
+        L->v_want = L->pre_want && L->fold_want;
+        L->eslots = e2_slots(L->maxlen);
+        if (L->pre_want) {
+            NODAL_HIP_TRY(h, L->ecol.reserve((size_t)L->eslots * ld * 4 + 64));
+            NODAL_HIP_TRY(h, L->eval.reserve((size_t)L->eslots * ld * 4 + 64));
+            NODAL_HIP_TRY(h, L->elen.reserve((size_t)ld * 4 + 64));
+        }
+        if (L->v_want) {
+            NODAL_HIP_TRY(h, L->vcol.reserve((size_t)apw * ld * 4 + 64));
+            NODAL_HIP_TRY(h, L->vval.reserve((size_t)apw * ld * 4 + 64));
+            NODAL_HIP_TRY(h, L->vlen.reserve((size_t)ld * 4 + 64));
+        }
     }
     hipStream_t main_st = h->stream;
     struct StreamGuard {
@@ -1378,6 +1715,7 @@
         NODAL_HIP_TRY(h, hipStreamWaitEvent(H->aux, H->ev_fork, 0));
         H->aux_pending = true;
         NODAL_TRY(galerkin_product<false>(h, H, l, nullptr, 1));
+        if (L->v_want) NODAL_HIP_TRY(h, hipEventRecord(H->ev_w, main_st));
         h->stream = H->aux;
         st = H->aux;
     }
@@ -1413,11 +1751,16 @@
             NODAL_HIP_TRY(h, hipEventRecord(H->ev_flags, H->aux));
             H->flags_levels = l + 1;
         }
+        if (L->pre_want) {
+            NODAL_TRY(fold_visit_products(h, H, l, H->aux, H->ev_w));
+            H->fold_aux = true;
+        }
         h->stream = main_st;
         st = main_st;
     }
     NODAL_TRY(galerkin_product<false>(h, H, l, forked ? H->ev_join : nullptr, forked ? 2 : 0));
-    if (forked && H->flags_levels != l + 1) H->aux_pending = false;
+    if (!forked) NODAL_TRY(fold_visit_products(h, H, l, main_st, nullptr));
+    if (forked && H->flags_levels != l + 1) H->aux_pending = H->fold_aux;
     return NODAL_OK;
 }
 
@@ -1586,14 +1929,102 @@
                     "(worst row against its own bound: %.3e)\n", l, (long long)n, (int)L->wslots, (int)L->maxlen, dm, qm);
     return NODAL_OK;
 }
+template <typename TC>
+int visit_check_level(nodal_ctx *h, SHierarchy *H, int l, bool two) {
+    hipStream_t st = h->stream;
+    const SLevel *L = H->pool[l];
+    const int64_t n = L->n, nc = H->pool[l + 1]->n;
+    const Ell A = L->A();
+    uint64_t seed = 0x9e3779b97f4a7c15ull + 64 + (uint64_t)l;
+    auto unit = [&]() {
+        uint64_t z = (seed += 0x9e3779b97f4a7c15ull);
+        z = (z ^ (z >> 30)) * 0xbf58476d1ce4e5b9ull;
+        z = (z ^ (z >> 27)) * 0x94d049bb133111ebull;
+        z ^= z >> 31;
+        return (double)(z >> 11) * (1.0 / 4503599627370496.0) - 1.0;
+    };
+    std::vector<cyc_t> hb((size_t)n);
+    std::vector<TC> he((size_t)2 * nc);
+    for (auto &v : hb) v = (cyc_t)unit();
+    for (auto &v : he) v = (TC)unit();
+    const double hcoef[2] = {0.9, 0.4};
+    const size_t vb = align256((size_t)n * sizeof(cyc_t)), eb = align256((size_t)nc * sizeof(TC)), db = align256((size_t)n * 8);
+    enum { B = 0, X0, X1T, RT, RF, X1F, YF, MT, OT, OF, NV };
+    DevBuf buf;
+    hipError_t e = buf.reserve(NV * vb + 2 * eb + 5 * db + 256);
+    char *p = buf.as<char>();
+    auto vec = [&](int k) { return reinterpret_cast<cyc_t *>(p + (size_t)k * vb); };
+    TC *c1 = reinterpret_cast<TC *>(p + NV * vb), *c2 = reinterpret_cast<TC *>(p + NV * vb + eb);
+    double *dd = reinterpret_cast<double *>(p + NV * vb + 2 * eb);
+    double *mag = dd, *d0 = dd + db / 8, *q0 = dd + 2 * (db / 8), *d1 = dd + 3 * (db / 8), *q1 = dd + 4 * (db / 8);
+    double *coef = reinterpret_cast<double *>(p + NV * vb + 2 * eb + 5 * db);
+    if (e == hipSuccess) e = hipMemcpyAsync(vec(B), hb.data(), (size_t)n * sizeof(cyc_t), hipMemcpyHostToDevice, st);
+    if (e == hipSuccess) e = hipMemcpyAsync(c1, he.data(), (size_t)nc * sizeof(TC), hipMemcpyHostToDevice, st);
+    if (e == hipSuccess) e = hipMemcpyAsync(c2, he.data() + nc, (size_t)nc * sizeof(TC), hipMemcpyHostToDevice, st);
+    if (e == hipSuccess) e = hipMemcpyAsync(coef, hcoef, sizeof hcoef, hipMemcpyHostToDevice, st);
+    const bool post = L->fold_v;
+    if (e == hipSuccess) {
+        const unsigned g = grid_for(n), tb = L->wfix ? TB : TB * LPR_RAGGED;
+        const double *dinv = L->dinv.as<double>(), *cf = two ? coef : nullptr;
+        const TC *e2 = two ? c2 : nullptr;
+        const int32_t *ec = L->ecol.as<int32_t>(), *el = L->elen.as<int32_t>();
+        const float *ev = L->eval.as<float>();
+        const cyc_t *b = vec(B);
+        k_visit_x0<<<g, TB, 0, st>>>(n, dinv, b, vec(X0));
+        SAGG_DISPATCH_W(L->wfix, (k_post<W, false, cyc_t, cyc_t><<<g, tb, 0, st>>>(A, dinv, b, vec(X0), vec(X1T), nullptr, nullptr, nullptr)));
+        SAGG_DISPATCH_W(L->wfix, (k_smooth_residual<W, cyc_t><<<g, tb, 0, st>>>(A, b, vec(X1T), vec(RT))));
+        k_pre_pair<cyc_t><<<grid_for(n * EL), TB, 0, st>>>(A, ec, ev, el, dinv, b, vec(X0), vec(RF), vec(X1F), vec(YF));
+        k_visit_mag<true, TC><<<g, TB, 0, st>>>(A, dinv, b, vec(X0), nullptr, nullptr, nullptr, c1, e2, cf, mag);
+        k_visit_check<true, TC><<<g, TB, 0, st>>>(A, dinv, b, nullptr, mag, ec, ev, el, c1, e2, cf, vec(RT), vec(X1T), vec(RF),
+                                                 vec(YF), d0, q0);
+        if (post) {
+            const int32_t *wc = L->wcol.as<int32_t>(), *wl = L->wlen.as<int32_t>(), *vc = L->vcol.as<int32_t>(),
+                          *vl = L->vlen.as<int32_t>();
+            const float *wv = L->wval.as<float>(), *vv = L->vval.as<float>();
+            k_prolong_post<TC, cyc_t><<<g, TB, 0, st>>>(n, L->ld, wc, wv, wl, vec(X1F), vec(RF), dinv, c1, e2, cf, vec(MT));
+            SAGG_DISPATCH_W(L->wfix, (k_post<W, false, cyc_t, cyc_t><<<g, tb, 0, st>>>(A, dinv, b, vec(MT), vec(OT), nullptr, nullptr, nullptr)));
+            SAGG_DISPATCH_W(L->wfix, (k_post_pair<W, false, TC, cyc_t, cyc_t><<<g, TB, 0, st>>>(A, dinv, b, vec(YF), vc, vv, vl, c1, e2, cf,
+                                                                                               vec(OF), nullptr, nullptr, nullptr)));
+            k_visit_mag<false, TC><<<g, TB, 0, st>>>(A, dinv, b, vec(YF), wc, wv, wl, c1, e2, cf, mag);
+            k_visit_check<false, TC><<<g, TB, 0, st>>>(A, dinv, b, vec(YF), mag, vc, vv, vl, c1, e2, cf, vec(OT), nullptr, vec(OF),
+                                                      nullptr, d1, q1);
+        }
+        e = hipGetLastError();
+    }
+    std::vector<double> hd((size_t)n), hq((size_t)n);
+    double m[2][2] = {{0.0, 0.0}, {0.0, 0.0}};
+    if (e == hipSuccess) e = hipStreamSynchronize(st);
+    for (int k = 0; k < (post ? 2 : 1); ++k) {
+        if (e == hipSuccess) e = hipMemcpy(hd.data(), k ? d1 : d0, (size_t)n * 8, hipMemcpyDeviceToHost);
+        if (e == hipSuccess) e = hipMemcpy(hq.data(), k ? q1 : q0, (size_t)n * 8, hipMemcpyDeviceToHost);
+        if (e != hipSuccess) break;
+        for (int64_t i = 0; i < n; ++i) {
+            m[k][0] = !(hd[i] <= m[k][0]) ? hd[i] : m[k][0];
+            m[k][1] = !(hq[i] <= m[k][1]) ? hq[i] : m[k][1];
+        }
+    }
+    buf.release();
+    NODAL_HIP_TRY(h, e);
+    fprintf(stderr, "[sagg] visit check: level %d, rows %lld, pre pair, slots %d, width %d, fused launch against the two d = %.3e "
+                    "(worst row against its own bound: %.3e)\n", l, (long long)n, (int)L->eslots, (int)L->maxlen, m[0][0], m[0][1]);
+    if (post)
+        fprintf(stderr, "[sagg] visit check: level %d, rows %lld, post pair, slots %d, width %d, fused launch against the two d = %.3e "
+                        "(worst row against its own bound: %.3e)\n", l, (long long)n, (int)L->wslots, (int)L->maxlen, m[1][0], m[1][1]);
+    return NODAL_OK;
+}
 int fold_self_check(nodal_ctx *h, SHierarchy *H) {
     static const bool check = getenv("NODAL_TRACE") && getenv("NODAL_SA_FOLD_CHECK") && atoi(getenv("NODAL_SA_FOLD_CHECK")) != 0;
     if (!check) return NODAL_OK;
     for (int l = 0; l + 1 < H->nlev; ++l) {
-        if (!H->pool[l]->fold) continue;
         const bool last = l + 1 == H->tail || l + 1 == H->nlev - 1;
-        if (last) NODAL_TRY(fold_check_level<double>(h, H, l, false));
-        else NODAL_TRY(fold_check_level<cyc_t>(h, H, l, true));
+        if (H->pool[l]->fold) {
+            if (last) NODAL_TRY(fold_check_level<double>(h, H, l, false));
+            else NODAL_TRY(fold_check_level<cyc_t>(h, H, l, true));
+        }
+        if (H->pool[l]->fold_pre) {
+            if (last) NODAL_TRY(visit_check_level<double>(h, H, l, false));
+            else NODAL_TRY(visit_check_level<cyc_t>(h, H, l, true));
+        }
     }
     return NODAL_OK;
 }
@@ -1718,9 +2149,17 @@
                                                      L->pcol.as<int32_t>(), L->pval.as<double>(), L->rval.as<double>(),
                                                      L->rvalf.as<float>());
         NODAL_HIP_TRY(h, hipGetLastError());
-        if (forked) NODAL_HIP_TRY(h, hipEventRecord(H->ev_join, H->aux));
+        if (forked) {
+            NODAL_HIP_TRY(h, hipEventRecord(H->ev_join, H->aux));
+            if (L->pre_want) {
+                if (L->v_want) NODAL_HIP_TRY(h, hipEventRecord(H->ev_w, st));
+                NODAL_TRY(fold_visit_products(h, H, l, H->aux, H->ev_w));
+                H->fold_aux = true;
+            }
+        }
         NODAL_TRY(galerkin_product<true>(h, H, l, forked ? H->ev_join : nullptr, forked ? 2 : 0));
-        if (forked) H->aux_pending = false;
+        if (!forked) NODAL_TRY(fold_visit_products(h, H, l, st, nullptr));
+        if (forked) H->aux_pending = H->fold_aux;
     }
     const int last = H->nlev - 1;
     if (H->dense_coarsest)
@@ -1728,6 +2167,7 @@
     if (H->tail >= 0) k_tail_pack<<<1, 1024, 0, st>>>(H->td, H->tail_image.as<char>());
     NODAL_HIP_TRY(h, hipGetLastError());
     NODAL_TRY(form_tail_op(h, H));
+    NODAL_TRY(join_fold(h, H));
     NODAL_HIP_TRY(h, hipMemcpyAsync(hs, dstats, (size_t)MAX_LEVELS * ST_COUNT * 8, hipMemcpyDeviceToHost, st));
     NODAL_WAIT_STREAM(h, st);
     const int64_t bar = n0 / 100 < 32 ? (n0 / 100 > 0 ? n0 / 100 : 1) : 32;
@@ -1759,6 +2199,7 @@
         H->aux_pending = false;
         (void)hipGetLastError();
     }
+    if (H) H->fold_aux = false;
     return s;
 }
 
@@ -1870,6 +2311,7 @@
     H->nlev = l + 1;
     SLevel *last = H->level(l);
     last->fold_want = last->fold = false;
+    last->pre_want = last->v_want = last->fold_pre = last->fold_v = false;
     if (H->nlev < 2) return NODAL_OK;
     NODAL_HIP_TRY(h, hipMemcpyAsync(hs, dstats, (size_t)MAX_LEVELS * ST_COUNT * 8, hipMemcpyDeviceToHost, st));
     if (!H->ev_copy) NODAL_HIP_TRY(h, hipEventCreateWithFlags(&H->ev_copy, hipEventDisableTiming));
@@ -1880,7 +2322,7 @@
             NODAL_TRY(grounded_flags(h, H->level(0)->gflag.as<uint8_t>()));
         } else {
             NODAL_HIP_TRY(h, hipStreamWaitEvent(st, H->ev_flags, 0));
-            H->aux_pending = false;
+            H->aux_pending = H->fold_aux;
         }
         for (int k = H->flags_levels; k + 1 < H->nlev; ++k) {
             SLevel *L = H->pool[k], *C = H->pool[k + 1];
@@ -1920,6 +2362,7 @@
     }
     NODAL_TRY(build_tail(h, H, hs));
 
+    NODAL_TRY(join_fold(h, H));
     if (!check_floating) {
         NODAL_HIP_TRY(h, hipMemcpyAsync(hs, dstats, (size_t)MAX_LEVELS * ST_COUNT * 8, hipMemcpyDeviceToHost, st));
         NODAL_WAIT_STREAM(h, st);
@@ -2009,9 +2452,20 @@
     const unsigned tb = L->wfix ? TB : TB * LPR_RAGGED;
     const int nu = H->nu[l < 2 ? l : 2];
     const bool fold = L->fold && !(sb && nu == 1);
+    const bool pre = nu == 2 && L->fold_pre, post = pre && fold && L->fold_v;
     auto hand_up = [&](const auto *c1, const auto *c2, const double *cf) {
         using TC = std::remove_cv_t<std::remove_pointer_t<decltype(c1)>>;
-        if (!fold)
+        if (post) {
+            const int32_t *vc = L->vcol.as<int32_t>(), *vl = L->vlen.as<int32_t>();
+            const float *vv = L->vval.as<float>();
+            if (sb) {
+                SAGG_DISPATCH_W(L->wfix, (k_post_pair<W, true, TC, TBV, TOUT><<<g, TB, 0, st>>>(A, dinv, b, xp, vc, vv, vl, c1, c2, cf, out,
+                                                                                               sb->Ap, sb->part_rz, sb->part_zap)));
+            } else {
+                SAGG_DISPATCH_W(L->wfix, (k_post_pair<W, false, TC, TBV, TOUT><<<g, TB, 0, st>>>(A, dinv, b, xp, vc, vv, vl, c1, c2, cf, out,
+                                                                                                nullptr, nullptr, nullptr)));
+            }
+        } else if (!fold)
             k_prolong<TC><<<grid_for(n), TB, 0, st>>>(n, L->ld, L->pcol.as<int32_t>(), L->pvalf.as<float>(), x, c1, c2, cf, xp);
         else if (nu == 1)
             k_prolong_post<TC, TOUT><<<grid_for(n), TB, 0, st>>>(n, L->ld, L->wcol.as<int32_t>(), L->wval.as<float>(),
@@ -2020,7 +2474,12 @@
             k_prolong_post<TC, cyc_t><<<grid_for(n), TB, 0, st>>>(n, L->ld, L->wcol.as<int32_t>(), L->wval.as<float>(),
                                                                 L->wlen.as<int32_t>(), x, r, dinv, c1, c2, cf, xp);
     };
-    if (nu >= 2) {
+    if (pre) {
+        cyc_t *x1 = L->v<cyc_t>(V_X1);
+        k_pre_pair<TBV><<<grid_for(n * EL), TB, 0, st>>>(A, L->ecol.as<int32_t>(), L->eval.as<float>(), L->elen.as<int32_t>(), dinv,
+                                                        b, x0, r, post ? nullptr : x1, post ? xp : nullptr);
+        x = x1;
+    } else if (nu >= 2) {
         cyc_t *x1 = L->v<cyc_t>(V_X1);
         SAGG_DISPATCH_W(L->wfix, (k_post<W, false, TBV, cyc_t><<<g, tb, 0, st>>>(A, dinv, b, x0, x1, nullptr, nullptr, nullptr)));
         x = x1;
@@ -2030,7 +2489,7 @@
         SAGG_DISPATCH_W(L->wfix, (k_post<W, false, TBV, cyc_t><<<g, tb, 0, st>>>(A, dinv, b, x, x2, nullptr, nullptr, nullptr)));
         x = x2;
     }
-    SAGG_DISPATCH_W(L->wfix, (k_smooth_residual<W, TBV><<<g, tb, 0, st>>>(A, b, x, r)));
+    if (!pre) SAGG_DISPATCH_W(L->wfix, (k_smooth_residual<W, TBV><<<g, tb, 0, st>>>(A, b, x, r)));
     const bool last = l + 1 == H->tail || l + 1 == H->nlev - 1;
     const double *coef = nullptr;
     if (last) {
@@ -2085,7 +2544,7 @@
         hand_up((const cyc_t *)c1, (const cyc_t *)c2, coef);
     }
     const cyc_t *cur = xp;
-    const int left = fold ? nu - 1 : nu;
+    const int left = post ? 0 : (fold ? nu - 1 : nu);
     if (left == 0) {
         NODAL_HIP_TRY(h, hipGetLastError());
         return NODAL_OK;
@@ -2298,6 +2757,9 @@
             for (const void *q : ps) mix((uint64_t)(uintptr_t)q);
             mix((uint64_t)(L->fold ? 1 + L->wslots : 0));
             if (L->fold) { mix((uint64_t)(uintptr_t)L->wcol.p); mix((uint64_t)(uintptr_t)L->wval.p); mix((uint64_t)(uintptr_t)L->wlen.p); }
+            mix((uint64_t)((L->fold_pre ? 1 + L->eslots : 0) * 2 + (L->fold_v ? 1 : 0)));
+            if (L->fold_pre) { mix((uint64_t)(uintptr_t)L->ecol.p); mix((uint64_t)(uintptr_t)L->eval.p); mix((uint64_t)(uintptr_t)L->elen.p); }
+            if (L->fold_v) { mix((uint64_t)(uintptr_t)L->vcol.p); mix((uint64_t)(uintptr_t)L->vval.p); mix((uint64_t)(uintptr_t)L->vlen.p); }
             mix((uint64_t)L->n); mix((uint64_t)L->ld); mix((uint64_t)L->wfix); mix((uint64_t)L->rld);
         }
         if (H->it_exec && H->it_key != key) H->drop_graph();
diff --git a/nodal_amd/csrc/sagg_cycle.h b/nodal_amd/csrc/sagg_cycle.h
--- a/nodal_amd/csrc/sagg_cycle.h
+++ b/nodal_amd/csrc/sagg_cycle.h
@@ -399,6 +399,208 @@
         d[i] = di;
         q[i] = di / ((double)(lw + la + 8) * 0x1p-23);
     }
+}
+
+constexpr int EL = 8;
+template <typename TBV>
+__global__ __launch_bounds__(TB) void k_pre_pair(Ell A, const int32_t *__restrict__ ecol, const float *__restrict__ eval,
+                                                 const int32_t *__restrict__ elen, const double *__restrict__ dinv,
+                                                 const TBV *__restrict__ b, const cyc_t *__restrict__ x0,
+                                                 cyc_t *__restrict__ r, cyc_t *__restrict__ x1, cyc_t *__restrict__ y) {
+    constexpr int AQ = 4, EQ = 8;
+    const int sub = threadIdx.x & (EL - 1);
+    const int64_t rows_per_pass = (int64_t)gridDim.x * (TB / EL);
+    for (int64_t i0 = (int64_t)xcd_block() * (TB / EL); i0 < A.n; i0 += rows_per_pass) {
+        const int64_t i = i0 + threadIdx.x / EL;
+        double sa = 0.0, se = 0.0;
+        if (i < A.n) {
+            const int32_t la = A.len[i], le = elen[i];
+            for (int32_t a0 = 0, e0 = 0; a0 < la || e0 * EL < le; a0 += AQ * EL, e0 += EQ) {
+                int32_t ca[AQ], ce[EQ];
+                double va[AQ], ve[EQ];
+#pragma unroll
+                for (int u = 0; u < AQ; ++u) {
+                    const int32_t s = a0 + sub + u * EL;
+                    const bool ok = s < la;
+                    const int64_t at = (int64_t)(ok ? s : 0) * A.ld + i;
+                    const int32_t c = A.col[at];
+                    const float loaded = A.valf[at];
+                    ca[u] = ok ? c : (int32_t)i;
+                    va[u] = ok ? (double)loaded : 0.0;
+                }
+#pragma unroll
+                for (int u = 0; u < EQ; ++u) {
+                    const bool ok = (e0 + u) * EL < le;
+                    const int64_t at = ((int64_t)(ok ? e0 + u : 0) * A.ld + i) * EL + sub;
+                    const int32_t c = ecol[at];
+                    const float loaded = eval[at];
+                    ce[u] = ok ? c : (int32_t)i;
+                    ve[u] = ok ? (double)loaded : 0.0;
+                }
+#pragma unroll
+                for (int u = 0; u < AQ; ++u) sa = fma(va[u], (double)x0[ca[u]], sa);
+#pragma unroll
+                for (int u = 0; u < EQ; ++u) se = fma(ve[u], (double)b[ce[u]], se);
+            }
+        }
+#pragma unroll
+        for (int off = EL >> 1; off > 0; off >>= 1) {
+            sa += __shfl_down(sa, off, EL);
+            se += __shfl_down(se, off, EL);
+        }
+        if (i < A.n && sub == 0) {
+            const double wd = OMEGA * dinv[i];
+            const cyc_t rs = (cyc_t)se;
+            const cyc_t xs = (cyc_t)fma(wd, (double)b[i] - sa, (double)x0[i]);
+            r[i] = rs;
+            if (x1) x1[i] = xs;
+            if (y) y[i] = (cyc_t)fma(wd, (double)rs, (double)xs);
+        }
+    }
+}
+
+template <int W, bool DOTS, typename TC, typename TBV, typename TOUT>
+__global__ __launch_bounds__(TB) void k_post_pair(Ell A, const double *__restrict__ dinv, const TBV *__restrict__ b,
+                                                  const cyc_t *__restrict__ y, const int32_t *__restrict__ vcol,
+                                                  const float *__restrict__ vval, const int32_t *__restrict__ vlen,
+                                                  const TC *__restrict__ c1, const TC *__restrict__ c2,
+                                                  const double *__restrict__ coef, TOUT *__restrict__ out,
+                                                  const double *__restrict__ u, double *__restrict__ p_ob,
+                                                  double *__restrict__ p_ou) {
+    static_assert(LPR_RAGGED == 1, "one thread per row");
+    constexpr int Q = 8, Q0 = 16;
+    const bool two = coef != nullptr;
+    const double s1 = two ? coef[0] : 1.0, s2 = two ? coef[1] : 0.0;
+    double a0 = 0.0, a1 = 0.0;
+    for (int64_t i = (int64_t)xcd_block() * TB + threadIdx.x; i < A.n; i += (int64_t)gridDim.x * TB) {
+        const int32_t len = vlen[i];
+        int32_t J[Q0];
+        float wf[Q0];
+#pragma unroll
+        for (int q = 0; q < Q0; ++q) {
+            J[q] = vcol[(int64_t)q * A.ld + i];
+            wf[q] = vval[(int64_t)q * A.ld + i];
+        }
+        [[maybe_unused]] int32_t ac[W > 0 ? W : 1];
+        [[maybe_unused]] float av[W > 0 ? W : 1];
+        if constexpr (W > 0) ell_row_load<W>(A, A.valf, i, ac, av);
+        double acc = 0.0;
+#pragma unroll
+        for (int q = 0; q < Q0; ++q) {
+            const int32_t j = q < len ? J[q] : 0;
+            const double e = two ? s1 * (double)c1[j] + s2 * (double)c2[j] : (double)c1[j];
+            acc = fma(q < len ? (double)wf[q] : 0.0, e, acc);
+        }
+        double s;
+        if constexpr (W > 0) s = ell_row_sum<W>(i, ac, av, [&](int32_t j) { return (double)y[j]; });
+        else s = ell_row_w<W>(A, A.valf, i, 0, [&](int32_t j) { return (double)y[j]; });
+        for (int32_t q0 = Q0; q0 < len; q0 += Q) {
+            int32_t Jr[Q];
+            double w[Q];
+#pragma unroll
+            for (int q = 0; q < Q; ++q) {
+                const bool ok = q0 + q < len;
+                const int64_t at = (int64_t)(ok ? q0 + q : q0) * A.ld + i;
+                Jr[q] = vcol[at];
+                const float loaded = vval[at];
+                w[q] = ok ? (double)loaded : 0.0;
+            }
+#pragma unroll
+            for (int q = 0; q < Q; ++q) {
+                const double e = two ? s1 * (double)c1[Jr[q]] + s2 * (double)c2[Jr[q]] : (double)c1[Jr[q]];
+                acc = fma(w[q], e, acc);
+            }
+        }
+        const double bi = (double)b[i];
+        const TOUT os = (TOUT)(fma(OMEGA * dinv[i], bi - s, (double)y[i]) + acc);
+        out[i] = os;
+        if (DOTS) {
+            const double o = (double)os;
+            a0 = fma(o, bi, a0);
+            a1 = fma(o, u[i], a1);
+        }
+    }
+    if (DOTS) {
+        a0 = block_sum<TB>(a0);
+        a1 = block_sum<TB>(a1);
+        if (threadIdx.x == 0) {
+            p_ob[blockIdx.x] = a0;
+            p_ou[blockIdx.x] = a1;
+        }
+    }
+}
+
+template <bool PRE, typename TC>
+__global__ __launch_bounds__(TB) void k_visit_mag(Ell A, const double *__restrict__ dinv, const cyc_t *__restrict__ b,
+                                                  const cyc_t *__restrict__ v, const int32_t *__restrict__ wcol,
+                                                  const float *__restrict__ wval, const int32_t *__restrict__ wlen,
+                                                  const TC *__restrict__ c1, const TC *__restrict__ c2,
+                                                  const double *__restrict__ coef, double *__restrict__ mag) {
+    const bool two = coef != nullptr;
+    const double s1 = two ? coef[0] : 1.0, s2 = two ? coef[1] : 0.0;
+    for (int64_t i = (int64_t)xcd_block() * TB + threadIdx.x; i < A.n; i += (int64_t)gridDim.x * TB) {
+        double s = 0.0;
+        if (PRE) {
+            const int32_t la = A.len[i];
+            for (int32_t t = 0; t < la; ++t)
+                s += fabs((double)A.valf[(int64_t)t * A.ld + i]) * fabs((double)v[A.col[(int64_t)t * A.ld + i]]);
+            mag[i] = fabs((double)v[i]) + OMEGA * dinv[i] * (fabs((double)b[i]) + s);
+        } else {
+            const int32_t lw = wlen[i];
+            for (int32_t t = 0; t < lw; ++t) {
+                const int32_t j = wcol[(int64_t)t * A.ld + i];
+                const double e = two ? s1 * (double)c1[j] + s2 * (double)c2[j] : (double)c1[j];
+                s += fabs((double)wval[(int64_t)t * A.ld + i]) * fabs(e);
+            }
+            mag[i] = fabs((double)v[i]) + s;
+        }
+    }
+}
+template <bool PRE, typename TC>
+__global__ __launch_bounds__(TB) void k_visit_check(Ell A, const double *__restrict__ dinv, const cyc_t *__restrict__ b,
+                                                    const cyc_t *__restrict__ yv, const double *__restrict__ mag,
+                                                    const int32_t *__restrict__ ocol, const float *__restrict__ oval,
+                                                    const int32_t *__restrict__ olen, const TC *__restrict__ c1,
+                                                    const TC *__restrict__ c2, const double *__restrict__ coef,
+                                                    const cyc_t *__restrict__ t0, const cyc_t *__restrict__ t1,
+                                                    const cyc_t *__restrict__ f0, const cyc_t *__restrict__ f1,
+                                                    double *__restrict__ d, double *__restrict__ q) {
+    const bool two = coef != nullptr;
+    const double s1 = two ? coef[0] : 1.0, s2 = two ? coef[1] : 0.0;
+    for (int64_t i = (int64_t)xcd_block() * TB + threadIdx.x; i < A.n; i += (int64_t)gridDim.x * TB) {
+        const int32_t la = A.len[i], lo = olen[i];
+        const double wd = OMEGA * dinv[i];
+        double am = 0.0, om = 0.0;
+        for (int32_t t = 0; t < la; ++t)
+            am += fabs((double)A.valf[(int64_t)t * A.ld + i]) * mag[A.col[(int64_t)t * A.ld + i]];
+        double di;
+        if (PRE) {
+            for (int32_t t = 0; t < lo; ++t) {
+                const int64_t at = ((int64_t)(t / EL) * A.ld + i) * EL + t % EL;
+                om += fabs((double)oval[at]) * fabs((double)b[ocol[at]]);
+            }
+            const double den_r = fabs((double)b[i]) + am + om, den_y = mag[i] + wd * den_r;
+            const double yt = (double)(cyc_t)fma(wd, (double)t0[i], (double)t1[i]);
+            const double dr = fabs((double)f0[i] - (double)t0[i]) / den_r, dy = fabs((double)f1[i] - yt) / den_y;
+            di = !(dr <= dy) ? dr : dy;
+            if (dy != dy) di = dy;
+        } else {
+            for (int32_t t = 0; t < lo; ++t) {
+                const int32_t j = ocol[(int64_t)t * A.ld + i];
+                const double e = two ? s1 * (double)c1[j] + s2 * (double)c2[j] : (double)c1[j];
+                om += fabs((double)oval[(int64_t)t * A.ld + i]) * fabs(e);
+            }
+            const double den = fabs((double)yv[i]) + wd * (fabs((double)b[i]) + am) + om;
+            di = fabs((double)f0[i] - (double)t0[i]) / den;
+        }
+        d[i] = di;
+        q[i] = di / ((double)(lo + la + 8) * 0x1p-23);
+    }
+}
+__global__ __launch_bounds__(TB) void k_visit_x0(int64_t n, const double *__restrict__ dinv, const cyc_t *__restrict__ b,
+                                                 cyc_t *__restrict__ x0) {
+    for (int64_t i = (int64_t)xcd_block() * TB + threadIdx.x; i < n; i += (int64_t)gridDim.x * TB)
+        x0[i] = (cyc_t)(OMEGA * dinv[i] * (double)b[i]);
 }
 
 template <int W>
```

New measurement: 170.7 circuits/s, median of 6. 3.7% higher.
